# NomaDamas/AutoRAG-Research

Hardware: AMD Instinct MI355X
Metric: queries/sec (higher is better)
Workload: dtype f32

## Files before the change

### autorag_research_amd/_native.py

```python

from __future__ import annotations

import ctypes
import os
from pathlib import Path

import numpy as np

_PKG_DIR = Path(__file__).resolve().parent
LIB_PATH = _PKG_DIR / "libmi355dr.so"

_lib: ctypes.CDLL | None = None

ABI_SYMBOLS = [
    "mi355dr_create", "mi355dr_destroy", "mi355dr_last_error", "mi355dr_version", "mi355dr_reserve",
    "mi355dr_add_rows", "mi355dr_add_rows_device", "mi355dr_size", "mi355dr_dim", "mi355dr_get_rows",
    "mi355dr_update_rows", "mi355dr_update_rows_device", "mi355dr_remove_rows", "mi355dr_live_rows", "mi355dr_compact",
    "mi355dr_search", "mi355dr_search_device", "mi355dr_search_device_async", "mi355dr_search_wait",
    "mi355dr_search_subset", "mi355dr_search_subset_device", "mi355dr_score_subset", "mi355dr_search_mmr", "mi355dr_search_mmr_device", "mi355dr_mmr_select", "mi355dr_merge_groups_device", "mi355dr_search_groups", "mi355dr_search_groups_device", "mi355dr_search_range", "mi355dr_search_range_device",
    "mi355dr_search_rows", "mi355dr_search_rows_device", "mi355dr_search_range_rows", "mi355dr_search_range_rows_device", "mi355dr_view_create", "mi355dr_add_multivec", "mi355dr_size_multivec",
    "mi355dr_search_maxsim", "mi355dr_search_maxsim_device", "mi355dr_search_maxsim_subset", "mi355dr_search_maxsim_subset_device", "mi355dr_maxsim_subset", "mi355dr_maxsim_subset_ex", "mi355dr_add_multivec_device", "mi355dr_gqr_refine", "mi355dr_gqr_refine_maxsim",
    "mi355dr_set_multivec", "mi355dr_set_multivec_device", "mi355dr_live_multivec",
    "mi355dr_add_sparse", "mi355dr_size_sparse", "mi355dr_sparse_df", "mi355dr_search_sparse", "mi355dr_search_sparse_device",
    "mi355dr_search_bm25", "mi355dr_search_bm25_device",
    "mi355dr_gqr_refine_scores", "mi355dr_merge_topk_device", "mi355dr_pack_topk_device",
    "mi355dr_merge_topk_packed_device", "mi355dr_comm_unique_id", "mi355dr_comm_init", "mi355dr_comm_world", "mi355dr_comm_count", "mi355dr_comm_init_custom",
    "mi355dr_search_sharded_device", "mi355dr_search_range_sharded_device", "mi355dr_search_rows_sharded_device",
    "mi355dr_search_range_rows_sharded_device", "mi355dr_search_mmr_sharded_device", "mi355dr_mmr_select_sharded",
    "mi355dr_set_option", "mi355dr_get_stat",
    "mi355dr_reset_stats", "mi355dr_timer_start", "mi355dr_timer_stop", "mi355dr_synchronize",
    "mi355dr_dev_alloc", "mi355dr_dev_free", "mi355dr_dev_upload", "mi355dr_dev_download",
    "mi355dr_diag_mfma_stream",
    "mi355dr_debug_screen_dense", "mi355dr_debug_screen_hits", "mi355dr_debug_screen_bound", "mi355dr_debug_i8_state", "mi355dr_debug_rescore",
    "mi355dr_debug_maxsim_pass",
]


ALLGATHER_FN = ctypes.CFUNCTYPE(ctypes.c_int, ctypes.c_void_p, ctypes.c_void_p, ctypes.c_size_t, ctypes.c_void_p, ctypes.c_void_p)


class NativeError(RuntimeError):

    def __init__(self, code: int, message: str):
        super().__init__(f"libmi355dr error {code}: {message}")
        self.code = code


def _preload_torch_hip_runtime() -> None:
    import importlib.util
    import sys

    if "torch" in sys.modules:
        return
    try:
        spec = importlib.util.find_spec("torch")
    except (ImportError, ValueError):
        return
    if spec is None or not spec.submodule_search_locations:
        return
    libdir = Path(list(spec.submodule_search_locations)[0]) / "lib"
    for name in ("libhsa-runtime64.so", "libamdhip64.so"):
        f = libdir / name
        if f.exists():
            try:
                ctypes.CDLL(str(f), mode=getattr(os, "RTLD_NOW", 2) | getattr(os, "RTLD_GLOBAL", 0x100))
            except OSError:
                return


def load() -> ctypes.CDLL:
    global _lib
    if _lib is not None:
        return _lib
    if not LIB_PATH.exists():
        raise ImportError(
            f"{LIB_PATH} not found: build it with `python -c 'import __graft_entry__ as g; g.build()'` "
            "(hipcc --offload-arch=gfx950).  There is no CPU fallback for the search path."
        )
    _preload_torch_hip_runtime()
    L = ctypes.CDLL(str(LIB_PATH), mode=getattr(os, "RTLD_NOW", 2))
    vp, c_int, i64 = ctypes.c_void_p, ctypes.c_int, ctypes.c_int64
    f32p, f64p = ctypes.POINTER(ctypes.c_float), ctypes.POINTER(ctypes.c_double)
    i64p, i32p = ctypes.POINTER(ctypes.c_int64), ctypes.POINTER(ctypes.c_int32)
    L.mi355dr_create.restype = c_int
    L.mi355dr_create.argtypes = [ctypes.POINTER(vp), c_int, c_int, c_int]
    L.mi355dr_destroy.restype = None
    L.mi355dr_destroy.argtypes = [vp]
    L.mi355dr_last_error.restype = ctypes.c_char_p
    L.mi355dr_last_error.argtypes = [vp]
    L.mi355dr_version.restype = c_int
    L.mi355dr_reserve.restype = c_int
    L.mi355dr_reserve.argtypes = [vp, i64]
    L.mi355dr_add_rows.restype = c_int
    L.mi355dr_add_rows.argtypes = [vp, f32p, i64]
    L.mi355dr_add_rows_device.restype = c_int
    L.mi355dr_add_rows_device.argtypes = [vp, vp, i64]
    L.mi355dr_update_rows.restype = c_int
    L.mi355dr_update_rows.argtypes = [vp, i64p, f32p, i64]
    L.mi355dr_update_rows_device.restype = c_int
    L.mi355dr_update_rows_device.argtypes = [vp, i64p, vp, i64]
    L.mi355dr_remove_rows.restype = c_int
    L.mi355dr_remove_rows.argtypes = [vp, i64p, i64]
    L.mi355dr_compact.restype = c_int
    L.mi355dr_compact.argtypes = [vp, i64p]
    L.mi355dr_live_rows.restype = i64
    L.mi355dr_live_rows.argtypes = [vp]
    L.mi355dr_size.restype = i64
    L.mi355dr_size.argtypes = [vp]
    L.mi355dr_dim.restype = c_int
    L.mi355dr_dim.argtypes = [vp]
    L.mi355dr_get_rows.restype = c_int
    L.mi355dr_get_rows.argtypes = [vp, i64, i64, f32p]
    L.mi355dr_search.restype = c_int
    L.mi355dr_search.argtypes = [vp, f32p, c_int, c_int, f64p, i64p]
    L.mi355dr_search_device.restype = c_int
    L.mi355dr_search_device.argtypes = [vp, vp, c_int, c_int, vp, vp, vp]
    L.mi355dr_search_device_async.restype = c_int
    L.mi355dr_search_device_async.argtypes = [vp, vp, c_int, c_int, vp, vp, vp, i64p]
    L.mi355dr_search_wait.restype = c_int
    L.mi355dr_search_wait.argtypes = [vp, i64]
    L.mi355dr_search_subset.restype = c_int
    L.mi355dr_search_subset.argtypes = [vp, f32p, c_int, c_int, i64p, i64, f64p, i64p]
    L.mi355dr_search_subset_device.restype = c_int
    L.mi355dr_search_subset_device.argtypes = [vp, vp, c_int, c_int, i64p, i64, vp, vp, vp]
    L.mi355dr_score_subset.restype = c_int
    L.mi355dr_score_subset.argtypes = [vp, f32p, c_int, i64p, c_int, f64p]
    L.mi355dr_search_mmr.restype = c_int
    L.mi355dr_search_mmr.argtypes = [vp, f32p, c_int, c_int, c_int, ctypes.c_double, f64p, i64p]
    L.mi355dr_search_mmr_device.restype = c_int
    L.mi355dr_search_mmr_device.argtypes = [vp, vp, c_int, c_int, c_int, ctypes.c_double, vp, vp, vp]
    L.mi355dr_mmr_select.restype = c_int
    L.mi355dr_mmr_select.argtypes = [vp, f32p, c_int, c_int, i64p, c_int, ctypes.c_double, f64p, i64p]
    L.mi355dr_merge_groups_device.restype = c_int
    L.mi355dr_merge_groups_device.argtypes = [vp, vp, vp, c_int, c_int, i32p, c_int, c_int, vp, vp, vp, vp]
    L.mi355dr_search_groups.restype = c_int
    L.mi355dr_search_groups.argtypes = [vp, f32p, i32p, c_int, c_int, c_int, f64p, i64p, i32p]
    L.mi355dr_search_groups_device.restype = c_int
    L.mi355dr_search_groups_device.argtypes = [vp, vp, i32p, c_int, c_int, c_int, vp, vp, vp, vp]
    L.mi355dr_search_range.restype = c_int
    L.mi355dr_search_range.argtypes = [vp, f32p, c_int, f64p, c_int, f64p, i64p, i64p]
    L.mi355dr_search_range_device.restype = c_int
    L.mi355dr_search_range_device.argtypes = [vp, vp, c_int, f64p, c_int, vp, vp, vp, vp]
    L.mi355dr_search_rows.restype = c_int
    L.mi355dr_search_rows.argtypes = [vp, i64p, c_int, c_int, c_int, f64p, i64p]
    L.mi355dr_search_rows_device.restype = c_int
    L.mi355dr_search_rows_device.argtypes = [vp, i64p, c_int, c_int, c_int, vp, vp, vp]
    L.mi355dr_search_range_rows.restype = c_int
    L.mi355dr_search_range_rows.argtypes = [vp, i64p, c_int, f64p, c_int, c_int, f64p, i64p, i64p]
    L.mi355dr_search_range_rows_device.restype = c_int
    L.mi355dr_search_range_rows_device.argtypes = [vp, i64p, c_int, f64p, c_int, c_int, vp, vp, vp, vp]
    L.mi355dr_view_create.restype = c_int
    L.mi355dr_view_create.argtypes = [vp, i64p, i64, i64p, i64, ctypes.POINTER(vp)]
    L.mi355dr_add_multivec.restype = c_int
    L.mi355dr_add_multivec.argtypes = [vp, f32p, i64p, i64]
    L.mi355dr_size_multivec.restype = i64
    L.mi355dr_size_multivec.argtypes = [vp]
    L.mi355dr_search_maxsim.restype = c_int
    L.mi355dr_search_maxsim.argtypes = [vp, f32p, i32p, c_int, c_int, f32p, i64p]
    L.mi355dr_search_maxsim_device.restype = c_int
    L.mi355dr_search_maxsim_device.argtypes = [vp, vp, i32p, c_int, c_int, vp, vp, vp]
    L.mi355dr_search_maxsim_subset.restype = c_int
    L.mi355dr_search_maxsim_subset.argtypes = [vp, f32p, i32p, c_int, c_int, i64p, i64, f32p, i64p]
    L.mi355dr_search_maxsim_subset_device.restype = c_int
    L.mi355dr_search_maxsim_subset_device.argtypes = [vp, vp, i32p, c_int, c_int, i64p, i64, vp, vp, vp]
    L.mi355dr_maxsim_subset.restype = c_int
    L.mi355dr_maxsim_subset.argtypes = [vp, f32p, i32p, c_int, i64p, c_int, f32p]
    L.mi355dr_maxsim_subset_ex.restype = c_int
    L.mi355dr_maxsim_subset_ex.argtypes = [vp, f32p, i32p, c_int, i64p, c_int, c_int, f32p]
    L.mi355dr_add_multivec_device.restype = c_int
    L.mi355dr_add_multivec_device.argtypes = [vp, vp, i64p, i64]
    L.mi355dr_set_multivec.restype = c_int
    L.mi355dr_set_multivec.argtypes = [vp, i64p, f32p, i64p, i64]
    L.mi355dr_set_multivec_device.restype = c_int
    L.mi355dr_set_multivec_device.argtypes = [vp, i64p, vp, i64p, i64]
    L.mi355dr_live_multivec.restype = i64
    L.mi355dr_live_multivec.argtypes = [vp]
    c_double = ctypes.c_double
    L.mi355dr_add_sparse.restype = c_int
    L.mi355dr_add_sparse.argtypes = [vp, i32p, i64p, i64]
    L.mi355dr_size_sparse.restype = i64
    L.mi355dr_size_sparse.argtypes = [vp]
    L.mi355dr_sparse_df.restype = c_int
    L.mi355dr_sparse_df.argtypes = [vp, i32p, i64, i64p]
    L.mi355dr_search_sparse.restype = c_int
    L.mi355dr_search_sparse.argtypes = [vp, i32p, f64p, i32p, c_int, c_int, c_double, c_double, f64p, i64p]
    L.mi355dr_search_sparse_device.restype = c_int
    L.mi355dr_search_sparse_device.argtypes = [vp, i32p, f64p, i32p, c_int, c_int, c_double, c_double, vp, vp, vp]
    L.mi355dr_search_bm25.restype = c_int
    L.mi355dr_search_bm25.argtypes = [vp, i32p, i32p, c_int, c_int, c_double, c_double, f64p, i64p]
    L.mi355dr_search_bm25_device.restype = c_int
    L.mi355dr_search_bm25_device.argtypes = [vp, i32p, i32p, c_int, c_int, c_double, c_double, vp, vp, vp]
    L.mi355dr_gqr_refine.restype = c_int
    L.mi355dr_gqr_refine.argtypes = [vp, f64p, c_int, i64p, c_int, f64p, c_int, c_double, c_double, c_double, f64p]
    L.mi355dr_gqr_refine_maxsim.restype = c_int
    L.mi355dr_gqr_refine_maxsim.argtypes = [vp, f64p, i32p, c_int, i64p, c_int, f64p, c_int, c_double, c_double, c_double,
                                            f64p]
    L.mi355dr_gqr_refine_scores.restype = c_int
    L.mi355dr_gqr_refine_scores.argtypes = [vp, f64p, i32p, c_int, c_int, f64p, c_int, c_double, c_double, c_double, f64p]
    L.mi355dr_merge_topk_device.restype = c_int
    L.mi355dr_merge_topk_device.argtypes = [vp, vp, vp, c_int, c_int, c_int, vp, vp, vp]
    L.mi355dr_pack_topk_device.restype = c_int
    L.mi355dr_pack_topk_device.argtypes = [vp, vp, vp, c_int, c_int, vp, vp]
    L.mi355dr_merge_topk_packed_device.restype = c_int
    L.mi355dr_merge_topk_packed_device.argtypes = [vp, vp, c_int, c_int, c_int, vp, vp, vp]
    L.mi355dr_comm_unique_id.restype = c_int
    L.mi355dr_comm_unique_id.argtypes = [vp, ctypes.c_size_t]
    L.mi355dr_comm_init.restype = c_int
    L.mi355dr_comm_init.argtypes = [vp, c_int, c_int, vp, ctypes.c_size_t]
    L.mi355dr_comm_init_custom.restype = c_int
    L.mi355dr_comm_init_custom.argtypes = [vp, c_int, c_int, ALLGATHER_FN, vp]
    L.mi355dr_comm_world.restype = c_int
    L.mi355dr_comm_world.argtypes = [vp]
    L.mi355dr_comm_count.restype = c_int
    L.mi355dr_comm_count.argtypes = [vp, ctypes.POINTER(c_int)]
    L.mi355dr_search_sharded_device.restype = c_int
    L.mi355dr_search_sharded_device.argtypes = [vp, vp, c_int, c_int, vp, vp, vp]
    L.mi355dr_search_range_sharded_device.restype = c_int
    L.mi355dr_search_range_sharded_device.argtypes = [vp, vp, c_int, f64p, c_int, vp, vp, vp, vp]
    L.mi355dr_search_rows_sharded_device.restype = c_int
    L.mi355dr_search_rows_sharded_device.argtypes = [vp, i64p, c_int, c_int, c_int, vp, vp, vp]
    L.mi355dr_search_range_rows_sharded_device.restype = c_int
    L.mi355dr_search_range_rows_sharded_device.argtypes = [vp, i64p, c_int, f64p, c_int, c_int, vp, vp, vp, vp]
    L.mi355dr_search_mmr_sharded_device.restype = c_int
    L.mi355dr_search_mmr_sharded_device.argtypes = [vp, vp, c_int, c_int, c_int, ctypes.c_double, vp, vp, vp]
    L.mi355dr_mmr_select_sharded.restype = c_int
    L.mi355dr_mmr_select_sharded.argtypes = [vp, f32p, c_int, c_int, i64p, c_int, ctypes.c_double, f64p, i64p]
    L.mi355dr_set_option.restype = c_int
    L.mi355dr_set_option.argtypes = [vp, ctypes.c_char_p, i64]
    L.mi355dr_get_stat.restype = c_int
    L.mi355dr_get_stat.argtypes = [vp, ctypes.c_char_p, i64p]
    L.mi355dr_reset_stats.restype = c_int
    L.mi355dr_reset_stats.argtypes = [vp]
    L.mi355dr_timer_start.restype = c_int
    L.mi355dr_timer_start.argtypes = [vp]
    L.mi355dr_timer_stop.restype = c_int
    L.mi355dr_timer_stop.argtypes = [vp, f64p]
    L.mi355dr_synchronize.restype = c_int
    L.mi355dr_synchronize.argtypes = [vp]
    L.mi355dr_dev_alloc.restype = c_int
    L.mi355dr_dev_alloc.argtypes = [vp, ctypes.c_size_t, ctypes.POINTER(vp)]
    L.mi355dr_dev_free.restype = c_int
    L.mi355dr_dev_free.argtypes = [vp, vp]
    L.mi355dr_dev_upload.restype = c_int
    L.mi355dr_dev_upload.argtypes = [vp, vp, vp, ctypes.c_size_t]
    L.mi355dr_dev_download.restype = c_int
    L.mi355dr_dev_download.argtypes = [vp, vp, vp, ctypes.c_size_t]
    L.mi355dr_debug_screen_dense.restype = c_int
    L.mi355dr_debug_screen_dense.argtypes = [vp, f32p, c_int, i64, i64, f32p]
    L.mi355dr_debug_screen_hits.restype = c_int
    L.mi355dr_debug_screen_hits.argtypes = [vp, f32p, c_int, i64, i64, f32p, c_int, ctypes.POINTER(c_int), i32p, f32p,
                                            ctypes.POINTER(c_int), ctypes.POINTER(c_int)]
    L.mi355dr_debug_screen_bound.restype = c_int
    L.mi355dr_debug_screen_bound.argtypes = [vp, f32p, c_int, f32p]
    L.mi355dr_debug_i8_state.restype = c_int
    L.mi355dr_debug_i8_state.argtypes = [vp, f32p, c_int, f32p, f32p, i64, i64, f32p, f32p]
    L.mi355dr_debug_rescore.restype = c_int
    L.mi355dr_debug_rescore.argtypes = [vp, f32p, c_int, i32p, i64p, i64, f32p, f64p]
    L.mi355dr_debug_maxsim_pass.restype = c_int
    L.mi355dr_debug_maxsim_pass.argtypes = [vp, f32p, i32p, c_int, c_int, i64p, i64, c_int, ctypes.POINTER(c_int), f32p, f32p, i32p,
                                            ctypes.POINTER(c_int), f32p, ctypes.POINTER(c_int), ctypes.POINTER(c_int)]
    L.mi355dr_diag_mfma_stream.restype = c_int
    L.mi355dr_diag_mfma_stream.argtypes = [c_int, c_int, ctypes.c_double, ctypes.POINTER(ctypes.c_double)]
    _lib = L
    return L


def diag_mfma_stream(device: int, fmt: str, seconds: float) -> float:
    out = ctypes.c_double(0.0)
    rc = load().mi355dr_diag_mfma_stream(int(device), {"i8": 0, "bf16": 1}[fmt], float(seconds), ctypes.byref(out))
    if rc != 0:
        raise NativeError(rc, "mi355dr_diag_mfma_stream failed")
    return float(out.value)


def check(handle, rc: int) -> None:
    if rc != 0:
        msg = load().mi355dr_last_error(handle)
        raise NativeError(rc, msg.decode("utf-8", "replace") if msg else "")


def f32c(a) -> np.ndarray:
    return np.ascontiguousarray(a, dtype=np.float32)


def ptr(a: np.ndarray, ct):
    return a.ctypes.data_as(ctypes.POINTER(ct))
```

### autorag_research_amd/csrc/dev_common.h

```cpp
#pragma once
#include <hip/hip_runtime.h>
#include <stdint.h>

namespace mi355 {

constexpr int kWave = 64;
constexpr int kQBlockMax = 1024;
constexpr int kKMax = 1024;
constexpr int kCandCap = 2048;
constexpr int kCandCapWide = 4096;
constexpr int kSortMax = 4096;
constexpr int kIrrCap = 1024;
constexpr uint64_t kKeyNaN = 0xFFFFFFFFFFFFFFFFull;
static_assert(kSortMax >= kKMax + kCandCap, "the general prune's sort must hold k kept entries and a full candidate list");

constexpr int kStOverflow = 1;
constexpr int kStIrregular = 2;

struct QueryState {
    float* qn;
    uint16_t* qhat;
    float* thr;
    int* cnt;
    int* best_n;
    uint64_t* best_key;
    int32_t* best_row;
    uint64_t* thr_key;
    int32_t* thr_row;
    int* status;
    float* E;
    float* E16;
    float* sc;
    float* kq;
    int8_t* qhat8;
    int* carry;
};

__device__ __forceinline__ float bf16_bits_to_f32(uint16_t h) { return __uint_as_float((uint32_t)h << 16); }

__host__ __device__ inline float bf16_screen_bound(float e_q, float e_c, int d, float cscale = 1.0f) {
    return 1.0001f * (e_q * cscale + e_c) + 3.0f * e_q * e_c + (8.0f * (float)d * 5.9604645e-8f + 1.5258789e-5f) * cscale;
}

constexpr float kI8Z = 6.0f;
constexpr int kI8GroupRows = 32;
struct I8Group {
    float step;
    float err;
};
__host__ __device__ inline float i8_row_peak_limit(int d) { return kI8Z / sqrtf((float)d); }
__host__ __device__ inline float i8_query_bound(float e_q, int d) {
    return 1.0001f * e_q + 4.0f * (float)d * 5.9604645e-8f + 1.5258789e-5f + 4.0e-6f;
}
__host__ __device__ inline float i8_pair_factor(float e_q) { return 1.0001f + 3.0f * e_q; }
__device__ __forceinline__ int i8_block_threshold(float th, float m, float ek) {
    const float r = __builtin_amdgcn_rcpf(m);
    const float x = (th - ek) * r;
    const float y = floorf(x - fabsf(x) * 4.8e-7f - fabsf(th) * (1.2e-7f * r) - 2.0f);
    int out;
    asm("v_cvt_i32_f32 %0, %1" : "=v"(out) : "v"(y));
    return out;
}

__device__ __forceinline__ float bits_f(uint32_t u) { return __uint_as_float(u); }

__device__ __forceinline__ uint16_t f32_to_bf16_rn(float f) {
    uint32_t u = __float_as_uint(f);
    u += 0x7FFFu + ((u >> 16) & 1u);
    return (uint16_t)(u >> 16);
}

__device__ __forceinline__ double cosine_distance_from(float dot, float nq, float nc) {
    double sim = (double)dot / sqrt((double)nq * (double)nc);
    if (sim > 1.0) sim = 1.0;
    else if (sim < -1.0) sim = -1.0;
    return 1.0 - sim;
}

__device__ __forceinline__ double distance_from(int metric, float dot, float nq, float nc) {
    return metric == 0 ? cosine_distance_from(dot, nq, nc) : (double)dot * -1.0;
}

__device__ __forceinline__ float sim_of_dist(int metric, double dist) {
    return metric == 0 ? (float)(1.0 - dist) : (float)(-dist);
}

__device__ __forceinline__ uint64_t dist_to_key(double d) {
    if (d != d) return kKeyNaN;
    uint64_t b = (uint64_t)__double_as_longlong(d);
    return (b >> 63) ? ~b : (b | 0x8000000000000000ull);
}
__device__ __forceinline__ double key_to_dist(uint64_t k) {
    if (k == kKeyNaN) return __longlong_as_double(0x7FF8000000000000ll);
    uint64_t b = (k >> 63) ? (k & 0x7FFFFFFFFFFFFFFFull) : ~k;
    return __longlong_as_double((long long)b);
}

__device__ __forceinline__ float float_below(float x) {
    if (x != x || x == -__builtin_inff()) return x;
    uint32_t u = __float_as_uint(x);
    if (x > 0.0f) u -= 1u;
    else if (x < 0.0f) u += 1u;
    else u = 0x80000001u;
    return __uint_as_float(u);
}

__device__ __forceinline__ bool norm_is_regular(float n2) { return n2 >= 1e-30f && n2 <= 1e30f; }

constexpr float kDeadNrm2 = -1.0f;
constexpr int32_t kRowNone = 0x7FFFFFFF;
__host__ __device__ __forceinline__ bool row_is_dead(float n2) { return n2 < 0.0f; }
__device__ __forceinline__ uint64_t exact_key_of(int metric, float dot, float nq, float nc, int32_t& row) {
    if (row_is_dead(nc)) {
        row = kRowNone;
        return kKeyNaN;
    }
    return dist_to_key(distance_from(metric, dot, nq, nc));
}

__device__ __forceinline__ int next_pow2(int x) {
    int p = 1;
    while (p < x) p <<= 1;
    return p;
}

__device__ __forceinline__ void bitonic_desc_f32(float* v, int n) {
    for (int k = 2; k <= n; k <<= 1) {
        for (int j = k >> 1; j > 0; j >>= 1) {
            for (int i = threadIdx.x; i < n; i += blockDim.x) {
                const int p = i ^ j;
                if (p > i) {
                    const bool desc = ((i & k) == 0);
                    const float a = v[i], b = v[p];
                    if (desc ? (a < b) : (a > b)) {
                        v[i] = b;
                        v[p] = a;
                    }
                }
            }
            __syncthreads();
        }
    }
}

constexpr int kSelPerLane = 16;

__device__ __forceinline__ uint32_t f32_order_key(float f) {
    const uint32_t u = __float_as_uint(f);
    return (u & 0x80000000u) ? ~u : (u | 0x80000000u);
}

template <int NS>
__device__ __forceinline__ int wave_count_ge_n(const uint32_t (&key)[kSelPerLane], uint32_t x) {
    int c = 0;
#pragma unroll
    for (int j = 0; j < NS; ++j) c += __builtin_popcountll(__builtin_amdgcn_ballot_w64(key[j] >= x));
    return c;
}
template <int NS>
__device__ __forceinline__ uint32_t wave_nth_largest_n(const uint32_t (&key)[kSelPerLane], int n) {
    uint32_t x = 0;
    for (int b = 31; b >= 0; --b) {
        const uint32_t t = x | (1u << b);
        if (wave_count_ge_n<NS>(key, t) >= n) x = t;
    }
    return x;
}
__device__ __forceinline__ int wave_count_ge(const uint32_t (&key)[kSelPerLane], uint32_t x, int entries) {
    if (entries <= kWave) return wave_count_ge_n<1>(key, x);
    if (entries <= 2 * kWave) return wave_count_ge_n<2>(key, x);
    if (entries <= 4 * kWave) return wave_count_ge_n<4>(key, x);
    if (entries <= 8 * kWave) return wave_count_ge_n<8>(key, x);
    return wave_count_ge_n<kSelPerLane>(key, x);
}
__device__ __forceinline__ uint32_t wave_nth_largest(const uint32_t (&key)[kSelPerLane], int n, int entries) {
    if (entries <= kWave) return wave_nth_largest_n<1>(key, n);
    if (entries <= 2 * kWave) return wave_nth_largest_n<2>(key, n);
    if (entries <= 4 * kWave) return wave_nth_largest_n<4>(key, n);
    if (entries <= 8 * kWave) return wave_nth_largest_n<8>(key, n);
    return wave_nth_largest_n<kSelPerLane>(key, n);
}

__device__ __forceinline__ int wave_count_ge(const uint32_t (&key)[kSelPerLane], uint32_t x) {
    return wave_count_ge_n<kSelPerLane>(key, x);
}
__device__ __forceinline__ uint32_t wave_nth_largest(const uint32_t (&key)[kSelPerLane], int n) {
    return wave_nth_largest_n<kSelPerLane>(key, n);
}
// ... 263 lines not shown
```

### autorag_research_amd/csrc/index.h

```cpp
#pragma once
#include <climits>
#include <hip/hip_runtime.h>

#include <algorithm>
#include <cmath>
#include <cstdio>
#include <cstring>
#include <mutex>
#include <string>
#include <vector>

#include "dev_common.h"
#include "mi355dr.h"

namespace mi355 {
template <class T, bool Pinned = false>
struct DevBuf {
    T* p = nullptr;
    size_t bytes = 0;
    DevBuf() = default;
    DevBuf(const DevBuf&) = delete;
    DevBuf& operator=(const DevBuf&) = delete;
    ~DevBuf() { release(); }
    void release() {
        if (p) (void)(Pinned ? hipHostFree(p) : hipFree(p));
        p = nullptr;
        bytes = 0;
    }
    hipError_t grow(size_t want) {
        if (want <= bytes) return hipSuccess;
        void* q = nullptr;
        const hipError_t e = Pinned ? hipHostMalloc(&q, want) : hipMalloc(&q, want);
        if (e != hipSuccess) return e;
        release();
        p = (T*)q;
        bytes = want;
        return hipSuccess;
    }
    void swap(DevBuf& o) {
        std::swap(p, o.p);
        std::swap(bytes, o.bytes);
    }
    operator T*() const { return p; }
};
template <class T>
using HostBuf = DevBuf<T, true>;

struct Event {
    hipEvent_t e = nullptr;
    Event() = default;
    Event(const Event&) = delete;
    Event& operator=(const Event&) = delete;
    ~Event() {
        if (e) (void)hipEventDestroy(e);
    }
    hipError_t create(unsigned flags = hipEventDefault) { return e ? hipSuccess : hipEventCreateWithFlags(&e, flags); }
    operator hipEvent_t() const { return e; }
};

struct EventPair {
    hipEvent_t a, b;
    int big;
};
struct EventPairs {
    std::vector<EventPair> v;
    ~EventPairs() {
        for (auto& p : v) {
            (void)hipEventDestroy(p.a);
            (void)hipEventDestroy(p.b);
        }
    }
};
struct MultiVecStore;
struct SparseStore;
struct Pass {
    int k = 0;
    int level = 0;
    bool screening = false;
    bool i8 = false;
    bool wide = false;
    int cap = 0;
    const char* refused = nullptr;
};
struct Pending {
    bool active = false;
    Event done;
    HostBuf<int> status_host;
    hipStream_t stream = nullptr;
    const float* q_dev = nullptr;
    int B = 0;
    Pass pass;
    double* out_dist = nullptr;
    int64_t* out_rows = nullptr;
};
struct RetryBufs {
    DevBuf<float> q;
    DevBuf<double> dist;
    DevBuf<int64_t> rows;
    DevBuf<int> map;
};
constexpr int kPendingRing = 4;

template <class... Bufs>
hipError_t grow_each(size_t n, Bufs&... bufs) {
    hipError_t e = hipSuccess;
    (void)(((e = bufs.grow(n * sizeof(*bufs.p))) == hipSuccess) && ...);
    return e;
}
struct MmrBufs {
    DevBuf<double> cand_dist;
    DevBuf<int64_t> cand_rows;
    DevBuf<unsigned long long> pairs_dev;
    hipError_t reserve(size_t nb, size_t stride) {
        hipError_t e = grow_each(nb * stride, cand_dist, cand_rows);
        if (!e) e = grow_each(1, pairs_dev);
        return e;
    }
};
struct GroupBufs {
    DevBuf<int32_t> offsets, count;
    DevBuf<double> cand_dist, out_dist;
    DevBuf<int64_t> cand_rows, out_rows;
    hipError_t reserve(size_t G, size_t S, size_t fetch_k, size_t k, bool host) {
        hipError_t e = grow_each(G + 1, offsets);
        if (!e) e = grow_each(S * fetch_k, cand_dist, cand_rows);
        if (!e && host) e = grow_each(G * k, out_dist, out_rows);
        if (!e && host) e = grow_each(G, count);
        return e;
    }
};
struct RangeBufs {
    DevBuf<uint64_t> key, rkey;
    DevBuf<int32_t> row, xfrom;
    DevBuf<unsigned long long> count, stat;
    DevBuf<double> radius, fb_dist;
    DevBuf<int> redo, flag, fb_map;
    DevBuf<int64_t> fb_rows;
    DevBuf<float> fb_q;
    int collect_lds = 0;
    hipError_t reserve(size_t nb, size_t R, size_t m, size_t pairs, size_t dim) {
        hipError_t e = grow_each(nb * R, key, row);
        if (!e) e = grow_each(nb, count, rkey, xfrom, radius, flag, fb_map);
        if (!e) e = grow_each(2, stat);
        if (!e) e = grow_each(2 + 2 * pairs, redo);
        if (!e) e = grow_each(nb * dim, fb_q);
        if (!e) e = grow_each(nb * m, fb_dist, fb_rows);
        return e;
    }
};
struct RowQueryBufs {
    DevBuf<int64_t> ids, pair_row, cand_rows, cand_count;
    DevBuf<float> q, self_dot;
    DevBuf<int> valid;
    DevBuf<int32_t> pair_q;
    DevBuf<double> cand_dist, self_dist, radius;
    DevBuf<unsigned long long> skipped_dev;
    hipError_t reserve(size_t nb, size_t stride, size_t dim, bool range) {
        hipError_t e = grow_each(nb, ids, valid, pair_q, pair_row);
        if (!e) e = grow_each(nb * dim, q);
        if (!e) e = grow_each(nb * stride, cand_dist, cand_rows);
        if (!e) e = grow_each(1, skipped_dev);
        if (!e && range) e = grow_each(nb, cand_count, self_dot, self_dist, radius);
        return e;
    }
};
struct ShardBufs {
    DevBuf<int64_t> send, recv;
    DevBuf<float> stage, stage_all;
    DevBuf<unsigned long long> local_skipped;
};
}

struct mi355dr_index {
    int device = 0, dim = 0, dpad = 0, metric = 0;
    hipStream_t stream = nullptr;
    std::mutex mu;
    std::string err;
    mi355dr_index() = default;
    ~mi355dr_index() {
        if (stream) (void)hipStreamDestroy(stream);
    }

    int64_t n = 0, cap_rows = 0;
    mi355::DevBuf<float> rows;
    mi355::DevBuf<uint16_t> shadow;
    mi355::DevBuf<float> nrm2;
    mi355::DevBuf<int32_t> irr_rows;
    mi355::DevBuf<int> irr_count;
    int irr_n = 0;
    mi355::DevBuf<unsigned> n2max_dev;
    float cmax = 0.0f;
    mi355::DevBuf<unsigned> bf16_res2_dev;
    float bf16_ec = 0.00390625f;
    int dpad8 = 0;
    mi355::DevBuf<int8_t> shadow8;
    mi355::DevBuf<uint8_t> flag8;
    mi355::DevBuf<mi355::I8Group> grp8;
    mi355::DevBuf<int32_t> irr8_rows;
    mi355::DevBuf<int> irr8_count;
    int irr8_n = 0;
    mi355::DevBuf<int> dead_count;
    int64_t dead_n = 0;

    bool qstate_ready = false;
    mi355::QueryState st{};
    mi355::DevBuf<void> st_mem[sizeof(mi355::QueryState) / sizeof(void*)];
    mi355::DevBuf<float> qdev;
    mi355::DevBuf<int32_t> cand_row;
    mi355::DevBuf<float> cand_val;
    mi355::DevBuf<int> qlist_dev;
    int* status_or_dev = nullptr;
    mi355::HostBuf<int> status_host;
    mi355::DevBuf<double> out_dist_dev;
    mi355::DevBuf<int64_t> out_rows_dev;
    mi355::DevBuf<int64_t> out_count_dev;
    mi355::DevBuf<unsigned long long> stat_dev;
    mi355::DevBuf<int> prune_skip;
    mi355::DevBuf<int32_t> subset_ids;
    mi355::MmrBufs mmr;
    mi355::GroupBufs grp;
    mi355::RangeBufs rng;
    mi355::RowQueryBufs rowq;
    mi355::ShardBufs shd;
    bool is_view = false;
    mi355::DevBuf<int64_t> view_row_map;
    mi355::DevBuf<int64_t> view_doc_map;
    int64_t view_rows = 0, view_docs = 0;
    int prune_parity = 0;

    int path = 0;
    int screen_dtype = 0;
    int i8_backoff = 0, i8_probation = 0;
    int i8_demoted_k = INT_MAX;
    double i8_min_budget = 0.25;
    mi355::RetryBufs retry[3];
    mi355::Pending pend[mi355::kPendingRing];
    mi355::Pending sub_pend[4];
    int64_t seq_next = 0, seq_done = 0;
    int last_pass_k = 10;
    int maxsim_coop = -1;
    int maxsim_persistent = 0;
    int maxsim_wg = -1;
    int maxsim_tighten = 1;
    int maxsim_aligned = 1;
    int maxsim_wg_min = 8;
    int maxsim_wg_pipe = 1;
    int maxsim_pack8 = -1;
    int maxsim_wg_bps = 4;
    int maxsim_pass_groups = 4;
    int maxsim_screen = 1;
    int maxsim_subset_screen = -1;
    int64_t maxsim_subset_screen_min = 512;
    int64_t row_offset = 0;
    int round_a = 0;
    int screen_rq = 1;
    int screen_stream = 1;
    int prefilter16 = 0;
    int profile = 0;
    int starter = 1;
    int prune_companion = 1;
    int scan_dma = 1;
    int defer_round_b = 1;
    int chunk0_set = 0;
    int64_t chunk0_rows = 1024;
    int64_t chunk_growth = 3;
    int chunk_growth_set = 0;
    int64_t small_chunk_rows = 16384;
    int cap = mi355::kCandCap;
    int cap_set = 0;
    int prune_wide = 1;
    int screen_flush_sync = 1, screen_flush_lanes = 48, screen_flush_alone = 40;
    int wide_inflation_x10 = 100;
    int chunk_taper_x100 = 0;
    int64_t compact_slice_rows = 65536;
    int64_t view_slice_rows = 65536;
    int64_t range_chunk_rows = (int64_t)1 << 21;
    int range_slots = mi355::kSortMax;
    int64_t shard_stage_bytes = (int64_t)256 << 20;
    int64_t starter_rows_wide = 65536;

    int64_t s_screen_launches = 0, s_screen_ns = 0, s_screen_rows = 0, s_fallback_queries = 0, s_chunks = 0,
            s_passes = 0, s_starters = 0;
    int64_t s_big_launches = 0, s_big_ns = 0, s_big_rows = 0;
    int screen_rq_split_tests = 1;
    int64_t debug_park = 0;
    mi355::DevBuf<float> park_thr;
    int screen_drift = 3;
    mi355::DevBuf<int> rq_progress;
    int rq_epoch = 0;
    int64_t s_rq_launches = 0;
    int64_t s_retry_queries = 0;
    int64_t s_ms_screened = 0, s_ms_candidates = 0, s_ms_fallbacks = 0;
    int64_t s_ms_screen_ns = 0, s_ms_screen_launches = 0, s_ms_exact_ns = 0, s_ms_exact_launches = 0, s_ms_pack_ns = 0;
    int64_t s_ms_packed_launches = 0;
    int64_t s_ms_packed_blocks = 0;
    int64_t s_ms_packed_built = 0;
    int64_t s_ms_set_docs = 0;
    int64_t s_ms_moved_blocks = 0;
    int64_t s_compactions = 0;
    int64_t s_compact_moved_rows = 0;
    int64_t s_subset_searches = 0;
    int64_t s_subset_rows_scored = 0;
    int64_t s_subset_rerun_queries = 0;
    int64_t s_mss_searches = 0, s_mss_docs = 0, s_mss_screened = 0, s_mss_exact = 0, s_mss_fallbacks = 0;
    int64_t s_mmr_searches = 0, s_mmr_queries = 0, s_mmr_pairs = 0;
    int64_t s_group_searches = 0, s_group_subqueries = 0, s_groups_merged = 0;
    int64_t s_range_searches = 0, s_range_queries = 0, s_range_in_range = 0, s_range_candidates = 0, s_range_rescored = 0,
            s_range_redo_chunks = 0, s_range_fallback_queries = 0;
    int64_t s_rows_searches = 0, s_rows_queries = 0, s_rows_skipped = 0;
    int64_t s_shard_range_searches = 0, s_shard_rows_searches = 0, s_shard_mmr_searches = 0, s_shard_gather_bytes = 0;
    int64_t s_sparse_searches = 0, s_sparse_queries = 0, s_sparse_postings_scored = 0, s_sparse_overflows = 0;
    int sparse_tile_docs = 2048;
    int sparse_cand_cap = 2048;
    int64_t s_ms_screen_cols = 0;
    mi355::Event ms_ev[4];
    struct MsScreenForm {
        int family = 0, ncb = 0, waves = 0, bps = 0, pipe = 0, now = 0, grid = 0, reserved = 0;
    } last_screen_form;
    mi355::EventPairs ev_pool, ev_pending;
    mi355::Event t0, t1;

    void* comm = nullptr;
    int comm_rank = 0, comm_world = 0;
    mi355dr_allgather_fn comm_custom = nullptr;
    void* comm_custom_user = nullptr;
    int64_t* comm_packed[2] = {nullptr, nullptr};
    int64_t* comm_packed_all[2] = {nullptr, nullptr};
    hipStream_t comm_stream = nullptr;
    hipEvent_t comm_done[2] = {nullptr, nullptr};
    bool comm_done_armed[2] = {false, false};
    size_t comm_cap = 0;

    mi355::MultiVecStore* mv = nullptr;
    mi355::SparseStore* sp = nullptr;
};


namespace mi355 {

int fail(mi355dr_index* idx, int code, const std::string& msg);
inline int view_refuses(mi355dr_index* idx, const char* what, bool ask_parent = false) {
    return fail(idx, MI355DR_E_INVALID, std::string(what) + (ask_parent ? ": not on a view (it is a read-only snapshot under the parent's ids) -- ask the parent index"
                                                                        : ": a view is read-only"));
}
void multivec_destroy(mi355dr_index* idx);
int multivec_reserve(mi355dr_index* idx, int64_t n_blocks, int64_t n_docs);
int64_t multivec_bytes(const mi355dr_index* idx);
void sparse_destroy(mi355dr_index* idx);
int64_t sparse_bytes(const mi355dr_index* idx);
enum { kSparseStatDocs, kSparseStatTotalLen, kSparseStatPostings, kSparseStatVocab };
int64_t sparse_stat(const mi355dr_index* idx, int which);
int drain_searches(mi355dr_index* idx);
void comm_destroy(mi355dr_index* idx);
int comm_all_gather(mi355dr_index* idx, const void* send_dev, void* recv_dev, size_t bytes_per_rank, hipStream_t stream);
struct MultiVecView {
    const float* tok;
    const int64_t* blk_off;
    const int64_t* blk_off_host;
    const int32_t* tok_cnt_host;
    int dpad;
    int64_t n_docs;
};
bool multivec_view(const mi355dr_index* idx, MultiVecView* out);

__host__ __device__ inline int ms_perm(int j) {
    constexpr int P[8] = {0, 4, 2, 6, 1, 5, 3, 7};
    return (j & ~7) | P[j & 7];
}

template <class T>
inline void multivec_pack_query_row(const T* src, int d, int dpad, T* dst) {
    for (int c = 0; c < dpad; ++c) {
        const int oc = ms_perm(c);
        dst[c] = oc < d ? src[oc] : T(0);
    }
}

#define HIPCHECK(idx, expr)                                                                              \
    do {                                                                                                 \
        hipError_t e__ = (expr);                                                                         \
        if (e__ != hipSuccess) {                                                                         \
            char buf__[512];                                                                             \
            snprintf(buf__, sizeof(buf__), "%s failed: %s (%s:%d)", #expr, hipGetErrorString(e__), __FILE__, \
                     __LINE__);                                                                          \
            return mi355::fail(idx, e__ == hipErrorOutOfMemory ? MI355DR_E_NOMEM : MI355DR_E_HIP, buf__); \
        }                                                                                                \
    } while (0)

#define CHECK(expr)                          \
    do {                                     \
        int rc__ = (expr);                   \
        if (rc__ != MI355DR_OK) return rc__; \
    } while (0)

inline int64_t round_up(int64_t x, int64_t m) { return (x + m - 1) / m * m; }

}
```

### autorag_research_amd/csrc/k_prep.h

```cpp
#pragma once
#include "dev_common.h"

namespace mi355 {

__global__ __launch_bounds__(64) void k_row_nrm2(const float* __restrict__ rows, int64_t row0, int64_t n, int d,
                                                  float* __restrict__ nrm2, unsigned* __restrict__ n2max,
                                                  const int64_t* __restrict__ ids) {
    __shared__ float tile[kStageFloats];
    const int lane = threadIdx.x;
    const int64_t j = (int64_t)blockIdx.x * kWave + lane;
    const bool live = j < n;
    const int64_t i = ids ? (live ? ids[j] : 0) : row0 + j;
    const float* my_row = live ? rows + i * (int64_t)d : nullptr;
    float acc = 0.0f;
    for (int k0 = 0; k0 < d; k0 += kStageCols) {
        stage_rows(tile, my_row, k0, d, lane);
        __syncthreads();
        const int kn = min(kStageCols, d - k0);
        const float* t = tile + lane * kStageLd;
        for (int k = 0; k < kn; ++k) acc = __builtin_fmaf(t[k], t[k], acc);
        __syncthreads();
    }
    if (live) nrm2[i] = acc;
    float m = (live && norm_is_regular(acc)) ? acc : 0.0f;
// ... 13 lines not shown
    __shared__ float sh[4];
    if ((int64_t)blockIdx.x >= n) return;
    const int64_t i = ids ? ids[blockIdx.x] : row0 + blockIdx.x;
    const float n2 = nrm2[i];
    const bool regular = norm_is_regular(n2);
    const float rc = regular ? (absolute ? 1.0f : 1.0f / sqrtf(n2)) : 0.0f;
    const float* r = rows + i * (int64_t)d;
    uint16_t* s = shadow + i * (int64_t)dpad;
    float e2 = 0.0f;
    for (int k = threadIdx.x; k < dpad; k += blockDim.x) {
        uint16_t v = 0;
        if (k < d) {
            if (regular) {
                const float ch = r[k] * rc;
                v = f32_to_bf16_rn(ch);
                const float e = ch - bf16_bits_to_f32(v);
                e2 = __builtin_fmaf(e, e, e2);
            } else {
                v = (uint16_t)0x7FC0;
            }
        }
        s[k] = v;
    }
#pragma unroll
    for (int o = 32; o > 0; o >>= 1) e2 += __shfl_xor(e2, o);
    if ((threadIdx.x & 63) == 0) sh[threadIdx.x >> 6] = e2;
    __syncthreads();
    if (threadIdx.x == 0) {
        if (regular) {
            const unsigned v = __float_as_uint((sh[0] + sh[1]) + (sh[2] + sh[3]));
            if (v > *(volatile unsigned*)res2_max) atomicMax(res2_max, v);
        }
        else if (ids == nullptr) {
            int slot = atomicAdd(irr_count, 1);
            if (slot < kIrrCap) irr_rows[slot] = (int32_t)i;
        }
    }
}


__device__ __forceinline__ float block256_reduce(float v, bool is_max, float* sh) {
#pragma unroll
    for (int o = 32; o > 0; o >>= 1) {
        const float w = __shfl_xor(v, o);
        v = is_max ? fmaxf(v, w) : v + w;
    }
    __syncthreads();
    if ((threadIdx.x & 63) == 0) sh[threadIdx.x >> 6] = v;
    __syncthreads();
    return is_max ? fmaxf(fmaxf(sh[0], sh[1]), fmaxf(sh[2], sh[3])) : (sh[0] + sh[1]) + (sh[2] + sh[3]);
}

__global__ __launch_bounds__(256) void k_build_shadow8(const float* __restrict__ rows, const float* __restrict__ nrm2,
                                                        int64_t g0, int64_t n_total, int64_t first_new, int d, int dpad8,
                                                        int8_t* __restrict__ shadow8, uint8_t* __restrict__ flag8,
                                                        I8Group* __restrict__ grp, int32_t* __restrict__ irr8_rows,
                                                        int* __restrict__ irr8_count, int absolute,
                                                        const int64_t* __restrict__ groups) {
    __shared__ float s_peak[kI8GroupRows];
    __shared__ float s_err[kI8GroupRows];
    __shared__ float s_step;
    const int lane = threadIdx.x & 63, wave = threadIdx.x >> 6;
    const int64_t g = groups ? groups[blockIdx.x] : g0 + blockIdx.x;
    const int64_t row_g = g * kI8GroupRows;
    const float peak_limit = i8_row_peak_limit(d);
    for (int j = 0; j < 8; ++j) {
        const int lr = wave * 8 + j;
        const int64_t i = row_g + lr;
        float peak = -1.0f;
        if (i < n_total) {
            const float n2 = nrm2[i];
            if (norm_is_regular(n2)) {
                const float rc = absolute ? 1.0f : 1.0f / sqrtf(n2);
                const float lim = absolute ? peak_limit * sqrtf(n2) : peak_limit;
                const float* r = rows + i * (int64_t)d;
                float mx = 0.0f;
                for (int k = lane; k < d; k += kWave) mx = fmaxf(mx, fabsf(r[k] * rc));
#pragma unroll
                for (int o = 32; o > 0; o >>= 1) mx = fmaxf(mx, __shfl_xor(mx, o));
                if (mx <= lim) peak = mx;
            }
        }
        if (lane == 0) s_peak[lr] = peak;
    }
    __syncthreads();
    if (threadIdx.x == 0) {
        float mx = 0.0f;
        for (int j = 0; j < kI8GroupRows; ++j) mx = fmaxf(mx, s_peak[j]);
        s_step = mx * (1.0f / 127.0f) * 1.0000005f;
    }
    __syncthreads();
    const float step = s_step;
    const float inv_step = step > 0.0f ? 1.0f / step : 0.0f;
    for (int j = 0; j < 8; ++j) {
        const int lr = wave * 8 + j;
        const int64_t i = row_g + lr;
        if (i >= n_total) {
            if (lane == 0) s_err[lr] = 0.0f;
            continue;
        }
        const bool tight = s_peak[lr] >= 0.0f && step > 0.0f;
        const float rc = tight ? (absolute ? 1.0f : 1.0f / sqrtf(nrm2[i])) : 0.0f;
        const float* r = rows + i * (int64_t)d;
        int8_t* s = shadow8 + i * (int64_t)dpad8;
        float e2 = 0.0f;
        for (int k = lane; k < dpad8; k += kWave) {
            float qv = 0.0f;
            if (k < d && tight) {
                const float ch = r[k] * rc;
                qv = fminf(fmaxf(rintf(ch * inv_step), -127.0f), 127.0f);
                const float e = __builtin_fmaf(-step, qv, ch);
                e2 = __builtin_fmaf(e, e, e2);
            }
            s[k] = (int8_t)qv;
        }
#pragma unroll
        for (int o = 32; o > 0; o >>= 1) e2 += __shfl_xor(e2, o);
        if (lane == 0) {
            s_err[lr] = tight ? sqrtf(e2) * 1.001f : 0.0f;
            flag8[i] = tight ? 0 : 1;
            if (!tight && i >= first_new) {
                const int slot = atomicAdd(irr8_count, 1);
                if (slot < kIrrCap) irr8_rows[slot] = (int32_t)i;
            }
        }
    }
    __syncthreads();
    if (threadIdx.x == 0) {
        float mx = 0.0f;
        for (int j = 0; j < kI8GroupRows; ++j) mx = fmaxf(mx, s_err[j]);
        grp[g].step = step;
        grp[g].err = mx;
    }
}

__global__ __launch_bounds__(64) void k_prep_queries(const float* __restrict__ q, int B, int d, int dpad, int metric,
                                                      QueryState st, int dpad8, int i8, float bf16_ec, int* status_or,
                                                      int* prune_skip, int cnt0, float cscale) {
    extern __shared__ float qs[];
    const int b = blockIdx.x;
    const int lane = threadIdx.x;
    if (b == 0 && lane == 0) {
        if (status_or) *status_or = 0;
        if (prune_skip) prune_skip[0] = prune_skip[1] = 0;
    }
    uint16_t* qh = st.qhat + (int64_t)b * dpad;
    if (b >= B) {
        for (int k = lane; k < dpad; k += kWave) qh[k] = 0;
        if (lane == 0) {
            st.qn[b] = 0.0f;
            st.thr[b] = __builtin_inff();
            st.cnt[b] = 0;
            st.carry[b] = 0;
            st.best_n[b] = 0;
            st.thr_key[b] = 0;
            st.thr_row[b] = -1;
            st.status[b] = 0;
            st.E[b] = bf16_screen_bound(0.00390625f, bf16_ec, d, cscale);
            st.E16[b] = st.E[b];
            st.sc[b] = 0.0f;
            st.kq[b] = 1.0f;
        }
        if (i8)
            for (int k = lane; k < dpad8; k += kWave) st.qhat8[(int64_t)b * dpad8 + k] = 0;
        return;
    }
    const float* qr = q + (int64_t)b * d;
    for (int k = lane; k < d; k += kWave) qs[k] = qr[k];
    __syncthreads();
    float acc = 0.0f;
    for (int k = 0; k < d; ++k) acc = __builtin_fmaf(qs[k], qs[k], acc);
    const bool regular = norm_is_regular(acc);
    const float rq = regular ? 1.0f / sqrtf(acc) : 0.0f;
    float eq2 = 0.0f;
    for (int k = lane; k < dpad; k += kWave) {
        uint16_t v = 0;
        if (k < d && regular) {
            const float qh_f = qs[k] * rq;
            v = f32_to_bf16_rn(qh_f);
            const float e = qh_f - bf16_bits_to_f32(v);
            eq2 = __builtin_fmaf(e, e, eq2);
        }
        qh[k] = v;
    }
#pragma unroll
    for (int o = 32; o > 0; o >>= 1) eq2 += __shfl_xor(eq2, o);
    float E = bf16_screen_bound(sqrtf(eq2) * 1.001f, bf16_ec, d, cscale), sc = 1.0f, kq = 1.0f;
    const float E16 = E;
    if (i8) {
        float mx = 0.0f;
        for (int k = lane; k < d; k += kWave) mx = fmaxf(mx, fabsf(qs[k] * rq));
#pragma unroll
        for (int o = 32; o > 0; o >>= 1) mx = fmaxf(mx, __shfl_xor(mx, o));
        const float sq = mx / 127.0f;
        const float inv = sq > 0.0f ? 1.0f / sq : 0.0f;
        float e2 = 0.0f;
        int8_t* q8 = st.qhat8 + (int64_t)b * dpad8;
        for (int k = lane; k < dpad8; k += kWave) {
            float qv = 0.0f;
            if (k < d && regular) {
                const float qh_f = qs[k] * rq;
                qv = fminf(fmaxf(rintf(qh_f * inv), -127.0f), 127.0f);
                const float e = __builtin_fmaf(-sq, qv, qh_f);
                e2 = __builtin_fmaf(e, e, e2);
            }
            q8[k] = (int8_t)qv;
        }
#pragma unroll
        for (int o = 32; o > 0; o >>= 1) e2 += __shfl_xor(e2, o);
        const float e_q = sqrtf(e2) * 1.001f;
        E = i8_query_bound(e_q, d) * cscale;
        kq = i8_pair_factor(e_q);
        sc = sq;
    }
    if (lane == 0) {
        st.qn[b] = acc;
        st.E[b] = E;
        st.E16[b] = E16;
        st.sc[b] = sc;
        st.kq[b] = kq;
        st.thr[b] = (regular || metric == 2) ? -__builtin_inff() : __builtin_inff();
        st.cnt[b] = cnt0;
        st.carry[b] = 0;
        st.best_n[b] = 0;
        st.thr_key[b] = kKeyNaN;
        st.thr_row[b] = 0x7FFFFFFF;
        st.status[b] = regular ? 0 : kStIrregular;
    }
}

}
```

### autorag_research_amd/csrc/k_select.h

```cpp
#pragma once
#include "dev_common.h"

namespace mi355 {

struct PruneArgs {
    const float* rows;
    const float* nrm2;
    const float* q;
    QueryState st;
    int32_t* cand_row;
    float* cand_val;
    const int* qlist;
    unsigned long long* stat;
    int cap, d, k, metric;
    int exact;
    const uint8_t* flag8;
    float cscale;
    const uint16_t* shadow16;
    int dpad;
    int round_a;
    int* skip_list;
    int skip_parity;
    int thr_only;
    int one_wave_only;
    int defer_b;
};

__device__ __forceinline__ float unit_sim(int metric, double dist, float inv_qn) {
    return metric == 0 ? (float)(1.0 - dist) : (float)(-dist) * inv_qn;
}
__device__ __forceinline__ float screen_threshold(int metric, double dist_k, float E, float nq) {
    if (metric == 0) return float_below((float)((1.0 - dist_k) - (double)E));
    const double u = -dist_k / sqrt((double)nq);
    return float_below((float)(u - fabs(u) * 4e-6 - (double)E));
}

constexpr int kPruneSmallThreads = 64, kPruneSmallSort = 1024;
constexpr int kPruneBigThreads = 256, kPruneBigSort = kSortMax;

__host__ __device__ inline size_t prune_qs_floats(int d) { return ((size_t)d + 3) / 4 * 4 + 16; }
__host__ __device__ inline size_t prune_lds_bytes(int d, int threads, int sortmax, int dpad16) {
    size_t x = (size_t)(threads / kWave) * kStageFloats * sizeof(float);
    size_t lf = (size_t)sortmax * sizeof(float);
    if (lf > x) x = lf;
    return (size_t)sortmax * 8 + (size_t)sortmax * 4 + x + (size_t)sortmax * 4 + prune_qs_floats(d) * 4 + (size_t)dpad16 * 4;
}

template <int PER, int T, bool ROWS = false>
__device__ __forceinline__ void load_candidate_keys(uint32_t (&key)[PER], const float* __restrict__ cval,
                                                    const int32_t* __restrict__ crow, const uint8_t* __restrict__ flag8,
                                                    int n_new, int tid, int32_t* rows_out = nullptr) {
    float v[PER];
    int32_t r[PER];
    const int last = n_new - 1;
#pragma unroll
    for (int j = 0; j < PER; ++j) {
        v[j] = 0.0f;
        r[j] = 0;
        if (j * T >= n_new) continue;
        v[j] = cval[min(j * T + tid, last)];
        if (ROWS) r[j] = crow[min(j * T + tid, last)];
    }
    uint8_t f[PER];
#pragma unroll
    for (int j = 0; j < PER; ++j) f[j] = 0;
    if (flag8 != nullptr) {
        if (!ROWS) {
#pragma unroll
            for (int j = 0; j < PER; ++j) {
                if (j * T >= n_new) continue;
                r[j] = crow[min(j * T + tid, last)];
            }
        }
#pragma unroll
        for (int j = 0; j < PER; ++j) {
            if (j * T >= n_new) continue;
            f[j] = flag8[r[j]];
        }
    }
#pragma unroll
    for (int j = 0; j < PER; ++j) {
        uint32_t kk = 0;
        if (j * T + tid < n_new) {
            if (v[j] != v[j]) kk = 0xFFFFFFFFu;
            else if (!f[j]) kk = f32_order_key(v[j]);
        }
        key[j] = kk;
        if (ROWS) rows_out[j] = r[j];
    }
}

template <int THREADS, int SORT>
__device__ __forceinline__ void prune_body(const PruneArgs& a, char* smem);

template <int THREADS, int SORT>
__global__ __launch_bounds__(THREADS) void k_prune(PruneArgs a) {
    extern __shared__ __attribute__((aligned(16))) char smem[];
    const bool list_mode = a.skip_list != nullptr && a.qlist == nullptr;
    const int tid = threadIdx.x;
    const int lane = tid & 63, wave = tid >> 6;
    int q = a.qlist ? a.qlist[blockIdx.x] : blockIdx.x;
    if (SORT == kPruneBigSort && list_mode) {
        if (blockIdx.x == 0 && tid == 0) a.skip_list[a.skip_parity ^ 1] = 0;
        const int n_left = a.skip_list[a.skip_parity];
        for (int i = blockIdx.x; i < n_left; i += gridDim.x) {
            PruneArgs b = a;
            b.skip_list = nullptr;
            b.qlist = a.skip_list + 2 + a.skip_parity * kQBlockMax + i - 0;
            b.qlist -= blockIdx.x;
            prune_body<THREADS, SORT>(b, smem);
            __syncthreads();
        }
        return;
    }
    prune_body<THREADS, SORT>(a, smem);
}

template <int THREADS, int SORT>
__device__ __forceinline__ void prune_body(const PruneArgs& a, char* smem) {
    constexpr int kWaves = THREADS / kWave;
    uint64_t* SK = (uint64_t*)smem;
    int32_t* SR = (int32_t*)(smem + (size_t)SORT * 8);
    char* X = smem + (size_t)SORT * 12;
    constexpr size_t xa = (size_t)kWaves * kStageFloats * sizeof(float), xb = (size_t)SORT * sizeof(float);
    constexpr size_t xbytes = xa > xb ? xa : xb;
    float* Lf = (float*)X;
    float* tiles = (float*)X;
    int32_t* R = (int32_t*)(X + xbytes);
    float* qs = (float*)(X + xbytes + (size_t)SORT * 4);
    int& s_cnt = *(int*)(X + xbytes + (size_t)SORT * 4 + (prune_qs_floats(a.d) - 16) * 4);
    float* q16 = qs + prune_qs_floats(a.d);
    const bool list_mode = a.skip_list != nullptr && a.qlist == nullptr;
    const int q = a.qlist ? a.qlist[blockIdx.x] : blockIdx.x;
    const int tid = threadIdx.x;
    const int lane = tid & 63, wave = tid >> 6;
    const int raw_cnt = a.st.cnt[q];
    const int n_best = a.st.best_n[q];
    if (raw_cnt == 0) return;
    if (a.exact && SORT < kPruneBigSort) return;
    auto leave_for_general = [&]() {
        if (a.one_wave_only) {
            if (tid == 0) {
                a.st.status[q] |= kStOverflow;
                a.st.cnt[q] = 0;
            }
            return;
        }
        if (list_mode && tid == 0) {
            const int i = atomicAdd(&a.skip_list[a.skip_parity], 1);
            a.skip_list[2 + a.skip_parity * kQBlockMax + i] = q;
        }
    };
    if (raw_cnt > a.cap) {
        if (SORT < kPruneBigSort) {
            leave_for_general();
            return;
        }
        if (tid == 0) {
            a.st.status[q] |= kStOverflow;
            a.st.cnt[q] = 0;
        }
        return;
    }
    if (n_best + raw_cnt > SORT) {
        if (SORT < kPruneBigSort) {
            leave_for_general();
            return;
        }
        if (tid == 0) {
            a.st.status[q] |= kStOverflow;
            a.st.cnt[q] = 0;
        }
        return;
    }
    const int n_new = raw_cnt;
    const int32_t* crow = a.cand_row + (int64_t)q * a.cap;
    const float* cval = a.cand_val + (int64_t)q * a.cap;
    uint64_t* bkey = a.st.best_key + (int64_t)q * kKMax;
// ... 37 lines not shown
                int n = 0;
#pragma unroll
                for (int j = 0; j < kSelPerLane; ++j) {
                    if (j * kWave >= n_new) break;
                    const bool want = key[j] >= x && key[j] != 0 && !((in_a >> j) & 1u);
                    const unsigned long long bal = __builtin_amdgcn_ballot_w64(want);
                    const int pos = n + (int)__builtin_amdgcn_mbcnt_hi((unsigned)(bal >> 32),
                                                                       __builtin_amdgcn_mbcnt_lo((unsigned)bal, 0));
                    if (want && pos < room) {
                        R[pos] = j * kWave + lane;
                        if (mark) in_a |= 1u << j;
                    }
                    n += __builtin_popcountll(bal);
                }
                return min(n, room);
            };
            wave_sync();
            const int wantA = min(n_cand, min(kWave, max(a.k, a.round_a > 0 ? a.round_a : max(32, 2 * a.k))));
            int nA = 0;
            if (wantA > 0) {
                const uint32_t xA = wave_nth_largest(key, wantA, n_new);
                nA = compact(xA, kWave, true);
                wave_sync();
                rescore_list(nA, n_best);
            }
            for (int i = lane; i < n_best; i += kWave) {
                SK[i] = bkey[i];
                SR[i] = brow[i];
            }
            kept_loaded = true;
            wave_sync();
            int n1 = n_best + nA;
            int nB = 0, carried = 0;
            if (n_cand > nA && !a.thr_only) {
                float cut = -__builtin_inff(), cut16 = -__builtin_inff();
                if (n1 >= a.k) {
                    uint32_t sk[kSelPerLane];
#pragma unroll
                    for (int j = 0; j < kSelPerLane; ++j) {
                        const int e = j * kWave + lane;
                        uint32_t kk = 0;
                        if (e < n1 && SK[e] != kKeyNaN) kk = f32_order_key(sim_of_dist(a.metric, key_to_dist(SK[e])));
                        sk[j] = kk;
                    }
                    if (wave_count_ge(sk, 1u, n1) >= a.k) {
                        const uint32_t xs = wave_nth_largest(sk, a.k, n1);
                        const float kth = __uint_as_float((xs & 0x80000000u) ? (xs & 0x7FFFFFFFu) : ~xs);
                        const float ku = a.metric == 0 ? kth : kth * inv_qn;
                        cut = ku - fabsf(ku) * (a.metric == 0 ? 0.0f : 4e-6f) - E * 1.001f - 2e-6f * a.cscale;
                        if (a.shadow16 != nullptr && a.metric == 0) cut16 = kth - a.st.E16[q] * 1.001f - 2e-6f;
                    }
                }
                const uint32_t xB = cut == -__builtin_inff() ? 1u : f32_order_key(cut);
                nB = compact(xB, SORT, false);
                wave_sync();
                if (a.defer_b && cut != -__builtin_inff()) {
                    int32_t* crow_w = a.cand_row + (int64_t)q * a.cap;
                    float* cval_w = a.cand_val + (int64_t)q * a.cap;
                    int32_t cr[kSelPerLane];
                    float cv[kSelPerLane];
#pragma unroll
                    for (int j = 0; j < kSelPerLane; ++j) {
                        if (j * kWave >= nB) break;
                        const int i = j * kWave + lane;
                        if (i < nB) {
                            cr[j] = crow[R[i]];
                            cv[j] = cval[R[i]];
                        }
                    }
                    asm volatile("s_waitcnt vmcnt(0)" ::: "memory");
#pragma unroll
                    for (int j = 0; j < kSelPerLane; ++j) {
                        if (j * kWave >= nB) break;
                        const int i = j * kWave + lane;
                        if (i < nB) {
                            crow_w[i] = cr[j];
                            cval_w[i] = cv[j];
                        }
                    }
                    carried = nB;
                    nB = 0;
                }
                if (a.shadow16 != nullptr && cut16 != -__builtin_inff() && nB > 0) {
                    const int words = a.dpad / 2;
                    int nS = 0;
                    for (int base = 0; base < nB; base += kWave) {
                        const int e = base + lane;
                        const bool live = e < nB;
                        const int ci = live ? R[e] : 0;
                        const float* rp = live ? (const float*)(a.shadow16 + (int64_t)crow[ci] * a.dpad) : nullptr;
                        const float t16 = staged_dot16(tile, rp, q16, words, lane);
                        const bool keep = live && !(t16 < cut16);
                        const unsigned long long bal = __builtin_amdgcn_ballot_w64(keep);
                        const int pos = nS + (int)__builtin_amdgcn_mbcnt_hi((unsigned)(bal >> 32),
                                                                           __builtin_amdgcn_mbcnt_lo((unsigned)bal, 0));
                        wave_sync();
                        if (keep) R[pos] = ci;
                        nS += __builtin_popcountll(bal);
                    }
                    nB = nS;
                    wave_sync();
                }
                rescore_list(nB, n1);
            }
            if (lane == 0) a.stat[2 * q + 1] += (unsigned long long)(nA + nB);
            wave_sync();
            const int n_tot = n1 + nB;
            uint64_t* K2 = (uint64_t*)X;
            int32_t* R2 = (int32_t*)(X + (size_t)SORT * 8);
            int n_sel = n_tot;
            if (n_tot > a.k) {
                uint32_t sk[kSelPerLane];
#pragma unroll
                for (int j = 0; j < kSelPerLane; ++j) {
                    const int e = j * kWave + lane;
                    uint32_t kk = 0;
                    if (e < n_tot) kk = SK[e] == kKeyNaN ? 1u : f32_order_key(sim_of_dist(a.metric, key_to_dist(SK[e])));
                    sk[j] = kk;
                }
                const uint32_t xs = wave_nth_largest(sk, a.k, n_tot);
                n_sel = 0;
#pragma unroll
                for (int j = 0; j < kSelPerLane; ++j) {
                    if (j * kWave >= n_tot) break;
                    const bool want = sk[j] >= xs && sk[j] != 0;
                    const unsigned long long bal = __builtin_amdgcn_ballot_w64(want);
                    const int pos = n_sel + (int)__builtin_amdgcn_mbcnt_hi((unsigned)(bal >> 32),
                                                                           __builtin_amdgcn_mbcnt_lo((unsigned)bal, 0));
                    if (want) {
                        K2[pos] = SK[j * kWave + lane];
                        R2[pos] = SR[j * kWave + lane];
                    }
                    n_sel += __builtin_popcountll(bal);
                }
            } else {
                for (int i = lane; i < n_tot; i += kWave) {
                    K2[i] = SK[i];
                    R2[i] = SR[i];
                }
            }
            const int np = next_pow2(max(n_sel, 1));
            for (int i = n_sel + lane; i < np; i += kWave) {
                K2[i] = kKeyNaN;
                R2[i] = 0x7FFFFFFF;
            }
            __syncthreads();
            bitonic_asc_key_row(K2, R2, np);
            const int n_keep = min(a.k, n_sel);
            if (!a.thr_only)
                for (int i = lane; i < n_keep; i += kWave) {
                    bkey[i] = K2[i];
                    brow[i] = R2[i];
                }
            if (lane == 0) {
                if (!a.thr_only) a.st.best_n[q] = n_keep;
                a.st.cnt[q] = carried;
                a.st.carry[q] = carried;
                if (n_keep >= a.k) {
                    const uint64_t wk = K2[a.k - 1];
                    if (!a.thr_only) {
                        a.st.thr_key[q] = wk;
                        a.st.thr_row[q] = R2[a.k - 1];
                    }
                    if (wk != kKeyNaN && !(a.st.status[q] & kStIrregular))
                        a.st.thr[q] = screen_threshold(a.metric, key_to_dist(wk), E, nq);
                }
            }
            return;
        }
    }
    if (!a.exact) {
        const int nLp = next_pow2(n_new);
        for (int i = tid; i < nLp; i += THREADS) {
            float v = -__builtin_inff();
            if (i < n_new) {
                v = cval[i];
                if (v != v) v = __builtin_inff();
                else if (a.flag8 && a.flag8[crow[i]]) v = -__builtin_inff();
            }
            Lf[i] = v;
            R[i] = i;
        }
        if (tid == 0) s_cnt = 0;
        __syncthreads();
        bitonic_desc_f32_i32(Lf, R, nLp);
        for (int i = tid; i < nLp; i += THREADS)
            if (Lf[i] > -__builtin_inff() && (i + 1 == nLp || !(Lf[i + 1] > -__builtin_inff()))) s_cnt = i + 1;
        for (int k = tid; k < a.d; k += THREADS) qs[k] = a.q[(int64_t)q * a.d + k];
        __syncthreads();
        const int n_cand = s_cnt;
        __syncthreads();
        float* tile = tiles + wave * kStageFloats;
        auto rescore = [&](int e0, int e1, int dst) {
            for (int base = e0; base < e1; base += THREADS) {
                const int e = base + wave * kWave + lane;
                const bool live = e < e1;
                const int32_t row = live ? crow[R[e]] : -1;
                const float* rp = live ? a.rows + (int64_t)row * a.d : nullptr;
                float acc = 0.0f;
                if (base + wave * kWave < e1) acc = staged_dot(tile, rp, qs, a.d, lane);
                if (live) {
                    int32_t kept = row;
                    SK[dst + (e - e0)] = exact_key_of(a.metric, acc, nq, a.nrm2[row], kept);
                    SR[dst + (e - e0)] = kept;
                }
            }
        };
        const int nA = min(n_cand, min(THREADS, max(32, 2 * a.k)));
        rescore(0, nA, n_best);
        int n_pass = nA;
        if (n_cand > nA) {
            for (int i = tid; i < n_best; i += THREADS) {
                SK[i] = bkey[i];
                SR[i] = brow[i];
            }
            kept_loaded = true;
            const int n1 = n_best + nA;
            const int np1 = next_pow2(n1);
            for (int i = n1 + tid; i < np1; i += THREADS) {
                SK[i] = kKeyNaN;
                SR[i] = 0x7FFFFFFF;
            }
            __syncthreads();
            bitonic_asc_key_row(SK, SR, np1);
            n_base = min(a.k, n1);
            float cut = -__builtin_inff();
            if (n1 >= a.k) {
                const uint64_t wk = SK[a.k - 1];
                if (wk != kKeyNaN) {
                    const float ku = unit_sim(a.metric, key_to_dist(wk), inv_qn);
                    cut = ku - fabsf(ku) * (a.metric == 0 ? 0.0f : 4e-6f) - E * 1.001f - 2e-6f * a.cscale;
                }
            }
            if (tid == 0) s_cnt = nA;
            __syncthreads();
            for (int i = nA + tid; i < n_cand; i += THREADS) {
                const float v = cval[R[i]];
                if (!(v < cut)) atomicMax(&s_cnt, i + 1);
            }
            __syncthreads();
            n_pass = s_cnt;
            rescore(nA, n_pass, n_base);
            n_res = n_pass - nA;
        } else {
            n_res = nA;
        }
        if (tid == 0) a.stat[2 * q + 1] += (unsigned long long)n_pass;
    } else {
        n_res = n_new;
        for (int i = tid; i < n_new; i += THREADS) {
            int32_t row = crow[i];
            SK[n_best + i] = exact_key_of(a.metric, cval[i], nq, a.nrm2[row], row);
            SR[n_best + i] = row;
        }
    }
    if (!kept_loaded)
        for (int i = tid; i < n_best; i += THREADS) {
            SK[i] = bkey[i];
            SR[i] = brow[i];
        }
    const int n_tot = n_base + n_res;
    const int np = next_pow2(n_tot);
    for (int i = n_tot + tid; i < np; i += THREADS) {
        SK[i] = kKeyNaN;
        SR[i] = 0x7FFFFFFF;
    }
    __syncthreads();
    bitonic_asc_key_row(SK, SR, np);
    const int n_keep = min(a.k, n_tot);
    for (int i = tid; i < n_keep; i += THREADS) {
        bkey[i] = SK[i];
        brow[i] = SR[i];
    }
    if (tid == 0) {
        a.st.best_n[q] = n_keep;
        a.st.cnt[q] = 0;
        if (n_keep >= a.k) {
            const uint64_t wk = SK[a.k - 1];
            a.st.thr_key[q] = wk;
            a.st.thr_row[q] = SR[a.k - 1];
            if (!a.exact && wk != kKeyNaN && !(a.st.status[q] & kStIrregular))
                a.st.thr[q] = screen_threshold(a.metric, key_to_dist(wk), E, nq);
        }
    }
}

__global__ __launch_bounds__(64) void k_emit_irregular(const int32_t* __restrict__ irr_rows, int irr_n, QueryState st,
                                                        int32_t* cand_row, float* cand_val, int cap, int skip_below) {
    const int q = blockIdx.x;
    if (st.status[q] & kStIrregular) return;
    for (int i = threadIdx.x; i < irr_n; i += blockDim.x) {
        if (irr_rows[i] < skip_below) continue;
        const int slot = atomicAdd(&st.cnt[q], 1);
        if (slot < cap) {
            cand_row[(int64_t)q * cap + slot] = irr_rows[i];
            cand_val[(int64_t)q * cap + slot] = __builtin_nanf("");
        }
    }
}

__global__ __launch_bounds__(64) void k_finalize(QueryState st, int k, int64_t row_offset, const int64_t* __restrict__ row_map,
                                                  double* out_dist, int64_t* out_rows, int* status_or) {
    const int q = blockIdx.x;
    const int n = st.best_n[q];
    for (int s = threadIdx.x; s < k; s += blockDim.x) {
        if (s < n && st.best_row[(int64_t)q * kKMax + s] != kRowNone) {
            out_dist[(int64_t)q * k + s] = key_to_dist(st.best_key[(int64_t)q * kKMax + s]);
            const int32_t r = st.best_row[(int64_t)q * kKMax + s];
            out_rows[(int64_t)q * k + s] = row_map ? row_map[r] : (int64_t)r + row_offset;
        } else {
            out_dist[(int64_t)q * k + s] = __longlong_as_double(0x7FF8000000000000ll);
            out_rows[(int64_t)q * k + s] = -1;
        }
    }
    if (threadIdx.x == 0 && st.status[q] != 0) atomicOr(status_or, st.status[q]);
}

__global__ __launch_bounds__(256) void k_merge_topk(const double* __restrict__ dist_all,
                                                     const int64_t* __restrict__ rows_all, int64_t rank_stride, int world,
                                                     int B, int k, double* out_dist, int64_t* out_rows) {
    extern __shared__ __attribute__((aligned(16))) char smem[];
    uint64_t* SK = (uint64_t*)smem;
    const int np_ = next_pow2(world * k);
    int32_t* SI = (int32_t*)(smem + (size_t)np_ * 8);
    const int q = blockIdx.x;
    const int n = world * k;
    const int np = next_pow2(n);
    for (int i = threadIdx.x; i < np; i += blockDim.x) {
        if (i < n) {
            const int w = i / k, s = i % k;
            const int64_t src = (int64_t)w * rank_stride + (int64_t)q * k + s;
            const int64_t r = rows_all[src];
            SK[i] = r < 0 ? kKeyNaN : dist_to_key(dist_all[src]);
            SI[i] = r < 0 ? 0x7FFFFFFF : i;
        } else {
            SK[i] = kKeyNaN;
            SI[i] = 0x7FFFFFFF;
        }
    }
    __syncthreads();
    for (int kk = 2; kk <= np; kk <<= 1) {
        for (int j = kk >> 1; j > 0; j >>= 1) {
            for (int i = threadIdx.x; i < np; i += blockDim.x) {
                const int p = i ^ j;
                if (p > i) {
                    const bool asc = ((i & kk) == 0);
                    const uint64_t ka = SK[i], kb = SK[p];
                    const int32_t ia = SI[i], ib = SI[p];
                    auto grow = [&](int32_t ix) -> int64_t {
                        if (ix == 0x7FFFFFFF) return INT64_MAX;
                        const int w = ix / k, s = ix % k;
                        return rows_all[(int64_t)w * rank_stride + (int64_t)q * k + s];
                    };
                    bool a_before_b, b_before_a;
                    if (ka != kb) {
                        a_before_b = ka < kb;
                        b_before_a = !a_before_b;
                    } else {
                        const int64_t ra = grow(ia), rb = grow(ib);
                        a_before_b = ra < rb;
                        b_before_a = rb < ra;
                    }
                    if (asc ? b_before_a : a_before_b) {
                        SK[i] = kb;
                        SK[p] = ka;
                        SI[i] = ib;
                        SI[p] = ia;
                    }
                }
            }
            __syncthreads();
        }
    }
    for (int s = threadIdx.x; s < k; s += blockDim.x) {
        const int32_t ix = s < np ? SI[s] : 0x7FFFFFFF;
        if (ix != 0x7FFFFFFF) {
            const int w = ix / k, ss = ix % k;
            const int64_t src = (int64_t)w * rank_stride + (int64_t)q * k + ss;
            out_dist[(int64_t)q * k + s] = dist_all[src];
            out_rows[(int64_t)q * k + s] = rows_all[src];
        } else {
            out_dist[(int64_t)q * k + s] = __longlong_as_double(0x7FF8000000000000ll);
            out_rows[(int64_t)q * k + s] = -1;
        }
    }
}

}
```

### autorag_research_amd/csrc/mi355dr.hip

```cpp
#include "index.h"
#include "k_prep.h"
#include "k_scan.h"
#include "k_scan_ids.h"
#include "subset_ids.h"
#include "screen_common.h"
#include "k_screen.h"
#include "k_screen256c.h"
#include "k_screen_rq.h"

#define MI355_RQ_FORMS(X) X(1) X(2) X(3) X(4) X(5) X(6)
inline bool screen_rq_has(int ksteps) { return ksteps >= 1 && ksteps <= 6; }
#include "k_screen_stream.h"
#include "k_select.h"
#include "k_prune_wide.h"
#include "k_update.h"
#include "k_compact.h"
#include "k_view.h"
#include "k_block.h"
#include "k_mmr.h"
#include "mmr_order.h"
#include "k_groups.h"
#include "k_range.h"
#include "k_rows.h"
#include "k_shard.h"

using namespace mi355;

namespace {
std::mutex g_err_mu;
std::string g_err;
}

namespace mi355 {
int fail(mi355dr_index* idx, int code, const std::string& msg) {
    if (idx) idx->err = msg;
    else {
        std::lock_guard<std::mutex> g(g_err_mu);
        g_err = msg;
    }
    return code;
}
}

namespace {


int ensure_capacity(mi355dr_index* idx, int64_t want_rows) {
    if (want_rows <= idx->cap_rows) return MI355DR_OK;
    int64_t new_cap = std::max<int64_t>(want_rows, idx->cap_rows + idx->cap_rows / 2);
    new_cap = round_up(std::max<int64_t>(new_cap, kT2), kT2);
    DevBuf<float> rows, nrm2;
    DevBuf<uint16_t> shadow;
    DevBuf<int8_t> shadow8;
    DevBuf<uint8_t> flag8;
    DevBuf<I8Group> grp8;
    const size_t row_b = (size_t)idx->dim * sizeof(float), sh_b = (size_t)idx->dpad * sizeof(uint16_t), sh8_b = (size_t)idx->dpad8;
    const size_t grp_b = (size_t)(new_cap / kI8GroupRows) * sizeof(I8Group);
    HIPCHECK(idx, rows.grow(new_cap * row_b));
    HIPCHECK(idx, shadow.grow(new_cap * sh_b));
    HIPCHECK(idx, nrm2.grow(new_cap * sizeof(float)));
    HIPCHECK(idx, shadow8.grow(new_cap * sh8_b));
    HIPCHECK(idx, flag8.grow(new_cap));
    HIPCHECK(idx, grp8.grow(grp_b));
    hipStream_t s = idx->stream;
    HIPCHECK(idx, hipMemsetAsync(shadow, 0, new_cap * sh_b, s));
    HIPCHECK(idx, hipMemsetAsync(shadow8, 0, new_cap * sh8_b, s));
    HIPCHECK(idx, hipMemsetAsync(flag8, 0, new_cap, s));
    HIPCHECK(idx, hipMemsetAsync(grp8, 0, grp_b, s));
    if (idx->n > 0) {
        const size_t n = idx->n, live_grp_b = (n + kI8GroupRows - 1) / kI8GroupRows * sizeof(I8Group);
        HIPCHECK(idx, hipMemcpyAsync(rows, idx->rows, n * row_b, hipMemcpyDeviceToDevice, s));
        HIPCHECK(idx, hipMemcpyAsync(shadow, idx->shadow, n * sh_b, hipMemcpyDeviceToDevice, s));
        HIPCHECK(idx, hipMemcpyAsync(nrm2, idx->nrm2, n * sizeof(float), hipMemcpyDeviceToDevice, s));
        HIPCHECK(idx, hipMemcpyAsync(shadow8, idx->shadow8, n * sh8_b, hipMemcpyDeviceToDevice, s));
        HIPCHECK(idx, hipMemcpyAsync(flag8, idx->flag8, n, hipMemcpyDeviceToDevice, s));
        HIPCHECK(idx, hipMemcpyAsync(grp8, idx->grp8, live_grp_b, hipMemcpyDeviceToDevice, s));
    }
    HIPCHECK(idx, hipStreamSynchronize(s));
    idx->rows.swap(rows);
    idx->shadow.swap(shadow);
    idx->nrm2.swap(nrm2);
    idx->shadow8.swap(shadow8);
    idx->flag8.swap(flag8);
    idx->grp8.swap(grp8);
    idx->cap_rows = new_cap;
    return MI355DR_OK;
}

int ensure_qstate(mi355dr_index* idx) {
    if (idx->qstate_ready) return MI355DR_OK;
    const size_t B = kQBlockMax;
    auto own = [&](auto*& view, size_t bytes) {
        DevBuf<void>& mem = idx->st_mem[((char*)&view - (char*)&idx->st) / sizeof(void*)];
        const hipError_t e = mem.grow(bytes);
        view = static_cast<std::remove_reference_t<decltype(view)>>(mem.p);
        return e;
    };
    HIPCHECK(idx, own(idx->st.qn, B * sizeof(float)));
    HIPCHECK(idx, own(idx->st.qhat, B * idx->dpad * sizeof(uint16_t)));
    HIPCHECK(idx, own(idx->st.thr, B * sizeof(float)));
    HIPCHECK(idx, own(idx->st.cnt, B * sizeof(int)));
    HIPCHECK(idx, own(idx->st.best_n, B * sizeof(int)));
    HIPCHECK(idx, own(idx->st.best_key, B * kKMax * sizeof(uint64_t)));
    HIPCHECK(idx, own(idx->st.best_row, B * kKMax * sizeof(int32_t)));
    HIPCHECK(idx, own(idx->st.thr_key, B * sizeof(uint64_t)));
    HIPCHECK(idx, own(idx->st.thr_row, B * sizeof(int32_t)));
    HIPCHECK(idx, own(idx->st.status, (B + 1) * sizeof(int)));
    idx->status_or_dev = idx->st.status + B;
    HIPCHECK(idx, own(idx->st.E, B * sizeof(float)));
    HIPCHECK(idx, own(idx->st.E16, B * sizeof(float)));
    HIPCHECK(idx, own(idx->st.sc, B * sizeof(float)));
    HIPCHECK(idx, own(idx->st.kq, B * sizeof(float)));
    HIPCHECK(idx, idx->rq_progress.grow(kRqProgressWords * sizeof(int)));
    HIPCHECK(idx, hipMemset(idx->rq_progress, 0, kRqProgressWords * sizeof(int)));
    HIPCHECK(idx, own(idx->st.qhat8, B * idx->dpad8));
    HIPCHECK(idx, own(idx->st.carry, B * sizeof(int)));
    HIPCHECK(idx, idx->qdev.grow(B * idx->dim * sizeof(float)));
    HIPCHECK(idx, idx->cand_row.grow(B * kCandCapWide * sizeof(int32_t)));
    HIPCHECK(idx, idx->cand_val.grow(B * kCandCapWide * sizeof(float)));
    HIPCHECK(idx, idx->qlist_dev.grow(2 * B * sizeof(int)));
    HIPCHECK(idx, idx->status_host.grow((B + 1) * sizeof(int)));
    HIPCHECK(idx, idx->out_dist_dev.grow(B * kKMax * sizeof(double)));
    HIPCHECK(idx, idx->out_rows_dev.grow(B * kKMax * sizeof(int64_t)));
    HIPCHECK(idx, idx->out_count_dev.grow(B * sizeof(int64_t)));
    HIPCHECK(idx, idx->prune_skip.grow((2 + 2 * B) * sizeof(int)));
    HIPCHECK(idx, idx->stat_dev.grow(2 * B * sizeof(unsigned long long)));
    HIPCHECK(idx, hipMemsetAsync(idx->stat_dev, 0, 2 * B * sizeof(unsigned long long), idx->stream));
    if (prune_lds_bytes(idx->dim, kPruneBigThreads, kPruneBigSort, 0) > 160 * 1024 || scan_lds_bytes(idx->dim, 1) > 160 * 1024)
        return fail(idx, MI355DR_E_UNSUPPORTED, "dim too large for the select kernels' LDS budget");
    HIPCHECK(idx, hipFuncSetAttribute((const void*)k_prune<kPruneBigThreads, kPruneBigSort>,
                                      hipFuncAttributeMaxDynamicSharedMemorySize,
                                      (int)prune_lds_bytes(idx->dim, kPruneBigThreads, kPruneBigSort, 0)));
    HIPCHECK(idx, hipFuncSetAttribute((const void*)k_prune<kPruneSmallThreads, kPruneSmallSort>,
                                      hipFuncAttributeMaxDynamicSharedMemorySize,
                                      (int)prune_lds_bytes(idx->dim, kPruneSmallThreads, kPruneSmallSort, idx->dpad)));
    HIPCHECK(idx, hipFuncSetAttribute((const void*)k_prune_wide<2, 32>, hipFuncAttributeMaxDynamicSharedMemorySize,
                                      (int)prune_wide_lds_bytes(idx->dim, 2)));
    {
        int per = kScanQ;
        while (per > 1 && scan_lds_bytes(idx->dim, per) > 150 * 1024) per >>= 1;
        HIPCHECK(idx, hipFuncSetAttribute((const void*)k_scan, hipFuncAttributeMaxDynamicSharedMemorySize,
                                          (int)scan_lds_bytes(idx->dim, per)));
    }
    HIPCHECK(idx, hipFuncSetAttribute((const void*)k_scan32, hipFuncAttributeMaxDynamicSharedMemorySize, kScan32Lds));
    HIPCHECK(idx, hipFuncSetAttribute((const void*)k_scan_ids, hipFuncAttributeMaxDynamicSharedMemorySize,
                                      (int)scan_ids_lds_bytes(idx->dim, kScanQ)));
    HIPCHECK(idx, hipFuncSetAttribute((const void*)k_screen<false>, hipFuncAttributeMaxDynamicSharedMemorySize, kScreenLds));
    HIPCHECK(idx, hipFuncSetAttribute((const void*)k_screen<true>, hipFuncAttributeMaxDynamicSharedMemorySize, kScreenLds));
    {
        const int stream_lds = kStreamQueryBytesMax + kStreamStages * kStreamStageBytes;
        HIPCHECK(idx, hipFuncSetAttribute((const void*)k_screen_stream<false, 32>, hipFuncAttributeMaxDynamicSharedMemorySize, stream_lds));
        HIPCHECK(idx, hipFuncSetAttribute((const void*)k_screen_stream<true, 32>, hipFuncAttributeMaxDynamicSharedMemorySize, stream_lds));
        HIPCHECK(idx, hipFuncSetAttribute((const void*)k_screen_stream<false, 64>, hipFuncAttributeMaxDynamicSharedMemorySize, stream_lds));
        HIPCHECK(idx, hipFuncSetAttribute((const void*)k_screen_stream<true, 64>, hipFuncAttributeMaxDynamicSharedMemorySize, stream_lds));
    }
    HIPCHECK(idx, hipFuncSetAttribute((const void*)k_screen256c<false>, hipFuncAttributeMaxDynamicSharedMemorySize,
                                      kScreen256Lds));
    HIPCHECK(idx, hipFuncSetAttribute((const void*)k_screen256c<true>, hipFuncAttributeMaxDynamicSharedMemorySize,
                                      kScreen256Lds));
#define MI355_RQ_ATTR(KS)                                                                                              \
    HIPCHECK(idx, hipFuncSetAttribute((const void*)k_screen_rq<KS, true, true>, hipFuncAttributeMaxDynamicSharedMemorySize, rq_lds(KS)));
    MI355_RQ_FORMS(MI355_RQ_ATTR)
#undef MI355_RQ_ATTR
    HIPCHECK(idx, hipFuncSetAttribute((const void*)k_screen_rq<6, false, true>, hipFuncAttributeMaxDynamicSharedMemorySize, rq_lds(6)));
    HIPCHECK(idx, hipFuncSetAttribute((const void*)k_merge_topk, hipFuncAttributeMaxDynamicSharedMemorySize,
                                      kSortMax * 12));
    if (mmr_lds_bytes(idx->dim, kMmrMax) > 160 * 1024)
        return fail(idx, MI355DR_E_UNSUPPORTED, "dim too large for the select kernels' LDS budget");
    HIPCHECK(idx, hipFuncSetAttribute((const void*)k_mmr_select, hipFuncAttributeMaxDynamicSharedMemorySize,
                                      (int)mmr_lds_bytes(idx->dim, kMmrMax)));
    HIPCHECK(idx, hipFuncSetAttribute((const void*)k_shard_mmr_select, hipFuncAttributeMaxDynamicSharedMemorySize,
                                      (int)mmr_lds_bytes(idx->dim, kMmrMax)));
    HIPCHECK(idx, hipFuncSetAttribute((const void*)k_merge_groups, hipFuncAttributeMaxDynamicSharedMemorySize,
                                      (int)groups_lds_bytes(kSortMax)));
    idx->qstate_ready = true;
    return MI355DR_OK;
}

inline float screen_bound(int d) {
    return (float)(std::ldexp(1.0, -7) + std::ldexp(1.0, -15) + 8.0 * d * std::ldexp(1.0, -24));
}

EventPair take_events(mi355dr_index* idx) {
    if (!idx->ev_pool.v.empty()) {
        EventPair p = idx->ev_pool.v.back();
        idx->ev_pool.v.pop_back();
        return p;
    }
    EventPair p{};
    (void)hipEventCreate(&p.a);
    (void)hipEventCreate(&p.b);
    return p;
}

void drain_events(mi355dr_index* idx) {
    std::vector<EventPair> keep;
    for (auto& p : idx->ev_pending.v) {
        if (hipEventQuery(p.b) == hipErrorNotReady) {
            keep.push_back(p);
            continue;
        }
        float ms = 0.f;
        if (hipEventElapsedTime(&ms, p.a, p.b) == hipSuccess) {
            idx->s_screen_ns += (int64_t)(ms * 1e6);
            if (p.big) idx->s_big_ns += (int64_t)(ms * 1e6);
        }
        idx->ev_pool.v.push_back(p);
    }
    idx->ev_pending.v.swap(keep);
}

constexpr double kInflationBf16 = 5.0, kInflationI8 = 16.0;
constexpr double kSmallBlockBudget = 1.6;
constexpr double kInflationI8Wide = 10.0, kInflationBf16Wide = 4.0;
inline bool wide_ok(const mi355dr_index* idx, int k) { return idx->prune_wide && k >= kWideKMin && k <= kWideKMax; }
inline double growth_budget(const mi355dr_index* idx, int k, bool i8) {
    if (wide_ok(idx, k) && idx->path != MI355DR_PATH_SCAN) {
        const int room = std::min(kWideEntries, idx->cap_set ? idx->cap : kCandCapWide);
        return 0.75 * room / ((double)k * (i8 ? idx->wide_inflation_x10 / 10.0 : kInflationBf16Wide)) - 1.0;
    }
    const int room = k < kPruneSmallSort / 2 ? kPruneSmallSort - k : idx->cap;
    return 0.6 * std::min(room, idx->cap) / ((double)k * (i8 ? kInflationI8 : kInflationBf16));
}

inline bool i8_available(const mi355dr_index* idx) { return idx->irr8_n <= kIrrCap; }
Pass decide_pass(const mi355dr_index* idx, int k, int level, bool force_scan, const char* no_screen = nullptr) {
    Pass ps;
    ps.k = k;
    ps.level = level;
    const int path = force_scan ? (int)MI355DR_PATH_SCAN : idx->path;
    if (level > 0) ps.i8 = false;
    else if (idx->screen_dtype == MI355DR_SCREEN_I8) ps.i8 = true;
    else ps.i8 = idx->screen_dtype == MI355DR_SCREEN_AUTO && i8_available(idx) && k < idx->i8_demoted_k &&
                 growth_budget(idx, k, true) >= idx->i8_min_budget;
    const bool screen_possible = ps.i8 ? i8_available(idx) : idx->irr_n <= kIrrCap;
    ps.screening = idx->n > 0 && screen_possible && path != MI355DR_PATH_SCAN;
    ps.wide = ps.screening && wide_ok(idx, k);
    ps.cap = !idx->cap_set && ps.wide ? kCandCapWide : idx->cap;
    if (idx->screen_dtype == MI355DR_SCREEN_I8 && !i8_available(idx) && path != MI355DR_PATH_SCAN)
        ps.refused = "int8 screen unavailable: too many rows outside the residual limit";
    else if (path == MI355DR_PATH_SCREEN && !screen_possible && idx->n > 0) ps.refused = no_screen;
    return ps;
}
inline bool idle_i8(const mi355dr_index* idx) { return decide_pass(idx, idx->last_pass_k, 0, false).i8; }

int launch_prune(mi355dr_index* idx, hipStream_t s, const Pass& ps, int nblocks, const int* qlist, int exact,
                 bool thr_only = false, bool one_wave_only = false, bool defer_b = false) {
    PruneArgs pa{};
    pa.thr_only = thr_only ? 1 : 0;
    pa.one_wave_only = one_wave_only ? 1 : 0;
    pa.defer_b = defer_b && idx->defer_round_b ? 1 : 0;
    pa.rows = idx->rows;
    pa.nrm2 = idx->nrm2;
    pa.q = idx->qdev;
    pa.st = idx->st;
    pa.cand_row = idx->cand_row;
    pa.cand_val = idx->cand_val;
    pa.qlist = qlist;
    pa.stat = idx->stat_dev;
    pa.cap = ps.cap;
    pa.d = idx->dim;
    pa.k = ps.k;
    pa.metric = idx->metric;
    pa.exact = exact;
    pa.flag8 = (ps.i8 && (idx->irr8_n > 0 || idx->dead_n > 0)) ? idx->flag8 : nullptr;
    pa.cscale = idx->metric == MI355DR_METRIC_IP ? idx->cmax : 1.0f;
    pa.shadow16 = (ps.i8 && idx->metric == 0 && !exact && idx->prefilter16) ? idx->shadow : nullptr;
    pa.dpad = idx->dpad;
    pa.round_a = idx->round_a;
    if (!exact && ps.wide) {
        pa.shadow16 = nullptr;
        hipLaunchKernelGGL((k_prune_wide<2, 32>), dim3(nblocks), dim3(2 * kWave), prune_wide_lds_bytes(idx->dim, 2), s, pa);
        HIPCHECK(idx, hipGetLastError());
        return MI355DR_OK;
    }
    if (pa.cap > kCandCap) return fail(idx, MI355DR_E_INTERNAL, "general-form prune on a list stride above kCandCap");
    const bool list_mode = qlist == nullptr;
    pa.skip_list = list_mode ? idx->prune_skip : nullptr;
    pa.skip_parity = list_mode ? (idx->prune_parity ^= 1) : 0;
    hipLaunchKernelGGL((k_prune<kPruneSmallThreads, kPruneSmallSort>), dim3(nblocks), dim3(kPruneSmallThreads),
                       prune_lds_bytes(idx->dim, kPruneSmallThreads, kPruneSmallSort, pa.shadow16 ? idx->dpad : 0), s, pa);
    HIPCHECK(idx, hipGetLastError());
    if (one_wave_only) return MI355DR_OK;
    hipLaunchKernelGGL((k_prune<kPruneBigThreads, kPruneBigSort>), dim3(list_mode ? std::min(nblocks, 64) : nblocks),
                       dim3(kPruneBigThreads), prune_lds_bytes(idx->dim, kPruneBigThreads, kPruneBigSort, 0), s, pa);
    HIPCHECK(idx, hipGetLastError());
    return MI355DR_OK;
}

int launch_prep(mi355dr_index* idx, hipStream_t s, int B, int Bpad, int metric, bool i8, int cnt0 = 0) {
    hipLaunchKernelGGL(k_prep_queries, dim3(Bpad), dim3(64), (size_t)idx->dim * sizeof(float), s, idx->qdev, B, idx->dim,
                       idx->dpad, metric, idx->st, idx->dpad8, i8 ? 1 : 0, idx->bf16_ec, idx->status_or_dev,
                       idx->prune_skip, cnt0, idx->metric == MI355DR_METRIC_IP ? idx->cmax : 1.0f);
    idx->prune_parity = 0;
    HIPCHECK(idx, hipGetLastError());
    return MI355DR_OK;
}

inline int screen_tile(int B) { return B > kTileN ? kT2 : kTileM; }

constexpr int kRetryLevels = 2;

enum ScreenKernel { kKernTile = 0, kKernStream = 1, kKern256c = 2, kKernRq = 3 };
inline ScreenKernel screen_kernel_for(const mi355dr_index* idx, bool i8, int B, int64_t rows, bool emit_all) {
    const int tile = (emit_all || rows <= idx->small_chunk_rows) ? kTileM : screen_tile(B);
    const int row_bytes = i8 ? idx->dpad8 : idx->dpad * 2;
    const int ksteps = row_bytes / kRowB;
    if (tile == kT2) return i8 && idx->screen_rq && screen_rq_has(ksteps) ? kKernRq : kKern256c;
    if (!emit_all && idx->screen_stream && B <= 64 && ksteps >= 1 && (B <= 32 ? 32 : 64) * row_bytes <= kStreamQueryBytesMax)
        return kKernStream;
    return kKernTile;
}

int launch_screen(mi355dr_index* idx, hipStream_t s, bool i8, int B, int64_t r0, int64_t r_end, int cap, int emit_mode,
                  int flush_mask) {
    const bool emit_all = emit_mode != 0;
    const ScreenKernel kern = screen_kernel_for(idx, i8, B, r_end - r0, emit_all);
    const int tile = kern == kKern256c || kern == kKernRq ? kT2 : kTileM;
    ScreenArgs2 sa{};
    sa.status = idx->st.status;
    sa.shadow = i8 ? (const void*)idx->shadow8 : (const void*)idx->shadow;
    sa.qhat = i8 ? (const void*)idx->st.qhat8 : (const void*)idx->st.qhat;
    sa.thr = idx->st.thr;
    sa.sc = idx->st.sc;
    sa.kq = idx->st.kq;
    sa.grp = idx->grp8;
    sa.flag8 = idx->flag8;
    sa.cnt = idx->st.cnt;
    sa.cand_row = idx->cand_row;
    sa.cand_val = idx->cand_val;
    sa.row_bytes = i8 ? idx->dpad8 : idx->dpad * 2;
    sa.ksteps = sa.row_bytes / kRowB;
    sa.cap = cap;
    sa.ct0 = (int)(r0 / tile);
    sa.n_ctiles = (int)(round_up(r_end, tile) / tile) - sa.ct0;
    sa.n_qtiles = (int)(round_up(B, tile) / tile);
    sa.row_end = r_end;
    sa.row0 = r0;
    sa.emit_all = emit_mode;
    const int64_t grid = round_up(sa.n_ctiles, 8) * sa.n_qtiles;
    switch (kern) {
    case kKernRq: {
        sa.ct0 = (int)(r0 / kRqRows);
        sa.n_ctiles = (int)(round_up(r_end, kRqRows) / kRqRows) - sa.ct0;
        const unsigned g2 = screen_rq_grid(sa.n_ctiles, sa.n_qtiles);
        idx->s_rq_launches++;
        if (idx->debug_park > 0 && r_end - r0 >= idx->debug_park) {
            if (!idx->park_thr) {
                std::vector<float> inf(kQBlockMax, INFINITY);
                HIPCHECK(idx, idx->park_thr.grow(kQBlockMax * sizeof(float)));
                HIPCHECK(idx, hipMemcpy(idx->park_thr, inf.data(), kQBlockMax * sizeof(float), hipMemcpyHostToDevice));
            }
            sa.thr = idx->park_thr;
        }
        sa.progress = idx->rq_progress;
        sa.epoch = idx->rq_epoch = idx->rq_epoch % 4095 + 1;
        if (sa.epoch == 1) HIPCHECK(idx, hipMemsetAsync(idx->rq_progress, 0, kRqProgressWords * sizeof(int), s));
        sa.drift = idx->screen_drift;
        sa.flush_mask = flush_mask;
        sa.flush_alone = idx->screen_flush_alone;
        if (sa.ksteps == 6 && !idx->screen_rq_split_tests) {
            hipLaunchKernelGGL((k_screen_rq<6, false, true>), dim3(g2), dim3(512), rq_lds(6), s, sa);
        } else {
            switch (sa.ksteps) {
#define MI355_RQ_LAUNCH(KS) \
    case KS: hipLaunchKernelGGL((k_screen_rq<KS, true, true>), dim3(g2), dim3(512), rq_lds(KS), s, sa); break;
                MI355_RQ_FORMS(MI355_RQ_LAUNCH)
#undef MI355_RQ_LAUNCH
            }
        }
        break;
    }
    case kKern256c: {
        const unsigned g2 = screen256_grid(sa.n_ctiles, sa.n_qtiles);
        if (i8) hipLaunchKernelGGL((k_screen256c<true>), dim3(g2), dim3(512), kScreen256Lds, s, sa);
        else hipLaunchKernelGGL((k_screen256c<false>), dim3(g2), dim3(512), kScreen256Lds, s, sa);
        break;
    }
    case kKernStream: {
        const int nq = B <= 32 ? 32 : 64;
        const unsigned gs = (unsigned)std::min(sa.n_ctiles, 256);
        const size_t lds = screen_stream_lds(nq, sa.row_bytes);
        if (i8 && nq == 32) hipLaunchKernelGGL((k_screen_stream<true, 32>), dim3(gs), dim3(256), lds, s, (ScreenArgs)sa);
        else if (i8) hipLaunchKernelGGL((k_screen_stream<true, 64>), dim3(gs), dim3(256), lds, s, (ScreenArgs)sa);
        else if (nq == 32) hipLaunchKernelGGL((k_screen_stream<false, 32>), dim3(gs), dim3(256), lds, s, (ScreenArgs)sa);
        else hipLaunchKernelGGL((k_screen_stream<false, 64>), dim3(gs), dim3(256), lds, s, (ScreenArgs)sa);
        break;
    }
    case kKernTile:
        if (i8) hipLaunchKernelGGL(k_screen<true>, dim3((unsigned)grid), dim3(256), kScreenLds, s, (ScreenArgs)sa);
        else hipLaunchKernelGGL(k_screen<false>, dim3((unsigned)grid), dim3(256), kScreenLds, s, (ScreenArgs)sa);
        break;
    }
    HIPCHECK(idx, hipGetLastError());
    if (emit_mode == kEmitAll) {
        const int per_query = (int)(r_end - r0);
        hipLaunchKernelGGL(k_set_counts, dim3((B + 255) / 256), dim3(256), 0, s, idx->st.cnt, B, per_query);
        HIPCHECK(idx, hipGetLastError());
    }
    return MI355DR_OK;
}

constexpr int kStarterKMax = 32;
constexpr int64_t kStarterRows = 16384;
struct PassPlan {
    int64_t sample = 0;
    std::vector<int64_t> ends;
    bool emit_all_first = false;
};
PassPlan plan_pass(const mi355dr_index* idx, const Pass& ps, int B, double growth) {
    PassPlan p;
    const int64_t n = idx->n;
    const int k = ps.k, cap = ps.cap;
    const bool wide = ps.wide;
    const int tile = screen_tile(B);
    int64_t seen = 0;
    const int64_t starter_rows = std::min<int64_t>(wide ? idx->starter_rows_wide : kStarterRows, n / 4) / kTileM * kTileM;
    const int64_t starter_slabs = (starter_rows + kSlabRows - 1) / kSlabRows;
    if (idx->starter && (k <= kStarterKMax || wide) && ps.level == 0 && idx->chunk0_set == 0 && n >= 4 * 1024 &&
        starter_slabs <= cap && starter_slabs >= k) {
        p.sample = starter_rows;
        seen = p.sample;
    } else {
        const int64_t c0 = std::min<int64_t>(n, round_up(std::max<int64_t>(tile, std::min<int64_t>(idx->chunk0_rows, cap)), tile));
        p.emit_all_first = c0 <= cap;
        p.ends.push_back(c0);
        seen = c0;
        if (c0 >= n) return p;
    }
    const double rmax = 1.0 + growth;
    const double span = (double)n / (double)seen;
    int steps = std::max(1, (int)std::ceil(std::log(span) / std::log(rmax) - 0.15));
    const double r = std::pow(span, 1.0 / steps);
    double taper = std::max(1.0, (idx->chunk_taper_x100 > 0 ? idx->chunk_taper_x100 : (wide ? 120 : 100)) / 100.0);
    if (steps > 1 && taper > 1.0) {
        const double room = std::max(1.0, rmax * 1.25 / r);
        taper = std::min(taper, std::pow(room, 2.0 / (steps - 1)));
    } else {
        taper = 1.0;
    }
    double pos = (double)seen;
    int64_t prev = p.sample > 0 ? 0 : seen;
    for (int i = 1; i <= steps; ++i) {
        pos *= r * std::pow(taper, (steps - 1) / 2.0 - (i - 1));
        int64_t end = i == steps ? n : std::min<int64_t>(n, round_up((int64_t)pos, tile));
        if (tile == kT2 && end < n) {
            const int n_qtiles = (int)(round_up(B, kT2) / kT2);
            const int64_t round_rows = (int64_t)8 * (32 / n_qtiles) * kT2;
            const int64_t len = end - prev;
            if (len >= 2 * round_rows) end = std::min<int64_t>(n, prev + (len + round_rows / 2) / round_rows * round_rows);
        }
        if (end <= prev) continue;
        p.ends.push_back(end);
        prev = end;
        if (end >= n) break;
    }
    if (p.ends.empty() || p.ends.back() < n) p.ends.push_back(n);
    return p;
}

inline int starter_count(const PassPlan& p) { return (int)((p.sample + kSlabRows - 1) / kSlabRows); }

PassPlan make_plan(const mi355dr_index* idx, const Pass& ps, int B) {
    const double budget = growth_budget(idx, ps.k, ps.i8);
    double growth = std::max(0.25, std::min((double)idx->chunk_growth, budget));
    if (B <= 64 && ps.level == 0 && idx->chunk_growth_set == 0) growth = std::max(growth, std::min(8.0, budget * kSmallBlockBudget));
    if (ps.level == 1) growth = std::max(0.25, growth * 0.5);
    if (ps.level >= 2) growth = 0.25;
    return plan_pass(idx, ps, B, growth);
}

int run_screen(mi355dr_index* idx, hipStream_t s, const Pass& ps, int B, const PassPlan& plan) {
    int64_t kept_all_below = 0;
    const bool i8 = ps.i8;
    const int side_n = i8 ? idx->irr8_n : idx->irr_n;
    constexpr int kSideMerge = 32;
    bool side_done = false;
    const bool lean = plan.sample > 0 && idx->prune_companion == 0;
    auto timed = [&](bool big, int64_t rows, auto&& launch) -> int {
        EventPair ev{};
        if (idx->profile) {
            ev = take_events(idx);
            HIPCHECK(idx, hipEventRecord(ev.a, s));
        }
        CHECK(launch());
        if (idx->profile) {
            HIPCHECK(idx, hipEventRecord(ev.b, s));
            ev.big = big ? 1 : 0;
            idx->ev_pending.v.push_back(ev);
        }
        idx->s_screen_launches++;
        idx->s_screen_rows += rows;
        if (big) {
            idx->s_big_launches++;
            idx->s_big_rows += rows;
        }
        return MI355DR_OK;
    };
    if (plan.sample > 0) {
        CHECK(timed(false, plan.sample, [&] { return launch_screen(idx, s, i8, B, 0, plan.sample, ps.cap, kEmitSlabMax, -1); }));
        CHECK(launch_prune(idx, s, ps, B, nullptr, 0, true, true));
        idx->s_starters++;
    }
    int64_t done = 0;
    for (size_t ci = 0; ci < plan.ends.size(); ++ci) {
        const int64_t end = plan.ends[ci];
        const bool emit_all = ci == 0 && plan.emit_all_first;
        if (emit_all) kept_all_below = end;
        const bool big = !emit_all && end - done > idx->small_chunk_rows && screen_tile(B) == kT2;
        const int64_t seen = ci == 0 ? (plan.sample > 0 ? plan.sample : end) : done;
        const double lanes = 8.0 * ps.k * 4096.0 / (double)std::max<int64_t>(seen, 1);
        int period = 1;
        while (period < 64 && period * 2 * lanes <= idx->screen_flush_lanes) period *= 2;
        const int flush_mask = idx->screen_flush_sync ? period - 1 : -1;
        CHECK(timed(big, end - done, [&] { return launch_screen(idx, s, i8, B, done, end, ps.cap, emit_all ? kEmitAll : 0, flush_mask); }));
        idx->s_chunks++;
        if (end >= idx->n && side_n > 0 && side_n <= kSideMerge) {
            hipLaunchKernelGGL(k_emit_irregular, dim3(B), dim3(64), 0, s, i8 ? idx->irr8_rows : idx->irr_rows, side_n, idx->st,
                               idx->cand_row, idx->cand_val, ps.cap, (int)kept_all_below);
            HIPCHECK(idx, hipGetLastError());
            side_done = true;
        }
        const bool last = end >= idx->n && (side_n == 0 || side_done);
        CHECK(launch_prune(idx, s, ps, B, nullptr, 0, false, lean, !last));
        done = end;
    }
    if (side_n > 0 && !side_done) {
        hipLaunchKernelGGL(k_emit_irregular, dim3(B), dim3(64), 0, s, i8 ? idx->irr8_rows : idx->irr_rows, side_n, idx->st,
                           idx->cand_row, idx->cand_val, ps.cap, (int)kept_all_below);
        HIPCHECK(idx, hipGetLastError());
        CHECK(launch_prune(idx, s, ps, B, nullptr, 0, false, lean));
    }
    idx->s_passes++;
    return MI355DR_OK;
}

int launch_scan(mi355dr_index* idx, hipStream_t s, const int* qlist, int nq, int cap, int64_t r0, int64_t r1,
                const int32_t* ids = nullptr) {
    ScanArgs sa{};
    sa.rows = idx->rows;
    sa.nrm2 = idx->nrm2;
    sa.q = idx->qdev;
    sa.st = idx->st;
    sa.cand_row = idx->cand_row;
    sa.cand_val = idx->cand_val;
    sa.qlist = qlist;
    sa.nq = nq;
    sa.cap = cap;
    sa.d = idx->dim;
    sa.metric = idx->metric;
    sa.row0 = r0;
    sa.row1 = r1;
    const dim3 grid((unsigned)((r1 - r0 + kScanThreads - 1) / kScanThreads));
    const ScanIdsArgs ia{sa, ids};
    if (ids) hipLaunchKernelGGL(k_scan_ids, grid, dim3(kScanThreads), scan_ids_lds_bytes(idx->dim, nq), s, ia);
    else if (idx->dim % kScan32PieceCols == 0 && idx->scan_dma)
        hipLaunchKernelGGL(k_scan32, grid, dim3(kScanThreads), kScan32Lds, s, sa, idx->n);
    else hipLaunchKernelGGL(k_scan, grid, dim3(kScanThreads), scan_lds_bytes(idx->dim, nq), s, sa);
    HIPCHECK(idx, hipGetLastError());
    return MI355DR_OK;
}

int scan_range(mi355dr_index* idx, hipStream_t s, const Pass& ps, int off, int nq, int64_t r0, int64_t r1, const int32_t* ids) {
    CHECK(launch_scan(idx, s, idx->qlist_dev + off, nq, ps.cap, r0, r1, ids));
    return launch_prune(idx, s, ps, nq, idx->qlist_dev + off, 1);
}

int run_scan(mi355dr_index* idx, hipStream_t s, const Pass& ps, const std::vector<int>& qs, int64_t total,
             const int32_t* ids = nullptr) {
    if (qs.empty()) return MI355DR_OK;
    HIPCHECK(idx, hipMemcpyAsync(idx->qlist_dev, qs.data(), qs.size() * sizeof(int), hipMemcpyHostToDevice, s));
    const int nq_all = (int)qs.size(), cap = ps.cap;
    hipLaunchKernelGGL(k_reset_queries, dim3((nq_all + 255) / 256), dim3(256), 0, s, idx->st, idx->qlist_dev, nq_all);
    HIPCHECK(idx, hipGetLastError());
    const int per = kScanQ;
    for (int off = 0; off < nq_all; off += per) {
        const int nq = std::min(per, nq_all - off);
        int64_t done = 0;
        int64_t chunk = std::min<int64_t>(idx->chunk0_rows, cap);
        while (done < total) {
            const int64_t end = std::min<int64_t>(total, done + chunk);
            CHECK(scan_range(idx, s, ps, off, nq, done, end, ids));
            if (end - done > cap) {
                HIPCHECK(idx, hipMemcpyAsync(idx->status_host, idx->st.status, kQBlockMax * sizeof(int),
                                             hipMemcpyDeviceToHost, s));
                HIPCHECK(idx, hipStreamSynchronize(s));
                std::vector<int> redo;
                for (int j = 0; j < nq; ++j)
                    if (idx->status_host[qs[off + j]] & kStOverflow) redo.push_back(qs[off + j]);
                if (!redo.empty()) {
                    const int roff = kQBlockMax;
                    HIPCHECK(idx, hipMemcpyAsync(idx->qlist_dev + roff, redo.data(), redo.size() * sizeof(int),
                                                 hipMemcpyHostToDevice, s));
                    for (int q : redo) idx->status_host[q] &= ~kStOverflow;
                    for (int q : redo)
                        HIPCHECK(idx, hipMemcpyAsync(idx->st.status + q, idx->status_host + q, sizeof(int),
                                                     hipMemcpyHostToDevice, s));
                    for (int64_t p = done; p < end; p += cap)
                        CHECK(scan_range(idx, s, ps, roff, (int)redo.size(), p, std::min<int64_t>(end, p + cap), ids));
                    if (ids) {
                        HIPCHECK(idx, hipStreamSynchronize(s));
                        idx->s_subset_rerun_queries += (int64_t)redo.size();
                    }
                }
            }
            done = end;
            chunk = std::max<int64_t>(chunk, done * (idx->chunk_growth_set ? idx->chunk_growth : 63));
        }
    }
    if (ids) HIPCHECK(idx, hipStreamSynchronize(s));
    else idx->s_fallback_queries += nq_all;
    return MI355DR_OK;
}

int subset_block(mi355dr_index* idx, hipStream_t s, const float* q_dev, int B, int k, int64_t m, double* out_dist_dev,
                 int64_t* out_rows_dev) {
    const Pass ps = decide_pass(idx, k, 0, true);
    idx->last_pass_k = k;
    if (q_dev != idx->qdev)
        HIPCHECK(idx, hipMemcpyAsync(idx->qdev, q_dev, (size_t)B * idx->dim * sizeof(float), hipMemcpyDeviceToDevice, s));
    CHECK(launch_prep(idx, s, B, (int)round_up(B, screen_tile(B)), idx->metric, ps.i8));
    std::vector<int> all(B);
    for (int i = 0; i < B; ++i) all[i] = i;
    if (m > 0) CHECK(run_scan(idx, s, ps, all, m, idx->subset_ids));
    hipLaunchKernelGGL(k_finalize, dim3(B), dim3(64), 0, s, idx->st, k, idx->row_offset, idx->view_row_map.p, out_dist_dev,
                       out_rows_dev, idx->status_or_dev);
    HIPCHECK(idx, hipGetLastError());
    HIPCHECK(idx, hipMemcpyAsync(idx->status_host, idx->st.status, (size_t)kQBlockMax * sizeof(int), hipMemcpyDeviceToHost, s));
    HIPCHECK(idx, hipStreamSynchronize(s));
    for (int i = 0; i < B; ++i)
        if (idx->status_host[i] & kStOverflow)
            return fail(idx, MI355DR_E_INTERNAL, "subset scan: query " + std::to_string(i) + " lost a candidate chunk");
    return MI355DR_OK;
}

int pending_alloc(mi355dr_index* idx, Pending& p) {
    HIPCHECK(idx, p.status_host.grow((kQBlockMax + 1) * sizeof(int)));
    HIPCHECK(idx, p.done.create(hipEventDisableTiming));
    return MI355DR_OK;
}

int enqueue_block(mi355dr_index* idx, hipStream_t s, const float* q_dev, int B, int k, double* out_dist_dev,
                  int64_t* out_rows_dev, Pending& p, int level = 0, bool force_scan = false) {
    CHECK(ensure_qstate(idx));
    CHECK(pending_alloc(idx, p));
    idx->last_pass_k = k;
    if (level == 0 && idx->screen_dtype == MI355DR_SCREEN_AUTO && k >= idx->i8_demoted_k && --idx->i8_probation <= 0)
        idx->i8_demoted_k = INT_MAX;
    const int Bpad = (int)round_up(B, screen_tile(B));
    const Pass ps = decide_pass(idx, k, level, force_scan, "screen path unavailable (metric or too many irregular rows)");
    if (ps.refused) return fail(idx, MI355DR_E_UNSUPPORTED, ps.refused);
    if (q_dev != idx->qdev)
        HIPCHECK(idx, hipMemcpyAsync(idx->qdev, q_dev, (size_t)B * idx->dim * sizeof(float), hipMemcpyDeviceToDevice, s));
    PassPlan plan;
    if (ps.screening) plan = make_plan(idx, ps, B);
    CHECK(launch_prep(idx, s, B, Bpad, idx->metric, ps.i8, starter_count(plan)));
    if (idx->n > 0) {
        if (ps.screening) {
            CHECK(run_screen(idx, s, ps, B, plan));
        } else {
            std::vector<int> all(B);
            for (int i = 0; i < B; ++i) all[i] = i;
            CHECK(run_scan(idx, s, ps, all, idx->n));
        }
    }
    hipLaunchKernelGGL(k_finalize, dim3(B), dim3(64), 0, s, idx->st, k, idx->row_offset, idx->view_row_map.p, out_dist_dev,
                       out_rows_dev, idx->status_or_dev);
    HIPCHECK(idx, hipGetLastError());
    HIPCHECK(idx, hipMemcpyAsync(p.status_host, idx->st.status, (size_t)(kQBlockMax + 1) * sizeof(int), hipMemcpyDeviceToHost, s));
    HIPCHECK(idx, hipEventRecord(p.done, s));
    p.active = true;
    p.stream = s;
    p.q_dev = q_dev;
    p.B = B;
    p.pass = ps;
    p.out_dist = out_dist_dev;
    p.out_rows = out_rows_dev;
    return MI355DR_OK;
}

int search_block(mi355dr_index* idx, hipStream_t s, const float* q_dev, int B, int k, double* out_dist_dev,
                 int64_t* out_rows_dev, int level = 0, bool force_scan = false);

int complete_block(mi355dr_index* idx, Pending& p) {
    if (!p.active) return MI355DR_OK;
    p.active = false;
    HIPCHECK(idx, hipEventSynchronize(p.done));
    drain_events(idx);
    if (!p.pass.screening) {
        for (int i = 0; i < p.B; ++i)
            if (p.status_host[i] & kStOverflow)
                return fail(idx, MI355DR_E_INTERNAL, "exact scan: query " + std::to_string(i) + " lost a candidate chunk");
        return MI355DR_OK;
    }
    if (p.status_host[kQBlockMax] == 0) return MI355DR_OK;
    hipStream_t s = p.stream;
    const int B = p.B, k = p.pass.k, level = p.pass.level;
    std::vector<int> sub;
    int n_todo = 0;
    {
        std::vector<int> retry;
        for (int i = 0; i < B; ++i) {
            const int st = p.status_host[i];
            if (st == 0) continue;
            if (level < kRetryLevels && !(st & kStIrregular)) retry.push_back(i);
            else sub.push_back(i);
        }
        n_todo = (int)sub.size();
        sub.insert(sub.end(), retry.begin(), retry.end());
    }
    const int n_sub = (int)sub.size(), n_retry = n_sub - n_todo;
    if (n_sub == 0) return MI355DR_OK;
    RetryBufs& rb = idx->retry[level];
    HIPCHECK(idx, rb.q.grow((size_t)kQBlockMax * idx->dim * sizeof(float)));
    HIPCHECK(idx, rb.dist.grow((size_t)kQBlockMax * kKMax * sizeof(double)));
    HIPCHECK(idx, rb.rows.grow((size_t)kQBlockMax * kKMax * sizeof(int64_t)));
    HIPCHECK(idx, rb.map.grow((size_t)kQBlockMax * sizeof(int)));
    HIPCHECK(idx, hipMemcpyAsync(rb.map, sub.data(), n_sub * sizeof(int), hipMemcpyHostToDevice, s));
    hipLaunchKernelGGL(k_gather_queries, dim3(n_sub), dim3(128), 0, s, p.q_dev, rb.map, idx->dim, rb.q);
    HIPCHECK(idx, hipGetLastError());
    HIPCHECK(idx, hipStreamSynchronize(s));
    if (n_todo > 0) CHECK(search_block(idx, s, rb.q, n_todo, k, rb.dist, rb.rows, level + 1, true));
    if (n_retry > 0) {
        idx->s_retry_queries += n_retry;
        if (p.pass.i8 && idx->screen_dtype == MI355DR_SCREEN_AUTO && n_retry * 100 > B) {
            idx->i8_demoted_k = std::min(idx->i8_demoted_k, k);
            idx->i8_backoff = idx->i8_backoff == 0 ? 16 : std::min(idx->i8_backoff * 2, 4096);
            idx->i8_probation = idx->i8_backoff;
        }
        CHECK(search_block(idx, s, rb.q + (size_t)n_todo * idx->dim, n_retry, k, rb.dist + (size_t)n_todo * k,
                           rb.rows + (size_t)n_todo * k, level + 1));
    }
    hipLaunchKernelGGL(k_scatter_results, dim3(n_sub), dim3(128), 0, s, rb.dist, rb.rows, rb.map, k, p.out_dist, p.out_rows);
    HIPCHECK(idx, hipGetLastError());
    HIPCHECK(idx, hipStreamSynchronize(s));
    return MI355DR_OK;
}

int complete_until(mi355dr_index* idx, int64_t seq) {
    int rc = MI355DR_OK;
    while (idx->seq_done < seq) {
        const int r = complete_block(idx, idx->pend[idx->seq_done % kPendingRing]);
        if (rc == MI355DR_OK) rc = r;
        idx->seq_done++;
    }
    return rc;
}
int drain_pending(mi355dr_index* idx) { return complete_until(idx, idx->seq_next); }

int search_block(mi355dr_index* idx, hipStream_t s, const float* q_dev, int B, int k, double* out_dist_dev,
                 int64_t* out_rows_dev, int level, bool force_scan) {
    Pending& p = idx->sub_pend[std::min(level, kRetryLevels + 1)];
    CHECK(enqueue_block(idx, s, q_dev, B, k, out_dist_dev, out_rows_dev, p, level, force_scan));
    return complete_block(idx, p);
}

inline size_t merge_lds(int world, int k) {
    size_t np = 1;
    while (np < (size_t)world * k) np <<= 1;
    return np * 12;
}
inline int merge_threads(int world, int k) { return (int64_t)world * k <= 128 ? 64 : 256; }

int launch_merge(mi355dr_index* idx, const double* dist_all, const int64_t* rows_all, int64_t stride, int world, int B, int k,
                 double* out_dist_dev, int64_t* out_rows_dev, void* stream) {
    if (world <= 0 || B < 0 || k <= 0) return fail(idx, MI355DR_E_INVALID, "bad merge shape");
    if ((int64_t)world * k > kSortMax) return fail(idx, MI355DR_E_UNSUPPORTED, "world*k exceeds 4096");
    if (B == 0) return MI355DR_OK;
    HIPCHECK(idx, hipSetDevice(idx->device));
    CHECK(ensure_qstate(idx));
    hipStream_t s = stream ? (hipStream_t)stream : idx->stream;
    hipLaunchKernelGGL(k_merge_topk, dim3(B), dim3(merge_threads(world, k)), merge_lds(world, k), s, dist_all, rows_all, stride,
                       world, B, k, out_dist_dev, out_rows_dev);
    HIPCHECK(idx, hipGetLastError());
    return MI355DR_OK;
}

int upload_and_prep(mi355dr_index* idx, const float* queries, int B, int metric) {
    HIPCHECK(idx, hipSetDevice(idx->device));
    CHECK(drain_pending(idx));
    CHECK(ensure_qstate(idx));
    HIPCHECK(idx, hipMemcpyAsync(idx->qdev, queries, (size_t)B * idx->dim * sizeof(float), hipMemcpyHostToDevice, idx->stream));
    return launch_prep(idx, idx->stream, B, (int)round_up(B, screen_tile(B)), metric, idle_i8(idx));
}

int check_search_args(mi355dr_index* idx, const void* q, int B, int k, const void* od, const void* orow) {
    if (!idx) return fail(nullptr, MI355DR_E_INVALID, "null index");
    if (B < 0 || k <= 0) return fail(idx, MI355DR_E_INVALID, "B must be >= 0 and k > 0");
    if (k > kKMax) return fail(idx, MI355DR_E_UNSUPPORTED, "k exceeds 1024");
    if (B > 0 && (!q || !od || !orow)) return fail(idx, MI355DR_E_INVALID, "null buffer");
    return MI355DR_OK;
}

int check_radii(mi355dr_index* idx, const std::string& what, const double* radius, int B) {
    for (int b = 0; b < B; ++b)
        if (radius[b] != radius[b]) return fail(idx, MI355DR_E_INVALID, what + ": radius " + std::to_string(b) + " is NaN");
    return MI355DR_OK;
}

enum : unsigned { kCallNoView = 1, kCallDrain = 2 };
struct Call {
    std::unique_lock<std::mutex> lock;
    hipStream_t s = nullptr;
};
template <class ArgCheck>
int begin_call(mi355dr_index* idx, const char* what, void* stream, unsigned flags, Call& c, ArgCheck&& args_ok) {
    if (!idx) return fail(nullptr, MI355DR_E_INVALID, "null index");
    if ((flags & kCallNoView) && idx->is_view) return view_refuses(idx, what, true);
    CHECK(args_ok());
    c.lock = std::unique_lock<std::mutex>(idx->mu);
    HIPCHECK(idx, hipSetDevice(idx->device));
    if (flags & kCallDrain) CHECK(drain_pending(idx));
    c.s = stream ? (hipStream_t)stream : idx->stream;
    return ensure_qstate(idx);
}

template <class Count>
struct BlockOut {
    double* dist;
    int64_t* rows;
    Count* count;
};
template <class Count = int64_t>
struct CallIO {
    bool host;
    hipStream_t s;
    const float* q;
    BlockOut<Count> out;
    int width;
};

template <class Count>
int block_queries(mi355dr_index* idx, const CallIO<Count>& io, int b0, int nb, const float** q_dev) {
    *q_dev = io.q + (int64_t)b0 * idx->dim;
    if (!io.host) return MI355DR_OK;
    HIPCHECK(idx, hipMemcpyAsync(idx->qdev, *q_dev, (size_t)nb * idx->dim * sizeof(float), hipMemcpyHostToDevice, io.s));
    *q_dev = idx->qdev;
    return MI355DR_OK;
}

BlockOut<int64_t> block_outputs(mi355dr_index* idx, const CallIO<>& io, int b0) {
    if (io.host) return {idx->out_dist_dev, idx->out_rows_dev, io.out.count ? idx->out_count_dev.p : nullptr};
    return {io.out.dist + (int64_t)b0 * io.width, io.out.rows + (int64_t)b0 * io.width, io.out.count ? io.out.count + b0 : nullptr};
}

template <class Count>
int block_return(mi355dr_index* idx, const CallIO<Count>& io, int b0, int nb, const BlockOut<Count>& o) {
    if (!io.host) return MI355DR_OK;
    const size_t n = (size_t)nb * io.width;
    HIPCHECK(idx, hipMemcpyAsync(io.out.dist + (int64_t)b0 * io.width, o.dist, n * sizeof(double), hipMemcpyDeviceToHost, io.s));
    HIPCHECK(idx, hipMemcpyAsync(io.out.rows + (int64_t)b0 * io.width, o.rows, n * sizeof(int64_t), hipMemcpyDeviceToHost, io.s));
    if (o.count) HIPCHECK(idx, hipMemcpyAsync(io.out.count + b0, o.count, (size_t)nb * sizeof(Count), hipMemcpyDeviceToHost, io.s));
    return MI355DR_OK;
}

int launch_rescore(mi355dr_index* idx, hipStream_t s, const int32_t* pair_q_dev, const int64_t* pair_row_dev, int64_t n_pairs,
                   float* dot_dev, double* dist_dev) {
    hipLaunchKernelGGL(k_rescore_pairs, dim3((unsigned)((n_pairs + kWave - 1) / kWave)), dim3(kWave), 0, s, idx->rows, idx->nrm2,
                       idx->qdev, idx->st.qn, pair_q_dev, pair_row_dev, n_pairs, idx->dim, idx->metric, dot_dev, dist_dev);
    HIPCHECK(idx, hipGetLastError());
    return MI355DR_OK;
}

struct PairBufs {
    DevBuf<int32_t> q;
    DevBuf<int64_t> row;
    DevBuf<float> dot;
    DevBuf<double> dist;
};
int rescore_host_pairs(mi355dr_index* idx, PairBufs& bufs, const float* queries, int B, const int32_t* pair_q,
                       const int64_t* pair_row, int64_t n_pairs, float* out_dot, double* out_dist) {
    hipStream_t s = idx->stream;
    CHECK(upload_and_prep(idx, queries, B, idx->metric));
    HIPCHECK(idx, grow_each(n_pairs, bufs.q, bufs.row, bufs.dot, bufs.dist));
    HIPCHECK(idx, hipMemcpyAsync(bufs.q.p, pair_q, n_pairs * sizeof(int32_t), hipMemcpyHostToDevice, s));
    HIPCHECK(idx, hipMemcpyAsync(bufs.row.p, pair_row, n_pairs * sizeof(int64_t), hipMemcpyHostToDevice, s));
    CHECK(launch_rescore(idx, s, bufs.q.p, bufs.row.p, n_pairs, bufs.dot.p, bufs.dist.p));
    if (out_dot) HIPCHECK(idx, hipMemcpyAsync(out_dot, bufs.dot.p, n_pairs * sizeof(float), hipMemcpyDeviceToHost, s));
// ... 153 lines not shown

int mi355dr_add_rows(mi355dr_index* idx, const float* rows, int64_t n) {
    return add_rows_impl(idx, rows, n, hipMemcpyHostToDevice);
}
int mi355dr_add_rows_device(mi355dr_index* idx, const float* rows_dev, int64_t n) {
    return add_rows_impl(idx, rows_dev, n, hipMemcpyDeviceToDevice);
}

namespace {
constexpr int64_t kMutSlice = (int64_t)1 << 16;

int mutate_rows_impl(mi355dr_index* idx, const int64_t* row_ids, const float* rows, int64_t n, hipMemcpyKind kind, bool remove) {
    if (!idx) return fail(nullptr, MI355DR_E_INVALID, "null index");
    std::lock_guard<std::mutex> g(idx->mu);
    if (idx->is_view) return view_refuses(idx, remove ? "remove_rows" : "update_rows");
    if (n < 0) return fail(idx, MI355DR_E_INVALID, "negative row count");
    if (n == 0) {
        HIPCHECK(idx, hipSetDevice(idx->device));
        return drain_pending(idx);
    }
    if (!row_ids || (!remove && !rows)) return fail(idx, MI355DR_E_INVALID, "null argument");
    std::vector<int64_t> sorted(row_ids, row_ids + n);
    std::sort(sorted.begin(), sorted.end());
    if (sorted.front() < 0 || sorted.back() >= idx->n) return fail(idx, MI355DR_E_INVALID, "row id out of range");
    for (int64_t i = 1; i < n; ++i)
        if (sorted[i] == sorted[i - 1]) return fail(idx, MI355DR_E_INVALID, "duplicated row id " + std::to_string(sorted[i]));
    std::vector<int64_t> groups;
    for (int64_t r : sorted)
        if (groups.empty() || groups.back() != r / kI8GroupRows) groups.push_back(r / kI8GroupRows);
    HIPCHECK(idx, hipSetDevice(idx->device));
    CHECK(drain_pending(idx));
    hipStream_t s = idx->stream;
    DevBuf<void> ids_dev, groups_dev, stage;
    HIPCHECK(idx, ids_dev.grow((size_t)n * sizeof(int64_t)));
    HIPCHECK(idx, groups_dev.grow(groups.size() * sizeof(int64_t)));
    HIPCHECK(idx, hipMemcpyAsync(ids_dev.p, row_ids, (size_t)n * sizeof(int64_t), hipMemcpyHostToDevice, s));
    HIPCHECK(idx, hipMemcpyAsync(groups_dev.p, groups.data(), groups.size() * sizeof(int64_t), hipMemcpyHostToDevice, s));
    if (!remove && kind == hipMemcpyHostToDevice)
        HIPCHECK(idx, stage.grow((size_t)std::min(n, kMutSlice) * idx->dim * sizeof(float)));
    for (int64_t r0 = 0; r0 < n; r0 += kMutSlice) {
        const int64_t m = std::min(kMutSlice, n - r0);
        const int64_t* ids = (const int64_t*)ids_dev.p + r0;
        if (remove) {
            hipLaunchKernelGGL(k_mark_dead, dim3((unsigned)((m + 255) / 256)), dim3(256), 0, s, ids, m, idx->nrm2);
            HIPCHECK(idx, hipGetLastError());
        } else {
            const float* src = rows + r0 * idx->dim;
            if (stage.p) {
                HIPCHECK(idx, hipMemcpyAsync(stage.p, src, (size_t)m * idx->dim * sizeof(float), hipMemcpyHostToDevice, s));
                src = (const float*)stage.p;
            }
            const int vec4 = idx->dim % 4 == 0 && (uintptr_t)src % 16 == 0;
            hipLaunchKernelGGL(k_update_rows, dim3((unsigned)m), dim3(256), 0, s, src, ids, m, idx->dim, vec4, idx->rows);
            HIPCHECK(idx, hipGetLastError());
        }
        CHECK(build_rows(idx, s, 0, m, ids, !remove));
    }
    CHECK(build_groups(idx, s, 0, (int64_t)groups.size(), (const int64_t*)groups_dev.p, idx->n, idx->n));
    HIPCHECK(idx, hipMemsetAsync(idx->irr_count, 0, sizeof(int), s));
    HIPCHECK(idx, hipMemsetAsync(idx->irr8_count, 0, sizeof(int), s));
    HIPCHECK(idx, hipMemsetAsync(idx->dead_count, 0, sizeof(int), s));
    hipLaunchKernelGGL(k_rebuild_side_lists, dim3((unsigned)((idx->n + 255) / 256)), dim3(256), 0, s, idx->nrm2, idx->flag8,
                       (int64_t)0, idx->n, idx->irr_rows, idx->irr_count, idx->irr8_rows, idx->irr8_count, idx->dead_count);
    HIPCHECK(idx, hipGetLastError());
    return commit_corpus(idx, s, true);
}
}

int mi355dr_update_rows(mi355dr_index* idx, const int64_t* row_ids, const float* rows, int64_t n) {
    return mutate_rows_impl(idx, row_ids, rows, n, hipMemcpyHostToDevice, false);
}
int mi355dr_update_rows_device(mi355dr_index* idx, const int64_t* row_ids, const float* rows_dev, int64_t n) {
    return mutate_rows_impl(idx, row_ids, rows_dev, n, hipMemcpyDeviceToDevice, false);
}
int mi355dr_remove_rows(mi355dr_index* idx, const int64_t* row_ids, int64_t n) {
    return mutate_rows_impl(idx, row_ids, nullptr, n, hipMemcpyHostToDevice, true);
}

int mi355dr_compact(mi355dr_index* idx, int64_t* new_of_old) {
    if (!idx) return fail(nullptr, MI355DR_E_INVALID, "null index");
    std::lock_guard<std::mutex> g(idx->mu);
    if (idx->is_view) return view_refuses(idx, "compact");
    HIPCHECK(idx, hipSetDevice(idx->device));
    CHECK(drain_pending(idx));
    const int64_t n_old = idx->n;
    if (idx->dead_n == 0) {
        if (new_of_old)
            for (int64_t r = 0; r < n_old; ++r) new_of_old[r] = r;
        return MI355DR_OK;
    }
    hipStream_t s = idx->stream;
    std::vector<float> n2;
    std::vector<int32_t> src_of_dst;
    int64_t first_dead = n_old;
    try {
        n2.resize((size_t)n_old);
        HIPCHECK(idx, hipMemcpyAsync(n2.data(), idx->nrm2, (size_t)n_old * sizeof(float), hipMemcpyDeviceToHost, s));
        HIPCHECK(idx, hipStreamSynchronize(s));
        for (int64_t r = 0; r < n_old; ++r)
            if (row_is_dead(n2[(size_t)r])) {
                first_dead = r;
                break;
            }
        src_of_dst.reserve((size_t)(n_old - first_dead));
        for (int64_t r = first_dead; r < n_old; ++r)
            if (!row_is_dead(n2[(size_t)r])) src_of_dst.push_back((int32_t)r);
    } catch (const std::bad_alloc&) {
        return fail(idx, MI355DR_E_NOMEM, "compact: out of host memory for the row maps");
    }
    const int64_t n_moved = (int64_t)src_of_dst.size(), n_new = first_dead + n_moved;
    const int64_t slice = std::min(idx->compact_slice_rows, n_moved);
    const size_t row_b = (size_t)idx->dim * sizeof(float);
    DevBuf<int32_t> map_dev;
    DevBuf<float> stage;
    if (n_moved > 0) {
        HIPCHECK(idx, map_dev.grow((size_t)n_moved * sizeof(int32_t)));
        HIPCHECK(idx, stage.grow((size_t)slice * (row_b + sizeof(float))));
        HIPCHECK(idx, hipMemcpyAsync(map_dev.p, src_of_dst.data(), (size_t)n_moved * sizeof(int32_t), hipMemcpyHostToDevice, s));
    }
    float* stage_n2 = stage.p + slice * idx->dim;
    const int vec4 = idx->dim % 4 == 0 && (uintptr_t)idx->rows.p % 16 == 0 && (uintptr_t)stage.p % 16 == 0;
    for (int64_t j0 = 0; j0 < n_moved; j0 += slice) {
        const int64_t m = std::min(slice, n_moved - j0), dst0 = first_dead + j0;
        hipLaunchKernelGGL(k_compact_gather, dim3((unsigned)((m + kCompactWaves - 1) / kCompactWaves)), dim3(64 * kCompactWaves),
                           0, s, idx->rows, idx->nrm2, map_dev.p + j0, m, idx->dim, vec4, stage.p, stage_n2);
        HIPCHECK(idx, hipGetLastError());
        HIPCHECK(idx, hipMemcpyAsync(idx->rows + dst0 * idx->dim, stage.p, (size_t)m * row_b, hipMemcpyDeviceToDevice, s));
        HIPCHECK(idx, hipMemcpyAsync(idx->nrm2 + dst0, stage_n2, (size_t)m * sizeof(float), hipMemcpyDeviceToDevice, s));
    }
    const int64_t tail_end = std::min(round_up(n_old, kT2), idx->cap_rows), tail = tail_end - n_new;
    const int64_t g_tail = (n_new + kI8GroupRows - 1) / kI8GroupRows, g_end = tail_end / kI8GroupRows;
    if (tail > 0) {
        HIPCHECK(idx, hipMemsetAsync(idx->nrm2 + n_new, 0, (size_t)tail * sizeof(float), s));
        HIPCHECK(idx, hipMemsetAsync(idx->shadow + n_new * idx->dpad, 0, (size_t)tail * idx->dpad * sizeof(uint16_t), s));
        HIPCHECK(idx, hipMemsetAsync(idx->shadow8 + n_new * idx->dpad8, 0, (size_t)tail * idx->dpad8, s));
        HIPCHECK(idx, hipMemsetAsync(idx->flag8 + n_new, 0, (size_t)tail, s));
    }
    if (g_end > g_tail) HIPCHECK(idx, hipMemsetAsync(idx->grp8 + g_tail, 0, (size_t)(g_end - g_tail) * sizeof(I8Group), s));
    CHECK(build_rows(idx, s, first_dead, n_moved, nullptr, false));
    const int64_t g_lo = first_dead / kI8GroupRows;
    CHECK(build_groups(idx, s, g_lo, g_tail - g_lo, nullptr, n_new, n_new));
    HIPCHECK(idx, hipMemsetAsync(idx->irr_count, 0, sizeof(int), s));
    HIPCHECK(idx, hipMemsetAsync(idx->irr8_count, 0, sizeof(int), s));
    HIPCHECK(idx, hipMemsetAsync(idx->dead_count, 0, sizeof(int), s));
    if (n_new > 0) {
        hipLaunchKernelGGL(k_rebuild_side_lists, dim3((unsigned)((n_new + 255) / 256)), dim3(256), 0, s, idx->nrm2, idx->flag8,
                           (int64_t)0, n_new, idx->irr_rows, idx->irr_count, idx->irr8_rows, idx->irr8_count, idx->dead_count);
        HIPCHECK(idx, hipGetLastError());
    }
    CHECK(commit_corpus(idx, s, true));
    idx->n = n_new;
    idx->i8_demoted_k = INT_MAX;
    idx->i8_backoff = idx->i8_probation = 0;
    idx->s_compactions += n_moved > 0;
    idx->s_compact_moved_rows += n_moved;
    if (new_of_old) {
        int64_t next = 0;
        for (int64_t r = 0; r < n_old; ++r) new_of_old[r] = row_is_dead(n2[(size_t)r]) ? -1 : next++;
    }
    return MI355DR_OK;
}

namespace {
#define VIEWCHECK(parent, view, expr)                                                         \
    do {                                                                                      \
        int rc__ = (expr);                                                                    \
        if (rc__ != MI355DR_OK) return fail(parent, rc__, "view_create: " + (view)->err);     \
    } while (0)

int view_local_ids(mi355dr_index* parent, const int64_t* ids, int64_t m, int64_t n, std::vector<int32_t>& out) {
    try {
        subset_prepare_ids(ids, m, parent->row_offset, n, out);
    } catch (const std::bad_alloc&) {
        return fail(parent, MI355DR_E_NOMEM, "view_create: out of host memory for the id list");
    }
    return MI355DR_OK;
}

int view_upload_map(mi355dr_index* parent, const std::vector<int32_t>& local, DevBuf<int64_t>& map) {
    if (local.empty()) return MI355DR_OK;
    std::vector<int64_t> global;
    try {
        global.resize(local.size());
    } catch (const std::bad_alloc&) {
        return fail(parent, MI355DR_E_NOMEM, "view_create: out of host memory for the id map");
    }
    for (size_t j = 0; j < local.size(); ++j) global[j] = (int64_t)local[j] + parent->row_offset;
    HIPCHECK(parent, map.grow(global.size() * sizeof(int64_t)));
    HIPCHECK(parent, hipMemcpy(map.p, global.data(), global.size() * sizeof(int64_t), hipMemcpyHostToDevice));
    return MI355DR_OK;
}

int view_build(mi355dr_index* parent, mi355dr_index* view, const int64_t* row_ids, int64_t m_rows, const int64_t* doc_ids,
               int64_t m_docs) {
    hipStream_t s = parent->stream;
    const int d = parent->dim;
    const size_t row_b = (size_t)d * sizeof(float);
    const int64_t slice = parent->view_slice_rows;
    std::vector<int32_t> rows, docs;
    CHECK(view_local_ids(parent, row_ids, m_rows, parent->n, rows));
    DevBuf<int32_t> ids_dev;
    if (!rows.empty()) {
        HIPCHECK(parent, ids_dev.grow(rows.size() * sizeof(int32_t)));
        HIPCHECK(parent, hipMemcpyAsync(ids_dev.p, rows.data(), rows.size() * sizeof(int32_t), hipMemcpyHostToDevice, s));
        HIPCHECK(parent, hipStreamSynchronize(s));
    }
    if (!rows.empty() && parent->dead_n > 0) {
        const int64_t m = (int64_t)rows.size();
        DevBuf<float> n2_dev;
        std::vector<float> n2;
        try {
            n2.resize((size_t)m);
        } catch (const std::bad_alloc&) {
            return fail(parent, MI355DR_E_NOMEM, "view_create: out of host memory for the listed rows' norms");
        }
        HIPCHECK(parent, n2_dev.grow((size_t)m * sizeof(float)));
        hipLaunchKernelGGL(k_view_gather_nrm2, dim3((unsigned)((m + 255) / 256)), dim3(256), 0, s, parent->nrm2.p, ids_dev.p, m, n2_dev.p);
        HIPCHECK(parent, hipGetLastError());
        HIPCHECK(parent, hipMemcpyAsync(n2.data(), n2_dev.p, (size_t)m * sizeof(float), hipMemcpyDeviceToHost, s));
        HIPCHECK(parent, hipStreamSynchronize(s));
        int64_t keep = 0;
        for (int64_t j = 0; j < m; ++j)
            if (!row_is_dead(n2[(size_t)j])) rows[(size_t)keep++] = rows[(size_t)j];
        if (keep < m) {
            rows.resize((size_t)keep);
            if (keep > 0) {
                HIPCHECK(parent, hipMemcpyAsync(ids_dev.p, rows.data(), (size_t)keep * sizeof(int32_t), hipMemcpyHostToDevice, s));
                HIPCHECK(parent, hipStreamSynchronize(s));
            }
        }
    }
    MultiVecView pv{};
    if (m_docs > 0 && multivec_view(parent, &pv)) {
        CHECK(view_local_ids(parent, doc_ids, m_docs, pv.n_docs, docs));
        docs.erase(std::remove_if(docs.begin(), docs.end(), [&](int32_t i) { return pv.tok_cnt_host[i] <= 0; }), docs.end());
    }
    const int64_t n_rows = (int64_t)rows.size(), n_docs = (int64_t)docs.size();
    int64_t tok_total = 0, tok_longest = 0, blk_total = 0;
    for (int32_t i : docs) {
        const int64_t T = pv.tok_cnt_host[i];
        tok_total += T;
        tok_longest = std::max(tok_longest, T);
        blk_total += (T + kMsBlkRows - 1) / kMsBlkRows;
    }
    const int64_t stage_rows = std::max(std::min(slice, n_rows), std::max(std::min(slice, tok_total), tok_longest));
    DevBuf<float> stage;
    if (stage_rows > 0) HIPCHECK(parent, stage.grow((size_t)stage_rows * row_b));
    if (n_rows > 0) {
        VIEWCHECK(parent, view, mi355dr_reserve(view, n_rows));
        const int vec4 = d % 4 == 0 && (uintptr_t)parent->rows.p % 16 == 0 && (uintptr_t)stage.p % 16 == 0;
        for (int64_t j0 = 0; j0 < n_rows; j0 += slice) {
            const int64_t m = std::min(slice, n_rows - j0);
            hipLaunchKernelGGL(k_view_gather_rows, dim3((unsigned)((m + kViewWaves - 1) / kViewWaves)), dim3(64 * kViewWaves), 0, s,
                               parent->rows.p, ids_dev.p + j0, m, d, vec4, stage.p);
            HIPCHECK(parent, hipGetLastError());
            HIPCHECK(parent, hipStreamSynchronize(s));
            VIEWCHECK(parent, view, mi355dr_add_rows_device(view, stage.p, m));
        }
        CHECK(view_upload_map(parent, rows, view->view_row_map));
    }
    if (n_docs > 0) {
        VIEWCHECK(parent, view, multivec_reserve(view, blk_total, n_docs));
        std::vector<ViewTokBlock> blocks;
        std::vector<int64_t> offsets;
        DevBuf<ViewTokBlock> blocks_dev;
        for (int64_t i0 = 0, i1; i0 < n_docs; i0 = i1) {
            blocks.clear();
            offsets.assign(1, 0);
            try {
                for (i1 = i0; i1 < n_docs && (i1 == i0 || offsets.back() + pv.tok_cnt_host[docs[(size_t)i1]] <= slice); ++i1) {
                    const int64_t T = pv.tok_cnt_host[docs[(size_t)i1]], blk0 = pv.blk_off_host[docs[(size_t)i1]];
                    for (int64_t t = 0; t < T; t += kMsBlkRows)
                        blocks.push_back(ViewTokBlock{blk0 + t / kMsBlkRows, offsets.back() + t, (int32_t)std::min<int64_t>(kMsBlkRows, T - t), 0});
                    offsets.push_back(offsets.back() + T);
                }
            } catch (const std::bad_alloc&) {
                return fail(parent, MI355DR_E_NOMEM, "view_create: out of host memory for a slice's block table");
            }
            HIPCHECK(parent, blocks_dev.grow(blocks.size() * sizeof(ViewTokBlock)));
            HIPCHECK(parent, hipMemcpyAsync(blocks_dev.p, blocks.data(), blocks.size() * sizeof(ViewTokBlock), hipMemcpyHostToDevice, s));
            hipLaunchKernelGGL(k_view_gather_toks, dim3((unsigned)blocks.size()), dim3(64 * kViewWaves), 0, s, pv.tok, blocks_dev.p, d,
                               pv.dpad, stage.p);
            HIPCHECK(parent, hipGetLastError());
            HIPCHECK(parent, hipStreamSynchronize(s));
            VIEWCHECK(parent, view, mi355dr_add_multivec_device(view, stage.p, offsets.data(), i1 - i0));
        }
        CHECK(view_upload_map(parent, docs, view->view_doc_map));
    }
    view->view_rows = n_rows;
    view->view_docs = n_docs;
    return MI355DR_OK;
}
}

int mi355dr_view_create(mi355dr_index* parent, const int64_t* row_ids, int64_t m_rows, const int64_t* doc_ids, int64_t m_docs,
                        mi355dr_index** out_view) {
    if (out_view) *out_view = nullptr;
    if (!parent) return fail(nullptr, MI355DR_E_INVALID, "null index");
    if (!out_view) return fail(parent, MI355DR_E_INVALID, "view_create: out_view is null");
    if (m_rows < 0 || m_docs < 0 || (m_rows > 0 && !row_ids) || (m_docs > 0 && !doc_ids))
        return fail(parent, MI355DR_E_INVALID, "view_create: counts must be >= 0 and a list with a count not null");
    std::lock_guard<std::mutex> g(parent->mu);
    if (parent->is_view) return view_refuses(parent, "view_create", true);
    HIPCHECK(parent, hipSetDevice(parent->device));
    CHECK(drain_pending(parent));
    mi355dr_index* view = nullptr;
// ... 975 lines not shown
    const CallIO<> io{true, s, nullptr, {out_dist, out_rows, nullptr}, k};
    std::vector<int32_t> pq;
    std::vector<int64_t> pr, first, ordered_rows, mine, all;
    std::vector<double> got, ordered_dist;
    std::vector<MmrCand> list;
    PairBufs bufs;
    for (int b0 = 0; b0 < B && m > 0; b0 += kQBlockMax) {
        const int nb = std::min(kQBlockMax, B - b0);
        const size_t plane = (size_t)nb * m;
        try {
            pr.clear();
            first.assign(1, 0);
            for (int b = 0; b < nb; ++b) {
                mmr_unique_rows(cand_rows + (int64_t)(b0 + b) * m, m, idx->row_offset, idx->n, pr);
                first.push_back((int64_t)pr.size());
            }
            pq.resize(pr.size());
            for (int b = 0; b < nb; ++b) std::fill(pq.begin() + first[b], pq.begin() + first[b + 1], b);
            got.resize(pr.size());
            mine.assign(2 * plane, -1);
            all.resize(2 * plane * world);
            ordered_dist.assign(plane, (double)NAN);
            ordered_rows.assign(plane, -1);
        } catch (const std::bad_alloc&) {
            return fail(idx, MI355DR_E_NOMEM, "mmr_select_sharded: out of host memory for the candidate lists");
        }
        CHECK(shard_reserve_words(idx, 2 * plane));
        const int64_t n_pairs = (int64_t)pr.size();
        if (n_pairs > 0)
            CHECK(rescore_host_pairs(idx, bufs, queries + (int64_t)b0 * idx->dim, nb, pq.data(), pr.data(), n_pairs, nullptr, got.data()));
        for (int b = 0; b < nb; ++b)
            for (int64_t i = first[b]; i < first[b + 1]; ++i) {
                const size_t at = (size_t)b * m + (size_t)(i - first[b]);
                mine[at] = pr[i] + idx->row_offset;
                memcpy(&mine[plane + at], &got[i], sizeof(double));
            }
        HIPCHECK(idx, hipMemcpyAsync(idx->shd.send.p, mine.data(), 2 * plane * sizeof(int64_t), hipMemcpyHostToDevice, s));
        CHECK(shard_gather(idx, s, idx->shd.send.p, idx->shd.recv.p, 2 * plane * sizeof(int64_t)));
        HIPCHECK(idx, hipMemcpyAsync(all.data(), idx->shd.recv.p, 2 * plane * world * sizeof(int64_t), hipMemcpyDeviceToHost, s));
        HIPCHECK(idx, hipStreamSynchronize(s));
        try {
            for (int b = 0; b < nb; ++b) {
                list.clear();
                for (int r = 0; r < world; ++r) {
                    const int64_t* rr = all.data() + (size_t)r * 2 * plane + (size_t)b * m;
                    for (int j = 0; j < m && (int)list.size() < m; ++j) {
                        if (rr[j] < 0) continue;
                        double dist;
                        memcpy(&dist, rr + plane + j, sizeof(double));
                        list.push_back(MmrCand{dist, rr[j]});
                    }
                }
                mmr_order(list.data(), (int64_t)list.size());
                for (size_t j = 0; j < list.size(); ++j) {
                    ordered_dist[(size_t)b * m + j] = list[j].dist;
                    ordered_rows[(size_t)b * m + j] = list[j].row;
                }
            }
        } catch (const std::bad_alloc&) {
            return fail(idx, MI355DR_E_NOMEM, "mmr_select_sharded: out of host memory for the candidate lists");
        }
        HIPCHECK(idx, hipMemcpyAsync(idx->mmr.cand_dist.p, ordered_dist.data(), plane * sizeof(double), hipMemcpyHostToDevice, s));
        HIPCHECK(idx, hipMemcpyAsync(idx->mmr.cand_rows.p, ordered_rows.data(), plane * sizeof(int64_t), hipMemcpyHostToDevice, s));
        const BlockOut<int64_t> o = block_outputs(idx, io, b0);
        CHECK(shard_mmr_block(idx, s, nb, m, k, lambda, o.dist, o.rows));
        CHECK(block_return(idx, io, b0, nb, o));
        HIPCHECK(idx, hipStreamSynchronize(s));
    }
    HIPCHECK(idx, hipStreamSynchronize(s));
    return shard_mmr_finish(idx, B);
}

int mi355dr_merge_topk_device(mi355dr_index* idx, const double* dist_all_dev, const int64_t* rows_all_dev, int world,
                              int B, int k, double* out_dist_dev, int64_t* out_rows_dev, void* stream) {
    if (!idx) return fail(nullptr, MI355DR_E_INVALID, "null index");
    std::lock_guard<std::mutex> g(idx->mu);
    return launch_merge(idx, dist_all_dev, rows_all_dev, (int64_t)B * k, world, B, k, out_dist_dev, out_rows_dev, stream);
}

int mi355dr_pack_topk_device(mi355dr_index* idx, const double* dist_dev, const int64_t* rows_dev, int B, int k,
                             int64_t* packed_dev, void* stream) {
    if (!idx || !dist_dev || !rows_dev || !packed_dev) return fail(idx, MI355DR_E_INVALID, "null argument");
    std::lock_guard<std::mutex> g(idx->mu);
    if (B < 0 || k <= 0) return fail(idx, MI355DR_E_INVALID, "bad shape");
    HIPCHECK(idx, hipSetDevice(idx->device));
    hipStream_t s = stream ? (hipStream_t)stream : idx->stream;
    const size_t bytes = (size_t)B * k * 8;
    if (bytes) {
        HIPCHECK(idx, hipMemcpyAsync(packed_dev, dist_dev, bytes, hipMemcpyDeviceToDevice, s));
        HIPCHECK(idx, hipMemcpyAsync(packed_dev + (size_t)B * k, rows_dev, bytes, hipMemcpyDeviceToDevice, s));
    }
    return MI355DR_OK;
}

int mi355dr_merge_topk_packed_device(mi355dr_index* idx, const int64_t* packed_all_dev, int world, int B, int k,
                                     double* out_dist_dev, int64_t* out_rows_dev, void* stream) {
    if (!idx) return fail(nullptr, MI355DR_E_INVALID, "null index");
    std::lock_guard<std::mutex> g(idx->mu);
    const int64_t plane = (int64_t)B * k;
    return launch_merge(idx, (const double*)packed_all_dev, packed_all_dev + plane, 2 * plane, world, B, k, out_dist_dev, out_rows_dev, stream);
}

namespace {
using Index = mi355dr_index;

struct Field {
    int Index::*i = nullptr;
    int64_t Index::*l = nullptr;
    double Index::*x100 = nullptr;
    bool is_switch = false;
    constexpr Field(int Index::*p, bool is_switch = false) : i(p), is_switch(is_switch) {}
    constexpr Field(int64_t Index::*p) : l(p) {}
    constexpr Field(double Index::*p) : x100(p) {}
    void set(Index* idx, int64_t v) const {
        if (i) idx->*i = is_switch ? v != 0 : (int)v;
        else if (l) idx->*l = v;
        else idx->*x100 = (double)v / 100.0;
    }
};
constexpr bool kSwitch = true;

struct Option {
    const char* key;
    Field field;
    int64_t lo = INT64_MIN, hi = INT64_MAX;
    void (*then)(Index*) = nullptr;
    int64_t gap_lo = 0, gap_hi = 0;
};
const Option kOptions[] = {
    {"path", &Index::path, 0, 2},
    {"screen_dtype", &Index::screen_dtype, 0, 2, [](Index* x) {
         x->i8_demoted_k = INT_MAX;
         x->i8_backoff = x->i8_probation = 0;
     }},
    {"i8_min_budget_x100", &Index::i8_min_budget, 1, 1000},
    {"maxsim_screen", {&Index::maxsim_screen, kSwitch}},
    {"maxsim_coop", &Index::maxsim_coop, -1, 1},
    {"maxsim_persistent", {&Index::maxsim_persistent, kSwitch}},
    {"maxsim_wg", &Index::maxsim_wg, -1, 2},
    {"maxsim_tighten", {&Index::maxsim_tighten, kSwitch}},
    {"maxsim_aligned", {&Index::maxsim_aligned, kSwitch}},
    {"maxsim_wg_min", &Index::maxsim_wg_min, 8, 9},
    {"maxsim_wg_pipe", {&Index::maxsim_wg_pipe, kSwitch}},
    {"maxsim_pack8", &Index::maxsim_pack8, -1, 1},
    {"maxsim_wg_bps", &Index::maxsim_wg_bps, 2, 4, nullptr, 2, 4},
    {"maxsim_pass_groups", &Index::maxsim_pass_groups, 1, 4},
    {"maxsim_subset_screen", &Index::maxsim_subset_screen, -1, 1},
    {"maxsim_subset_screen_min", &Index::maxsim_subset_screen_min, 0},
    {"row_offset", &Index::row_offset},
    {"profile", {&Index::profile, kSwitch}},
    {"chunk0_rows", &Index::chunk0_rows, 1, INT64_MAX, [](Index* x) { x->chunk0_set = 1; }},
    {"starter", {&Index::starter, kSwitch}},
    {"prune_companion", {&Index::prune_companion, kSwitch}},
    {"scan_dma", {&Index::scan_dma, kSwitch}},
    {"defer_round_b", {&Index::defer_round_b, kSwitch}},
    {"chunk_growth", &Index::chunk_growth, 1, INT64_MAX, [](Index* x) { x->chunk_growth_set = 1; }},
    {"screen_stream", {&Index::screen_stream, kSwitch}},
    {"screen_rq", {&Index::screen_rq, kSwitch}},
    {"debug_park_thresholds", &Index::debug_park},
    {"screen_rq_split_tests", {&Index::screen_rq_split_tests, kSwitch}},
    {"screen_drift", &Index::screen_drift, 0, 1024},
    {"small_chunk_rows", &Index::small_chunk_rows, 0},
    {"round_a", &Index::round_a, 0, 64},
    {"prefilter16", {&Index::prefilter16, kSwitch}},
    {"cand_cap", &Index::cap, 16, kCandCap, [](Index* x) { x->cap_set = 1; }},
    {"prune_wide", {&Index::prune_wide, kSwitch}},
    {"screen_flush_sync", {&Index::screen_flush_sync, kSwitch}},
    {"screen_flush_lanes", &Index::screen_flush_lanes, 1, 64},
    {"screen_flush_alone", &Index::screen_flush_alone, 8, 60},
    {"wide_inflation_x10", &Index::wide_inflation_x10, 20, 400},
    {"chunk_taper_x100", &Index::chunk_taper_x100, 0, 300, nullptr, 0, 100},
    {"starter_rows_wide", &Index::starter_rows_wide, 4096, 262144},
    {"compact_slice_rows", &Index::compact_slice_rows, 32, (int64_t)1 << 22},
    {"view_slice_rows", &Index::view_slice_rows, 32, (int64_t)1 << 22},
    {"range_chunk_rows", &Index::range_chunk_rows, 256, (int64_t)1 << 31},
    {"range_slots", &Index::range_slots, 16, kSortMax},
    {"sparse_tile_docs", &Index::sparse_tile_docs, 256, 8192},
    {"sparse_cand_cap", &Index::sparse_cand_cap, 16, 2048},
    {"shard_stage_bytes", &Index::shard_stage_bytes, 1},
};

struct Stat {
    const char* key;
    int64_t Index::*counter;
    bool reset;
    int64_t (*value)(const Index*) = nullptr;
};
const Stat kStats[] = {
    {"screen_launches", &Index::s_screen_launches, true},
    {"screen_ns", &Index::s_screen_ns, true},
    {"screen_rows", &Index::s_screen_rows, true},
    {"screen256_launches", &Index::s_big_launches, true},
    {"screen_rq_launches", &Index::s_rq_launches, true},
    {"screen256_ns", &Index::s_big_ns, true},
    {"screen256_rows", &Index::s_big_rows, true},
    {"fallback_queries", &Index::s_fallback_queries, true},
    {"chunks", &Index::s_chunks, true},
    {"passes", &Index::s_passes, true},
    {"starters", &Index::s_starters, true},
    {"retry_queries", &Index::s_retry_queries, true},
    {"maxsim_screened", &Index::s_ms_screened, true},
    {"maxsim_candidates", &Index::s_ms_candidates, true},
    {"maxsim_fallbacks", &Index::s_ms_fallbacks, true},
    {"maxsim_screen_ns", &Index::s_ms_screen_ns, true},
    {"maxsim_pack_ns", &Index::s_ms_pack_ns, true},
    {"maxsim_screen_launches", &Index::s_ms_screen_launches, true},
    {"maxsim_exact_ns", &Index::s_ms_exact_ns, true},
    {"maxsim_exact_launches", &Index::s_ms_exact_launches, true},
    {"maxsim_screen_cols", &Index::s_ms_screen_cols, true},
    {"maxsim_packed_launches", &Index::s_ms_packed_launches, true},
    {"maxsim_packed_blocks", &Index::s_ms_packed_blocks, false},
    {"maxsim_packed_built", &Index::s_ms_packed_built, false},
    {"maxsim_set_docs", &Index::s_ms_set_docs, true},
    {"maxsim_moved_blocks", &Index::s_ms_moved_blocks, true},
    {"subset_searches", &Index::s_subset_searches, true},
    {"subset_rows_scored", &Index::s_subset_rows_scored, true},
    {"subset_rerun_queries", &Index::s_subset_rerun_queries, true},
    {"maxsim_subset_searches", &Index::s_mss_searches, true},
    {"maxsim_subset_docs", &Index::s_mss_docs, true},
    {"maxsim_subset_screened", &Index::s_mss_screened, true},
    {"maxsim_subset_exact", &Index::s_mss_exact, true},
    {"maxsim_subset_fallbacks", &Index::s_mss_fallbacks, true},
    {"mmr_searches", &Index::s_mmr_searches, true},
    {"mmr_queries", &Index::s_mmr_queries, true},
    {"mmr_pairs_scored", &Index::s_mmr_pairs, true},
    {"group_searches", &Index::s_group_searches, true},
    {"group_subqueries", &Index::s_group_subqueries, true},
    {"groups_merged", &Index::s_groups_merged, true},
    {"range_searches", &Index::s_range_searches, true},
    {"range_queries", &Index::s_range_queries, true},
    {"range_in_range", &Index::s_range_in_range, true},
    {"range_candidates", &Index::s_range_candidates, true},
    {"range_rescored", &Index::s_range_rescored, true},
    {"range_redo_chunks", &Index::s_range_redo_chunks, true},
    {"range_fallback_queries", &Index::s_range_fallback_queries, true},
    {"rows_searches", &Index::s_rows_searches, true},
    {"rows_queries", &Index::s_rows_queries, true},
    {"rows_skipped", &Index::s_rows_skipped, true},
    {"sharded_range_searches", &Index::s_shard_range_searches, true},
    {"sharded_rows_searches", &Index::s_shard_rows_searches, true},
    {"sharded_mmr_searches", &Index::s_shard_mmr_searches, true},
    {"shard_gather_bytes", &Index::s_shard_gather_bytes, true},
    {"sparse_searches", &Index::s_sparse_searches, true},
    {"sparse_queries", &Index::s_sparse_queries, true},
    {"sparse_postings_scored", &Index::s_sparse_postings_scored, true},
    {"sparse_overflows", &Index::s_sparse_overflows, true},
    {"sparse_docs", nullptr, false, [](const Index* x) -> int64_t { return sparse_stat(x, kSparseStatDocs); }},
    {"sparse_total_len", nullptr, false, [](const Index* x) -> int64_t { return sparse_stat(x, kSparseStatTotalLen); }},
    {"sparse_postings", nullptr, false, [](const Index* x) -> int64_t { return sparse_stat(x, kSparseStatPostings); }},
    {"sparse_vocab", nullptr, false, [](const Index* x) -> int64_t { return sparse_stat(x, kSparseStatVocab); }},
    {"compactions", &Index::s_compactions, true},
    {"compact_moved_rows", &Index::s_compact_moved_rows, true},
    {"view", nullptr, false, [](const Index* x) -> int64_t { return x->is_view ? 1 : 0; }},
    {"view_rows", &Index::view_rows, false},
    {"view_docs", &Index::view_docs, false},
    {"i8_demoted", nullptr, false, [](const Index* x) -> int64_t { return x->i8_demoted_k != INT_MAX ? 1 : 0; }},
    {"i8_demoted_k", nullptr, false, [](const Index* x) -> int64_t { return x->i8_demoted_k == INT_MAX ? 0 : x->i8_demoted_k; }},
    {"irregular_rows", nullptr, false, [](const Index* x) -> int64_t { return x->irr_n; }},
    {"loose_rows", nullptr, false, [](const Index* x) -> int64_t { return x->irr8_n; }},
    {"dead_rows", nullptr, false, [](const Index* x) -> int64_t { return x->dead_n; }},
    {"screen_dtype_active", nullptr, false, [](const Index* x) -> int64_t { return idle_i8(x) ? MI355DR_SCREEN_I8 : MI355DR_SCREEN_BF16; }},
    {"hbm_bytes_resident", nullptr, false, [](const Index* x) -> int64_t {
         return x->cap_rows * ((int64_t)x->dim * 4 + (int64_t)x->dpad * 2 + (int64_t)x->dpad8 + 5) +
                x->cap_rows / kI8GroupRows * (int64_t)sizeof(I8Group) + multivec_bytes(x) +
                (int64_t)(x->view_row_map.bytes + x->view_doc_map.bytes) +
                sparse_bytes(x);
     }},
};
}

int mi355dr_set_option(mi355dr_index* idx, const char* key, int64_t value) {
    if (!idx || !key) return fail(idx, MI355DR_E_INVALID, "null argument");
    std::lock_guard<std::mutex> g(idx->mu);
    if (idx->seq_done < idx->seq_next) {
        HIPCHECK(idx, hipSetDevice(idx->device));
        CHECK(drain_pending(idx));
    }
    if (idx->is_view && strcmp(key, "row_offset") == 0) return view_refuses(idx, "option row_offset");
    for (const Option& o : kOptions) {
        if (strcmp(o.key, key) != 0) continue;
        if (value < o.lo || value > o.hi || (value > o.gap_lo && value < o.gap_hi)) {
            std::string range = o.hi == INT64_MAX ? " must be >= " + std::to_string(o.lo)
                                                  : " must be in [" + std::to_string(o.lo) + ", " + std::to_string(o.hi) + "]";
            if (o.gap_lo < o.gap_hi) range += ", not between " + std::to_string(o.gap_lo) + " and " + std::to_string(o.gap_hi);
            return fail(idx, MI355DR_E_INVALID, o.key + range);
        }
        if (strcmp(key, "sparse_tile_docs") == 0 && (value & (value - 1)) != 0)
            return fail(idx, MI355DR_E_INVALID, "sparse_tile_docs must be a power of two");
        o.field.set(idx, value);
        if (o.then) o.then(idx);
        return MI355DR_OK;
    }
    return fail(idx, MI355DR_E_INVALID, std::string("unknown option: ") + key);
}

int mi355dr_get_stat(mi355dr_index* idx, const char* key, int64_t* out) {
    if (!idx || !key || !out) return fail(idx, MI355DR_E_INVALID, "null argument");
    std::lock_guard<std::mutex> g(idx->mu);
    const std::string k(key);
    if (k == "candidates" || k == "rescored") {
        unsigned long long v[2] = {0, 0};
        if (idx->stat_dev) {
            std::vector<unsigned long long> per(2 * kQBlockMax);
            HIPCHECK(idx, hipSetDevice(idx->device));
            HIPCHECK(idx, hipMemcpy(per.data(), idx->stat_dev, per.size() * sizeof(unsigned long long), hipMemcpyDeviceToHost));
            for (int i = 0; i < kQBlockMax; ++i) {
                v[0] += per[2 * i];
                v[1] += per[2 * i + 1];
            }
        }
        *out = (int64_t)(k == "candidates" ? v[0] : v[1]);
        return MI355DR_OK;
    }
    for (const Stat& st : kStats) {
        if (k != st.key) continue;
        *out = st.counter ? idx->*st.counter : st.value(idx);
        return MI355DR_OK;
    }
    return fail(idx, MI355DR_E_INVALID, "unknown stat: " + k);
}

int mi355dr_reset_stats(mi355dr_index* idx) {
    if (!idx) return fail(nullptr, MI355DR_E_INVALID, "null index");
    std::lock_guard<std::mutex> g(idx->mu);
    for (const Stat& st : kStats)
        if (st.reset) idx->*st.counter = 0;
    if (idx->stat_dev) {
        HIPCHECK(idx, hipSetDevice(idx->device));
        HIPCHECK(idx, hipMemset(idx->stat_dev, 0, 2 * kQBlockMax * sizeof(unsigned long long)));
    }
    return MI355DR_OK;
}

int mi355dr_timer_start(mi355dr_index* idx) {
    if (!idx) return fail(nullptr, MI355DR_E_INVALID, "null index");
    HIPCHECK(idx, hipSetDevice(idx->device));
    HIPCHECK(idx, hipEventRecord(idx->t0, idx->stream));
    return MI355DR_OK;
}
int mi355dr_timer_stop(mi355dr_index* idx, double* elapsed_ms) {
    if (!idx || !elapsed_ms) return fail(idx, MI355DR_E_INVALID, "null argument");
    HIPCHECK(idx, hipSetDevice(idx->device));
    HIPCHECK(idx, hipEventRecord(idx->t1, idx->stream));
    HIPCHECK(idx, hipEventSynchronize(idx->t1));
    float ms = 0.f;
    HIPCHECK(idx, hipEventElapsedTime(&ms, idx->t0, idx->t1));
    *elapsed_ms = ms;
    return MI355DR_OK;
}
int mi355dr_synchronize(mi355dr_index* idx) {
    if (!idx) return fail(nullptr, MI355DR_E_INVALID, "null index");
    HIPCHECK(idx, hipSetDevice(idx->device));
    HIPCHECK(idx, hipStreamSynchronize(idx->stream));
    return MI355DR_OK;
}

int mi355dr_dev_alloc(mi355dr_index* idx, size_t bytes, void** out) {
    if (!idx || !out) return fail(idx, MI355DR_E_INVALID, "null argument");
    HIPCHECK(idx, hipSetDevice(idx->device));
    HIPCHECK(idx, hipMalloc(out, bytes ? bytes : 1));
    return MI355DR_OK;
}
int mi355dr_dev_free(mi355dr_index* idx, void* p) {
    if (!idx) return fail(nullptr, MI355DR_E_INVALID, "null index");
    HIPCHECK(idx, hipSetDevice(idx->device));
    if (p) HIPCHECK(idx, hipFree(p));
    return MI355DR_OK;
}
int mi355dr_dev_upload(mi355dr_index* idx, void* dst_dev, const void* src_host, size_t bytes) {
    if (!idx) return fail(nullptr, MI355DR_E_INVALID, "null index");
    HIPCHECK(idx, hipSetDevice(idx->device));
    HIPCHECK(idx, hipMemcpy(dst_dev, src_host, bytes, hipMemcpyHostToDevice));
    return MI355DR_OK;
}
int mi355dr_dev_download(mi355dr_index* idx, void* dst_host, const void* src_dev, size_t bytes) {
    if (!idx) return fail(nullptr, MI355DR_E_INVALID, "null index");
    HIPCHECK(idx, hipSetDevice(idx->device));
    HIPCHECK(idx, hipMemcpy(dst_host, src_dev, bytes, hipMemcpyDeviceToHost));
    return MI355DR_OK;
}

int mi355dr_debug_screen_dense(mi355dr_index* idx, const float* queries, int B, int64_t row0, int64_t n, float* out_t) {
    if (!idx || !queries || !out_t) return fail(idx, MI355DR_E_INVALID, "null argument");
    std::lock_guard<std::mutex> g(idx->mu);
    if (B <= 0 || B > kQBlockMax || n <= 0 || n > kCandCap || row0 < 0 || row0 % screen_tile(B) != 0 || row0 + n > idx->n)
        return fail(idx, MI355DR_E_INVALID,
                    "debug_screen_dense: need 1<=B<=1024, 1<=n<=2048, row0 a multiple of the tile (128; 256 if B>128)");
    CHECK(upload_and_prep(idx, queries, B, 2));
    hipStream_t s = idx->stream;
    const bool i8 = idle_i8(idx);
    CHECK(launch_screen(idx, s, i8, B, row0, row0 + n, kCandCap, 0, -1));
    std::vector<int> cnt(B);
    std::vector<int32_t> crow((size_t)B * kCandCap);
    std::vector<float> cval((size_t)B * kCandCap);
    HIPCHECK(idx, hipMemcpyAsync(cnt.data(), idx->st.cnt, B * sizeof(int), hipMemcpyDeviceToHost, s));
    HIPCHECK(idx, hipMemcpyAsync(crow.data(), idx->cand_row, crow.size() * sizeof(int32_t), hipMemcpyDeviceToHost, s));
    HIPCHECK(idx, hipMemcpyAsync(cval.data(), idx->cand_val, cval.size() * sizeof(float), hipMemcpyDeviceToHost, s));
    std::vector<uint8_t> flag(n, 0);
    if (i8) HIPCHECK(idx, hipMemcpyAsync(flag.data(), idx->flag8 + row0, n, hipMemcpyDeviceToHost, s));
    HIPCHECK(idx, hipStreamSynchronize(s));
    for (int64_t i = 0; i < (int64_t)B * n; ++i) out_t[i] = NAN;
    for (int b = 0; b < B; ++b) {
        const int c = std::min(cnt[b], kCandCap);
        for (int j = 0; j < c; ++j) {
            const int64_t r = crow[(size_t)b * kCandCap + j] - row0;
            if (r >= 0 && r < n && !flag[r]) out_t[(int64_t)b * n + r] = cval[(size_t)b * kCandCap + j];
        }
    }
    return MI355DR_OK;
}

int mi355dr_debug_screen_hits(mi355dr_index* idx, const float* queries, int B, int64_t row0, int64_t n, const float* thr,
                              int cap, int* out_count, int32_t* out_rows, float* out_vals, int* out_status, int* out_kernel) {
    if (!idx || !queries || !thr || !out_count || !out_rows || !out_vals || !out_status || !out_kernel)
        return fail(idx, MI355DR_E_INVALID, "null argument");
    std::lock_guard<std::mutex> g(idx->mu);
    if (B <= 0 || B > kQBlockMax || n <= 0 || row0 < 0 || row0 % screen_tile(B) != 0 || row0 + n > idx->n || cap < 16 ||
        cap > kCandCapWide)
        return fail(idx, MI355DR_E_INVALID,
                    "debug_screen_hits: need 1<=B<=1024, n>=1, row0 a multiple of the tile (128; 256 if B>128), 16<=cap<=4096");
    for (int b = 0; b < B; ++b)
        if (!(thr[b] < INFINITY))
            return fail(idx, MI355DR_E_INVALID, "debug_screen_hits: thresholds must be finite or -inf");
// ... 77 lines not shown
```

### autorag_research_amd/csrc/screen_common.h

```cpp
#pragma once
#include "dev_common.h"

namespace mi355 {

typedef __bf16 bf16x8 __attribute__((ext_vector_type(8)));
typedef float f32x16 __attribute__((ext_vector_type(16)));
typedef int i32x4 __attribute__((ext_vector_type(4)));
typedef int i32x16 __attribute__((ext_vector_type(16)));

constexpr int kTileM = 128;
constexpr int kTileN = 128;
constexpr int kStepK = 64;
constexpr int kRowB = 128;

struct ScreenArgs {
    const void* shadow;
    const void* qhat;
    const float* thr;
    const float* sc;
    const float* kq;
    const I8Group* grp;
    const uint8_t* flag8;
    int* cnt;
    int32_t* cand_row;
    float* cand_val;
    int row_bytes;
    int ksteps;
    int cap;
    int ct0;
    int n_ctiles;
    int n_qtiles;
    int64_t row_end;
    int64_t row0;
    int emit_all;
};
constexpr int kEmitAll = 1, kEmitSlabMax = 2;
constexpr int kSlabRows = 64;

__device__ __forceinline__ void glds16(const void* gsrc, void* lds_wave_base) {
    __builtin_amdgcn_global_load_lds((const __attribute__((address_space(1))) void*)gsrc,
                                     (__attribute__((address_space(3))) void*)lds_wave_base, 16, 0, 0);
}

template <bool I8>
__device__ __forceinline__ f32x16 screen_mfma(bf16x8 fa, bf16x8 fb, f32x16 acc) {
    if constexpr (I8) {
        return __builtin_bit_cast(f32x16, __builtin_amdgcn_mfma_i32_32x32x32_i8(__builtin_bit_cast(i32x4, fa),
                                                                                __builtin_bit_cast(i32x4, fb),
                                                                                __builtin_bit_cast(i32x16, acc), 0, 0, 0));
    } else {
        return __builtin_amdgcn_mfma_f32_32x32x16_bf16(fa, fb, acc, 0, 0, 0);
    }
}

struct I8Blk {
    float m, ek;
};
__device__ __forceinline__ I8Blk i8_blk(const I8Group g, float sq, float kq) { return I8Blk{g.step * sq, g.err * kq}; }
__device__ __forceinline__ float i8_value(int acc, const I8Blk& b) { return __builtin_fmaf((float)acc, b.m, b.ek); }
__device__ __forceinline__ I8Group i8_group_of(const I8Group* grp, int64_t row0) {
    typedef const __attribute__((address_space(4))) float cfloat;
    cfloat* p = (cfloat*)(const float*)(grp + (row0 >> 5));
    return I8Group{p[0], p[1]};
}

__device__ __forceinline__ unsigned lds_addr(const void* p) {
    return (unsigned)(unsigned long)((const __attribute__((address_space(3))) char*)p);
}

}
```

### autorag_research_amd/csrc/screen_hits.h

```cpp
#pragma once
#include "screen_common.h"

namespace mi355 {


template <bool I8>
__device__ __forceinline__ void screen_emit_block(const ScreenArgs& a, f32x16 acc, int q, int64_t rbase, float th,
                                                  I8Blk blk) {
    bool any;
    if constexpr (I8) {
        const i32x16 v = __builtin_bit_cast(i32x16, acc);
        int m = v[0];
#pragma unroll
        for (int r = 1; r < 16; ++r) m = max(m, v[r]);
        any = i8_value(m, blk) >= th;
    } else {
        float m = acc[0];
#pragma unroll
        for (int r = 1; r < 16; ++r) m = fmaxf(m, acc[r]);
        any = m >= th;
    }
    if (!any) return;
    unsigned mask = 0;
#pragma unroll
    for (int r = 0; r < 16; ++r) {
        const int64_t row = rbase + (r & 3) + 8 * (r >> 2);
        bool hit;
        if constexpr (I8) hit = i8_value(__builtin_bit_cast(i32x16, acc)[r], blk) >= th;
        else hit = acc[r] >= th;
        if (hit && row < a.row_end) mask |= 1u << r;
    }
    if (mask == 0) return;
    int slot = atomicAdd(&a.cnt[q], __builtin_popcount(mask));
#pragma unroll
    for (int r = 0; r < 16; ++r) {
        if ((mask >> r) & 1u) {
            if (slot < a.cap) {
                float val;
                if constexpr (I8) val = i8_value(__builtin_bit_cast(i32x16, acc)[r], blk);
                else val = acc[r];
                a.cand_row[(int64_t)q * a.cap + slot] = (int32_t)(rbase + (r & 3) + 8 * (r >> 2));
                a.cand_val[(int64_t)q * a.cap + slot] = val;
            }
            ++slot;
        }
    }
}

template <bool I8>
__device__ __forceinline__ void screen_emit_all_block(const ScreenArgs& a, f32x16 acc, int q, int64_t rbase, I8Blk blk) {
#pragma unroll
    for (int r = 0; r < 16; ++r) {
        const int64_t row = rbase + (r & 3) + 8 * (r >> 2);
        if (row < a.row_end) {
            float val;
            if constexpr (I8) {
                val = a.flag8[row] ? __builtin_nanf("") : i8_value(__builtin_bit_cast(i32x16, acc)[r], blk);
            } else {
                val = acc[r];
            }
            a.cand_row[(int64_t)q * a.cap + (row - a.row0)] = (int32_t)row;
            a.cand_val[(int64_t)q * a.cap + (row - a.row0)] = val;
        }
    }
}

template <bool I8>
__device__ __forceinline__ void screen_emit_slab_max(const ScreenArgs& a, const f32x16 (&acc)[2], int q, int64_t slab_row0,
                                                     int lane, const I8Blk (&blk)[2]) {
    float best = -__builtin_inff();
    int64_t best_row = slab_row0;
#pragma unroll
    for (int i = 0; i < 2; ++i) {
        const int64_t rbase = slab_row0 + 32 * i + 4 * (lane >> 5);
        int br = 0;
        float bv;
        if constexpr (I8) {
            const i32x16 v = __builtin_bit_cast(i32x16, acc[i]);
            int m = v[0];
#pragma unroll
            for (int r = 1; r < 16; ++r)
                if (v[r] > m) {
                    m = v[r];
                    br = r;
                }
            bv = i8_value(m, blk[i]);
        } else {
            float m = acc[i][0];
            if (!(m == m)) m = -__builtin_inff();
#pragma unroll
            for (int r = 1; r < 16; ++r)
                if (acc[i][r] > m) {
                    m = acc[i][r];
                    br = r;
                }
            bv = m;
        }
        const int64_t row = rbase + (br & 3) + 8 * (br >> 2);
        if (row < a.row_end && bv > best) {
            best = bv;
            best_row = row;
        }
    }
    const float ov = __shfl_xor(best, 32, kWave);
    const int orow = __shfl_xor((int)best_row, 32, kWave);
    if (ov > best || (ov == best && orow < (int)best_row)) {
        best = ov;
        best_row = orow;
    }
    if (lane < 32) {
        const int64_t slot = (slab_row0 - a.row0) / kSlabRows;
        a.cand_row[(int64_t)q * a.cap + slot] = (int32_t)best_row;
        a.cand_val[(int64_t)q * a.cap + slot] = best;
    }
}

constexpr int kWaveQueueCap = 320;

__device__ __forceinline__ void wave_queue_flush(const ScreenArgs& a, const int32_t* que, int n) {
    const int lane = threadIdx.x & 63;
    for (int e = lane; e < n; e += kWave) {
        const int q = que[e];
        const int slot = atomicAdd(&a.cnt[q], 1);
        if (slot < a.cap) {
            a.cand_row[(int64_t)q * a.cap + slot] = que[kWaveQueueCap + e];
            a.cand_val[(int64_t)q * a.cap + slot] = __int_as_float(que[2 * kWaveQueueCap + e]);
        }
    }
}

template <bool I8>
__device__ __forceinline__ int screen_queue_hits_body(f32x16 acc, int any_i, int q, int rbase, int row_end, float th,
                                                     float m, float ek, unsigned a_q, int que_n, int* status) {
    const bool any = any_i != 0;
    bool gany[4];
    int thi = 0;
    if constexpr (I8) {
        const i32x16 v = __builtin_bit_cast(i32x16, acc);
        thi = i8_block_threshold(th, m, ek);
#pragma unroll
        for (int i = 0; i < 4; ++i)
            gany[i] = any && max(max(v[4 * i], v[4 * i + 1]), max(v[4 * i + 2], v[4 * i + 3])) >= thi;
    } else {
#pragma unroll
        for (int i = 0; i < 4; ++i)
            gany[i] = fmaxf(fmaxf(acc[4 * i], acc[4 * i + 1]), fmaxf(acc[4 * i + 2], acc[4 * i + 3])) >= th;
    }
    const unsigned a_r = a_q + 4u * kWaveQueueCap, a_v = a_q + 8u * kWaveQueueCap;
#pragma unroll
    for (int gi = 0; gi < 4; ++gi) {
        if (__builtin_amdgcn_ballot_w64(gany[gi]) == 0) continue;
#pragma unroll
        for (int ri = 0; ri < 4; ++ri) {
            const int r = 4 * gi + ri;
            bool hit;
            if constexpr (I8) hit = any && __builtin_bit_cast(i32x16, acc)[r] >= thi;
            else hit = acc[r] >= th;
            if (__builtin_amdgcn_ballot_w64(hit) == 0) continue;
            const int row = rbase + (r & 3) + 8 * (r >> 2);
            hit = hit && row < row_end;
            const unsigned long long bal = __builtin_amdgcn_ballot_w64(hit);
            if (hit) {
                const unsigned e = (unsigned)que_n +
                                   __builtin_amdgcn_mbcnt_hi((unsigned)(bal >> 32), __builtin_amdgcn_mbcnt_lo((unsigned)bal, 0));
                float val;
                if constexpr (I8) val = __builtin_fmaf((float)__builtin_bit_cast(i32x16, acc)[r], m, ek);
                else val = acc[r];
                if (e < (unsigned)kWaveQueueCap) {
                    asm volatile("ds_write_b32 %0, %1" ::"v"(a_q + 4u * e), "v"(q) : "memory");
                    asm volatile("ds_write_b32 %0, %1" ::"v"(a_r + 4u * e), "v"(row) : "memory");
                    asm volatile("ds_write_b32 %0, %1" ::"v"(a_v + 4u * e), "v"(val) : "memory");
                } else {
                    __hip_atomic_fetch_or(&status[q], kStOverflow, __ATOMIC_RELAXED, __HIP_MEMORY_SCOPE_AGENT);
                }
            }
            que_n += __builtin_popcountll(bal);
        }
    }
    return que_n;
}
template <bool I8>
__device__ __attribute__((noinline)) int screen_queue_hits(f32x16 acc, int any_i, int q, int rbase, int row_end, float th,
                                                            float m, float ek, unsigned a_q, int que_n, int* status) {
    return screen_queue_hits_body<I8>(acc, any_i, q, rbase, row_end, th, m, ek, a_q, que_n, status);
}
template <bool I8>
__device__ __forceinline__ void screen_test_block(int* status, f32x16 acc, int q, int rbase, int row_end, float th, I8Blk blk,
                                                  int32_t* que, int& que_n) {
    bool any;
    if constexpr (I8) {
        const i32x16 v = __builtin_bit_cast(i32x16, acc);
        int g[4];
#pragma unroll
        for (int i = 0; i < 4; ++i) g[i] = max(max(v[4 * i], v[4 * i + 1]), max(v[4 * i + 2], v[4 * i + 3]));
        any = i8_value(max(max(g[0], g[1]), max(g[2], g[3])), blk) >= th;
    } else {
        float g[4];
#pragma unroll
        for (int i = 0; i < 4; ++i) g[i] = fmaxf(fmaxf(acc[4 * i], acc[4 * i + 1]), fmaxf(acc[4 * i + 2], acc[4 * i + 3]));
        any = fmaxf(fmaxf(g[0], g[1]), fmaxf(g[2], g[3])) >= th;
    }
    if (__builtin_amdgcn_ballot_w64(any) == 0) return;
    que_n = screen_queue_hits<I8>(acc, any ? 1 : 0, q, rbase, row_end, th, blk.m, blk.ek, lds_addr(que), que_n, status);
}

constexpr int kLaneQueueCap = 64;
constexpr int kLaneQueueEntryBytes = 80;
constexpr int kLaneQueueBytes = kLaneQueueCap * kLaneQueueEntryBytes;
constexpr int kLaneQueueFlushAt = 24;

__device__ __forceinline__ void lds_store16(unsigned addr, i32x4 v) {
    asm volatile("ds_write_b128 %0, %1" ::"v"(addr), "v"(v) : "memory");
}

struct LaneQueueEntry {
    const __attribute__((address_space(3))) int* acc;
    int q, rbase;
    float m, ek, th;
    int thi;
};
template <bool I8>
__device__ __forceinline__ LaneQueueEntry lane_queue_entry(const ScreenArgs& a, unsigned lq_addr, int lane) {
    const __attribute__((address_space(3))) int* e =
        (const __attribute__((address_space(3))) int*)(unsigned long)(lq_addr + (unsigned)lane * 64u);
// ... 121 lines not shown
```

### include/mi355dr.h

```cpp
#ifndef MI355DR_H
#define MI355DR_H

#include <stddef.h>
#include <stdint.h>

#ifdef __cplusplus
extern "C" {
#endif

typedef struct mi355dr_index mi355dr_index;

enum {
    MI355DR_OK = 0,
    MI355DR_E_INVALID = -1,
    MI355DR_E_HIP = -2,
    MI355DR_E_NOMEM = -3,
    MI355DR_E_UNSUPPORTED = -4,
    MI355DR_E_INTERNAL = -5
};

enum { MI355DR_METRIC_COSINE = 0, MI355DR_METRIC_IP = 1 };

enum {
    MI355DR_PATH_AUTO = 0,
// ... 32 lines not shown
                                int64_t* out_rows_dev, void* stream, int64_t* ticket);
int mi355dr_search_wait(mi355dr_index* idx, int64_t ticket);

int mi355dr_search_subset(mi355dr_index* idx, const float* queries, int B, int k, const int64_t* row_ids, int64_t m,
                          double* out_dist, int64_t* out_rows);
int mi355dr_search_subset_device(mi355dr_index* idx, const float* queries_dev, int B, int k, const int64_t* row_ids, int64_t m,
                                 double* out_dist_dev, int64_t* out_rows_dev, void* stream);
int mi355dr_score_subset(mi355dr_index* idx, const float* queries, int B, const int64_t* row_ids, int m, double* out_dist);

int mi355dr_search_mmr(mi355dr_index* idx, const float* queries, int B, int k, int fetch_k, double lambda, double* out_dist,
                       int64_t* out_rows);
int mi355dr_search_mmr_device(mi355dr_index* idx, const float* queries_dev, int B, int k, int fetch_k, double lambda,
                              double* out_dist_dev, int64_t* out_rows_dev, void* stream);
int mi355dr_mmr_select(mi355dr_index* idx, const float* queries, int B, int k, const int64_t* cand_rows , int m,
                       double lambda, double* out_dist, int64_t* out_rows);

int mi355dr_merge_groups_device(mi355dr_index* idx, const double* vals_dev, const int64_t* rows_dev, int S, int width,
                                const int32_t* group_offsets , int G, int k_out, double* out_vals_dev,
                                int64_t* out_rows_dev, int32_t* out_count_dev , void* stream);
int mi355dr_search_groups(mi355dr_index* idx, const float* queries , const int32_t* group_offsets, int G, int k,
                          int fetch_k, double* out_dist , int64_t* out_rows ,
                          int32_t* out_count );
int mi355dr_search_groups_device(mi355dr_index* idx, const float* queries_dev, const int32_t* group_offsets , int G, int k,
                                 int fetch_k, double* out_dist_dev, int64_t* out_rows_dev, int32_t* out_count_dev, void* stream);

int mi355dr_search_range(mi355dr_index* idx, const float* queries, int B, const double* radius ,
                         int max_results, double* out_dist , int64_t* out_rows ,
                         int64_t* out_count );
int mi355dr_search_range_device(mi355dr_index* idx, const float* queries_dev, int B, const double* radius ,
                                int max_results, double* out_dist_dev, int64_t* out_rows_dev, int64_t* out_count_dev,
                                void* stream);

#define MI355DR_ROWS_INCLUDE_SELF 1
int mi355dr_search_rows(mi355dr_index* idx, const int64_t* row_ids , int B, int k, int flags,
                        double* out_dist , int64_t* out_rows );
int mi355dr_search_rows_device(mi355dr_index* idx, const int64_t* row_ids , int B, int k, int flags,
                               double* out_dist_dev, int64_t* out_rows_dev, void* stream);
int mi355dr_search_range_rows(mi355dr_index* idx, const int64_t* row_ids , int B, const double* radius ,
                              int max_results, int flags, double* out_dist ,
                              int64_t* out_rows , int64_t* out_count );
int mi355dr_search_range_rows_device(mi355dr_index* idx, const int64_t* row_ids , int B,
                                     const double* radius , int max_results, int flags, double* out_dist_dev,
                                     int64_t* out_rows_dev, int64_t* out_count_dev, void* stream);

int mi355dr_view_create(mi355dr_index* parent, const int64_t* row_ids, int64_t m_rows, const int64_t* doc_ids, int64_t m_docs,
                        mi355dr_index** out_view);

int mi355dr_add_multivec(mi355dr_index* idx, const float* vecs, const int64_t* offsets, int64_t n_docs);
int mi355dr_add_multivec_device(mi355dr_index* idx, const float* vecs_dev, const int64_t* offsets, int64_t n_docs);
int64_t mi355dr_size_multivec(const mi355dr_index* idx);

int mi355dr_set_multivec(mi355dr_index* idx, const int64_t* doc_ids, const float* vecs, const int64_t* offsets, int64_t n);
int mi355dr_set_multivec_device(mi355dr_index* idx, const int64_t* doc_ids, const float* vecs_dev, const int64_t* offsets, int64_t n);
int64_t mi355dr_live_multivec(const mi355dr_index* idx);

int mi355dr_search_maxsim(mi355dr_index* idx, const float* qtok, const int32_t* q_offsets, int B, int k,
                          float* out_dist, int64_t* out_rows);
int mi355dr_search_maxsim_device(mi355dr_index* idx, const float* qtok_dev, const int32_t* q_offsets, int B, int k,
                                 float* out_dist_dev, int64_t* out_rows_dev, void* stream);

int mi355dr_maxsim_subset(mi355dr_index* idx, const float* qtok, const int32_t* q_offsets, int B, const int64_t* doc_ids,
                          int m, float* out_dist);
#define MI355DR_MAXSIM_CLAMP0 1
int mi355dr_maxsim_subset_ex(mi355dr_index* idx, const float* qtok, const int32_t* q_offsets, int B, const int64_t* doc_ids,
                             int m, int flags, float* out_dist);

int mi355dr_search_maxsim_subset(mi355dr_index* idx, const float* qtok, const int32_t* q_offsets, int B, int k,
                                 const int64_t* doc_ids, int64_t m, float* out_dist, int64_t* out_rows);
int mi355dr_search_maxsim_subset_device(mi355dr_index* idx, const float* qtok_dev, const int32_t* q_offsets, int B, int k,
                                        const int64_t* doc_ids, int64_t m, float* out_dist_dev, int64_t* out_rows_dev,
                                        void* stream);

int mi355dr_add_sparse(mi355dr_index* idx, const int32_t* terms, const int64_t* offsets , int64_t n_docs);
int64_t mi355dr_size_sparse(const mi355dr_index* idx);
int mi355dr_sparse_df(mi355dr_index* idx, const int32_t* terms, int64_t n, int64_t* out_df);
int mi355dr_search_sparse(mi355dr_index* idx, const int32_t* q_terms, const double* q_weights, const int32_t* q_offsets ,
                          int B, int k, double k1, double b, double* out_dist , int64_t* out_rows );
int mi355dr_search_sparse_device(mi355dr_index* idx, const int32_t* q_terms, const double* q_weights, const int32_t* q_offsets,
                                 int B, int k, double k1, double b, double* out_dist_dev, int64_t* out_rows_dev, void* stream);
int mi355dr_search_bm25(mi355dr_index* idx, const int32_t* q_tokens, const int32_t* q_offsets , int B, int k, double k1,
                        double b, double* out_dist, int64_t* out_rows);
int mi355dr_search_bm25_device(mi355dr_index* idx, const int32_t* q_tokens, const int32_t* q_offsets, int B, int k, double k1,
                               double b, double* out_dist_dev, int64_t* out_rows_dev, void* stream);

int mi355dr_gqr_refine(mi355dr_index* idx, const double* queries, int B, const int64_t* cand_rows, int P,
                       const double* comp_dist, int n_steps, double learning_rate, double temperature,
                       double mixture_alpha, double* out_scores);
int mi355dr_gqr_refine_maxsim(mi355dr_index* idx, const double* qtok, const int32_t* q_offsets, int B,
                              const int64_t* doc_ids, int P, const double* comp_dist, int n_steps, double learning_rate,
                              double temperature, double mixture_alpha, double* out_scores);
int mi355dr_gqr_refine_scores(mi355dr_index* idx, const double* primary_scores, const int32_t* counts, int B, int P,
                              const double* comp_dist, int n_steps, double learning_rate, double temperature,
                              double mixture_alpha, double* out_scores);

int mi355dr_merge_topk_device(mi355dr_index* idx, const double* dist_all_dev, const int64_t* rows_all_dev, int world,
                              int B, int k, double* out_dist_dev, int64_t* out_rows_dev, void* stream);

int mi355dr_pack_topk_device(mi355dr_index* idx, const double* dist_dev, const int64_t* rows_dev, int B, int k,
                             int64_t* packed_dev, void* stream);
int mi355dr_merge_topk_packed_device(mi355dr_index* idx, const int64_t* packed_all_dev, int world, int B, int k,
                                     double* out_dist_dev, int64_t* out_rows_dev, void* stream);

int mi355dr_comm_unique_id(void* out_128_bytes, size_t len);
int mi355dr_comm_init(mi355dr_index* idx, int rank, int world, const void* nccl_unique_id, size_t id_len);
int mi355dr_comm_world(const mi355dr_index* idx);
int mi355dr_comm_count(mi355dr_index* idx, int* out);
typedef int (*mi355dr_allgather_fn)(const void* send_dev, void* recv_dev, size_t bytes_per_rank, void* stream, void* user);
int mi355dr_comm_init_custom(mi355dr_index* idx, int rank, int world, mi355dr_allgather_fn fn, void* user);
int mi355dr_search_sharded_device(mi355dr_index* idx, const float* queries_dev, int B, int k, double* out_dist_dev,
                                  int64_t* out_rows_dev, void* stream);

int mi355dr_search_range_sharded_device(mi355dr_index* idx, const float* queries_dev, int B, const double* radius ,
                                        int max_results, double* out_dist_dev, int64_t* out_rows_dev, int64_t* out_count_dev,
                                        void* stream);
int mi355dr_search_rows_sharded_device(mi355dr_index* idx, const int64_t* row_ids , int B, int k, int flags,
                                       double* out_dist_dev, int64_t* out_rows_dev, void* stream);
int mi355dr_search_range_rows_sharded_device(mi355dr_index* idx, const int64_t* row_ids , int B,
                                             const double* radius , int max_results, int flags,
                                             double* out_dist_dev, int64_t* out_rows_dev, int64_t* out_count_dev, void* stream);
int mi355dr_search_mmr_sharded_device(mi355dr_index* idx, const float* queries_dev, int B, int k, int fetch_k, double lambda,
                                      double* out_dist_dev, int64_t* out_rows_dev, void* stream);
int mi355dr_mmr_select_sharded(mi355dr_index* idx, const float* queries, int B, int k, const int64_t* cand_rows ,
                               int m, double lambda, double* out_dist, int64_t* out_rows);

int mi355dr_set_option(mi355dr_index* idx, const char* key, int64_t value);
int mi355dr_get_stat(mi355dr_index* idx, const char* key, int64_t* out);
int mi355dr_reset_stats(mi355dr_index* idx);
int mi355dr_timer_start(mi355dr_index* idx);
int mi355dr_timer_stop(mi355dr_index* idx, double* elapsed_ms);
int mi355dr_synchronize(mi355dr_index* idx);

int mi355dr_dev_alloc(mi355dr_index* idx, size_t bytes, void** out);
int mi355dr_dev_free(mi355dr_index* idx, void* p);
int mi355dr_dev_upload(mi355dr_index* idx, void* dst_dev, const void* src_host, size_t bytes);
int mi355dr_dev_download(mi355dr_index* idx, void* dst_host, const void* src_dev, size_t bytes);

int mi355dr_debug_screen_dense(mi355dr_index* idx, const float* queries, int B, int64_t row0, int64_t n, float* out_t);
int mi355dr_debug_screen_hits(mi355dr_index* idx, const float* queries, int B, int64_t row0, int64_t n, const float* thr,
                              int cap, int* out_count, int32_t* out_rows, float* out_vals, int* out_status, int* out_kernel);
#define MI355DR_MS_FORM_NONE 0
#define MI355DR_MS_FORM_GENERIC 1
#define MI355DR_MS_FORM_D128 2
#define MI355DR_MS_FORM_D128_PACKED 3
#define MI355DR_MS_FORM_WG 4
#define MI355DR_MS_FORM_WG_PACKED 5
#define MI355DR_MS_FORM_LIST_GENERIC 6
#define MI355DR_MS_FORM_LIST_D128 7
int mi355dr_debug_maxsim_pass(mi355dr_index* idx, const float* qtok, const int32_t* q_offsets, int B, int k, const int64_t* doc_ids,
                              int64_t m, int list_cap, int* out_live, float* out_screen, float* out_two_e, int32_t* out_lists,
                              int* out_ctl, float* out_wide_sd, int* out_form, int* out_info);
int mi355dr_debug_screen_bound(mi355dr_index* idx, const float* queries, int B, float* out_E);
int mi355dr_debug_i8_state(mi355dr_index* idx, const float* queries, int B, float* out_sq, float* out_kq, int64_t g0,
                           int64_t n_groups, float* out_step, float* out_err);
int mi355dr_debug_rescore(mi355dr_index* idx, const float* queries, int B, const int32_t* pair_q,
                          const int64_t* pair_row, int64_t n_pairs, float* out_dot, double* out_dist);

int mi355dr_diag_mfma_stream(int device, int format, double seconds, double* out_tops);

#ifdef __cplusplus
}
#endif
#endif
```

Measured before the change: 156,300.

## Speculate screen threshold from starter-sample score moments, skipping chunked passes

During the starter sample screen, per-slab sums and sums of squares of scores are recorded. The prune then fits a normal model and raises the screen threshold to the predicted k-th-best quantile (via spec_m expected survivors). The rest of the corpus is screened in a single pass. Finalize flags queries whose true k-th score falls below the speculative threshold as misses, which are then retried, and a backoff/probation scheme suspends speculation when misses are frequent. It aims to cut candidate volume and per-chunk prune overhead on large indexes, at the risk of retry cost when the score distribution is not normal.

After: 161,700 (median of 6 runs). 3.5% higher.

```diff
diff --git a/autorag_research_amd/_native.py b/autorag_research_amd/_native.py
--- a/autorag_research_amd/_native.py
+++ b/autorag_research_amd/_native.py
@@ -32,7 +32,7 @@
     "mi355dr_dev_alloc", "mi355dr_dev_free", "mi355dr_dev_upload", "mi355dr_dev_download",
     "mi355dr_diag_mfma_stream",
     "mi355dr_debug_screen_dense", "mi355dr_debug_screen_hits", "mi355dr_debug_screen_bound", "mi355dr_debug_i8_state", "mi355dr_debug_rescore",
-    "mi355dr_debug_maxsim_pass",
+    "mi355dr_debug_maxsim_pass", "mi355dr_debug_spec_m",
 ]
 
 
@@ -256,6 +256,8 @@
     L.mi355dr_debug_i8_state.argtypes = [vp, f32p, c_int, f32p, f32p, i64, i64, f32p, f32p]
     L.mi355dr_debug_rescore.restype = c_int
     L.mi355dr_debug_rescore.argtypes = [vp, f32p, c_int, i32p, i64p, i64, f32p, f64p]
+    L.mi355dr_debug_spec_m.restype = c_int
+    L.mi355dr_debug_spec_m.argtypes = [c_int]
     L.mi355dr_debug_maxsim_pass.restype = c_int
     L.mi355dr_debug_maxsim_pass.argtypes = [vp, f32p, i32p, c_int, c_int, i64p, i64, c_int, ctypes.POINTER(c_int), f32p, f32p, i32p,
                                             ctypes.POINTER(c_int), f32p, ctypes.POINTER(c_int), ctypes.POINTER(c_int)]
diff --git a/autorag_research_amd/csrc/dev_common.h b/autorag_research_amd/csrc/dev_common.h
--- a/autorag_research_amd/csrc/dev_common.h
+++ b/autorag_research_amd/csrc/dev_common.h
@@ -16,6 +16,7 @@
 
 constexpr int kStOverflow = 1;
 constexpr int kStIrregular = 2;
+constexpr int kStSpecMiss = 4;
 
 struct QueryState {
     float* qn;
@@ -34,6 +35,19 @@
     float* kq;
     int8_t* qhat8;
     int* carry;
+    float* thr_used;
+};
+
+constexpr int kSpecKMax = 32;
+constexpr int kSpecSlabsMax = 256;
+constexpr int kSpecInflation = 10;
+constexpr int kSpecM[kSpecKMax + 1] = {0,  0,  74, 58, 54, 53, 53, 54, 55, 57, 58, 60, 62, 64, 66, 68, 70,
+                                       71, 73, 75, 0,  0,  0,  0,  0,  0,  0,  0,  0,  0,  0,  0,  0};
+inline int spec_m_of(int k) { return k >= 1 && k <= kSpecKMax ? kSpecM[k] : 0; }
+struct SpecModel {
+    const float* moments;
+    int slabs, rows;
+    float zq;
 };
 
 __device__ __forceinline__ float bf16_bits_to_f32(uint16_t h) { return __uint_as_float((uint32_t)h << 16); }
diff --git a/autorag_research_amd/csrc/index.h b/autorag_research_amd/csrc/index.h
--- a/autorag_research_amd/csrc/index.h
+++ b/autorag_research_amd/csrc/index.h
@@ -80,6 +80,9 @@
     bool i8 = false;
     bool wide = false;
     int cap = 0;
+    bool speculative = false;
+    bool spec_eligible = false;
+    int spec_m = 0;
     const char* refused = nullptr;
 };
 struct Pending {
@@ -231,6 +234,11 @@
     int path = 0;
     int screen_dtype = 0;
     int i8_backoff = 0, i8_probation = 0;
+    int speculate = 1;
+    int64_t spec_min_rows = (int64_t)1 << 20;
+    int spec_shift_milli = 0;
+    int spec_backoff = 0, spec_probation = 0;
+    mi355::DevBuf<float> spec_moments;
     int i8_demoted_k = INT_MAX;
     double i8_min_budget = 0.25;
     mi355::RetryBufs retry[3];
@@ -289,6 +297,7 @@
     mi355::DevBuf<int> rq_progress;
     int rq_epoch = 0;
     int64_t s_rq_launches = 0;
+    int64_t s_spec_passes = 0, s_spec_miss_queries = 0, s_spec_overflow_queries = 0;
     int64_t s_retry_queries = 0;
     int64_t s_ms_screened = 0, s_ms_candidates = 0, s_ms_fallbacks = 0;
     int64_t s_ms_screen_ns = 0, s_ms_screen_launches = 0, s_ms_exact_ns = 0, s_ms_exact_launches = 0, s_ms_pack_ns = 0;
diff --git a/autorag_research_amd/csrc/k_prep.h b/autorag_research_amd/csrc/k_prep.h
--- a/autorag_research_amd/csrc/k_prep.h
+++ b/autorag_research_amd/csrc/k_prep.h
@@ -189,6 +189,7 @@
             st.thr[b] = __builtin_inff();
             st.cnt[b] = 0;
             st.carry[b] = 0;
+            st.thr_used[b] = -__builtin_inff();
             st.best_n[b] = 0;
             st.thr_key[b] = 0;
             st.thr_row[b] = -1;
@@ -259,6 +260,7 @@
         st.thr[b] = (regular || metric == 2) ? -__builtin_inff() : __builtin_inff();
         st.cnt[b] = cnt0;
         st.carry[b] = 0;
+        st.thr_used[b] = -__builtin_inff();
         st.best_n[b] = 0;
         st.thr_key[b] = kKeyNaN;
         st.thr_row[b] = 0x7FFFFFFF;
diff --git a/autorag_research_amd/csrc/k_select.h b/autorag_research_amd/csrc/k_select.h
--- a/autorag_research_amd/csrc/k_select.h
+++ b/autorag_research_amd/csrc/k_select.h
@@ -24,6 +24,7 @@
     int thr_only;
     int one_wave_only;
     int defer_b;
+    SpecModel spec;
 };
 
 __device__ __forceinline__ float unit_sim(int metric, double dist, float inv_qn) {
@@ -367,6 +368,23 @@
                     bkey[i] = K2[i];
                     brow[i] = R2[i];
                 }
+            float t_model = -__builtin_inff();
+            if (a.thr_only && a.spec.moments != nullptr) {
+                const float* mo = a.spec.moments + (int64_t)q * a.spec.slabs * 2;
+                double s1 = 0.0, s2 = 0.0;
+                for (int i = lane; i < a.spec.slabs; i += kWave) {
+                    s1 += (double)mo[2 * i];
+                    s2 += (double)mo[2 * i + 1];
+                }
+#pragma unroll
+                for (int o = 32; o > 0; o >>= 1) {
+                    s1 += __shfl_xor(s1, o, kWave);
+                    s2 += __shfl_xor(s2, o, kWave);
+                }
+                const double mean = s1 / (double)a.spec.rows;
+                const double var = s2 / (double)a.spec.rows - mean * mean;
+                t_model = (float)(mean + sqrt(var > 0.0 ? var : 0.0) * (double)a.spec.zq);
+            }
             if (lane == 0) {
                 if (!a.thr_only) a.st.best_n[q] = n_keep;
                 a.st.cnt[q] = carried;
@@ -377,8 +395,16 @@
                         a.st.thr_key[q] = wk;
                         a.st.thr_row[q] = R2[a.k - 1];
                     }
-                    if (wk != kKeyNaN && !(a.st.status[q] & kStIrregular))
-                        a.st.thr[q] = screen_threshold(a.metric, key_to_dist(wk), E, nq);
+                    if (wk != kKeyNaN && !(a.st.status[q] & kStIrregular)) {
+                        float thr = screen_threshold(a.metric, key_to_dist(wk), E, nq);
+                        if (a.thr_only && a.spec.moments != nullptr) {
+                            const double dist_t = a.metric == 0 ? 1.0 - (double)t_model : -(double)t_model * sqrt((double)nq);
+                            const float thr_model = screen_threshold(a.metric, dist_t, E, nq);
+                            if (thr_model > thr && thr_model < __builtin_inff()) thr = thr_model;
+                            a.st.thr_used[q] = thr;
+                        }
+                        a.st.thr[q] = thr;
+                    }
                 }
             }
             return;
@@ -515,9 +541,17 @@
 }
 
 __global__ __launch_bounds__(64) void k_finalize(QueryState st, int k, int64_t row_offset, const int64_t* __restrict__ row_map,
-                                                  double* out_dist, int64_t* out_rows, int* status_or) {
+                                                  double* out_dist, int64_t* out_rows, int* status_or, int spec_metric) {
     const int q = blockIdx.x;
     const int n = st.best_n[q];
+    if (threadIdx.x == 0 && spec_metric >= 0 && !(st.status[q] & kStIrregular)) {
+        float thr_final = -__builtin_inff();
+        if (n >= k) {
+            const uint64_t wk = st.best_key[(int64_t)q * kKMax + k - 1];
+            if (wk != kKeyNaN) thr_final = screen_threshold(spec_metric, key_to_dist(wk), st.E[q], st.qn[q]);
+        }
+        if (n < k || thr_final < st.thr_used[q]) st.status[q] |= kStSpecMiss;
+    }
     for (int s = threadIdx.x; s < k; s += blockDim.x) {
         if (s < n && st.best_row[(int64_t)q * kKMax + s] != kRowNone) {
             out_dist[(int64_t)q * k + s] = key_to_dist(st.best_key[(int64_t)q * kKMax + s]);
diff --git a/autorag_research_amd/csrc/mi355dr.hip b/autorag_research_amd/csrc/mi355dr.hip
--- a/autorag_research_amd/csrc/mi355dr.hip
+++ b/autorag_research_amd/csrc/mi355dr.hip
@@ -115,6 +115,8 @@
     HIPCHECK(idx, hipMemset(idx->rq_progress, 0, kRqProgressWords * sizeof(int)));
     HIPCHECK(idx, own(idx->st.qhat8, B * idx->dpad8));
     HIPCHECK(idx, own(idx->st.carry, B * sizeof(int)));
+    HIPCHECK(idx, own(idx->st.thr_used, B * sizeof(float)));
+    HIPCHECK(idx, idx->spec_moments.grow(B * kSpecSlabsMax * 2 * sizeof(float)));
     HIPCHECK(idx, idx->qdev.grow(B * idx->dim * sizeof(float)));
     HIPCHECK(idx, idx->cand_row.grow(B * kCandCapWide * sizeof(int32_t)));
     HIPCHECK(idx, idx->cand_val.grow(B * kCandCapWide * sizeof(float)));
@@ -224,6 +226,17 @@
 }
 
 inline bool i8_available(const mi355dr_index* idx) { return idx->irr8_n <= kIrrCap; }
+constexpr int kStarterKMax = 32;
+constexpr int64_t kStarterRows = 16384;
+static_assert(kStarterRows / kSlabRows <= kSpecSlabsMax, "the moment scratch holds one entry per slab of the starter's sample");
+int64_t starter_sample_rows(const mi355dr_index* idx, const Pass& ps) {
+    const int64_t n = idx->n;
+    const int64_t rows = std::min<int64_t>(ps.wide ? idx->starter_rows_wide : kStarterRows, n / 4) / kTileM * kTileM;
+    const int64_t slabs = (rows + kSlabRows - 1) / kSlabRows;
+    const bool take = idx->starter && (ps.k <= kStarterKMax || ps.wide) && ps.level == 0 && idx->chunk0_set == 0 && n >= 4 * 1024 &&
+                      slabs <= ps.cap && slabs >= ps.k;
+    return take ? rows : 0;
+}
 Pass decide_pass(const mi355dr_index* idx, int k, int level, bool force_scan, const char* no_screen = nullptr) {
     Pass ps;
     ps.k = k;
@@ -240,13 +253,19 @@
     if (idx->screen_dtype == MI355DR_SCREEN_I8 && !i8_available(idx) && path != MI355DR_PATH_SCAN)
         ps.refused = "int8 screen unavailable: too many rows outside the residual limit";
     else if (path == MI355DR_PATH_SCREEN && !screen_possible && idx->n > 0) ps.refused = no_screen;
+    ps.spec_m = spec_m_of(k);
+    ps.spec_eligible = level == 0 && ps.screening && !ps.wide && ps.spec_m > 0 && idx->speculate && idx->n >= idx->spec_min_rows &&
+                       kSpecInflation * ps.spec_m * 4 <= 3 * (std::min(kPruneSmallSort, ps.cap) - k) &&
+                       starter_sample_rows(idx, ps) > 0;
+    ps.speculative = ps.spec_eligible && idx->spec_probation <= 0;
     return ps;
 }
 inline bool idle_i8(const mi355dr_index* idx) { return decide_pass(idx, idx->last_pass_k, 0, false).i8; }
 
 int launch_prune(mi355dr_index* idx, hipStream_t s, const Pass& ps, int nblocks, const int* qlist, int exact,
-                 bool thr_only = false, bool one_wave_only = false, bool defer_b = false) {
+                 bool thr_only = false, bool one_wave_only = false, bool defer_b = false, const SpecModel* spec = nullptr) {
     PruneArgs pa{};
+    if (spec) pa.spec = *spec;
     pa.thr_only = thr_only ? 1 : 0;
     pa.one_wave_only = one_wave_only ? 1 : 0;
     pa.defer_b = defer_b && idx->defer_round_b ? 1 : 0;
@@ -313,7 +332,7 @@
 }
 
 int launch_screen(mi355dr_index* idx, hipStream_t s, bool i8, int B, int64_t r0, int64_t r_end, int cap, int emit_mode,
-                  int flush_mask) {
+                  int flush_mask, int moment_slabs = 0) {
     const bool emit_all = emit_mode != 0;
     const ScreenKernel kern = screen_kernel_for(idx, i8, B, r_end - r0, emit_all);
     const int tile = kern == kKern256c || kern == kKernRq ? kT2 : kTileM;
@@ -338,6 +357,10 @@
     sa.row_end = r_end;
     sa.row0 = r0;
     sa.emit_all = emit_mode;
+    if (moment_slabs > 0) {
+        sa.moments = idx->spec_moments;
+        sa.moment_slabs = moment_slabs;
+    }
     const int64_t grid = round_up(sa.n_ctiles, 8) * sa.n_qtiles;
     switch (kern) {
     case kKernRq: {
@@ -401,8 +424,6 @@
     return MI355DR_OK;
 }
 
-constexpr int kStarterKMax = 32;
-constexpr int64_t kStarterRows = 16384;
 struct PassPlan {
     int64_t sample = 0;
     std::vector<int64_t> ends;
@@ -411,16 +432,18 @@
 PassPlan plan_pass(const mi355dr_index* idx, const Pass& ps, int B, double growth) {
     PassPlan p;
     const int64_t n = idx->n;
-    const int k = ps.k, cap = ps.cap;
+    const int cap = ps.cap;
     const bool wide = ps.wide;
     const int tile = screen_tile(B);
     int64_t seen = 0;
-    const int64_t starter_rows = std::min<int64_t>(wide ? idx->starter_rows_wide : kStarterRows, n / 4) / kTileM * kTileM;
-    const int64_t starter_slabs = (starter_rows + kSlabRows - 1) / kSlabRows;
-    if (idx->starter && (k <= kStarterKMax || wide) && ps.level == 0 && idx->chunk0_set == 0 && n >= 4 * 1024 &&
-        starter_slabs <= cap && starter_slabs >= k) {
+    const int64_t starter_rows = starter_sample_rows(idx, ps);
+    if (starter_rows > 0) {
         p.sample = starter_rows;
         seen = p.sample;
+        if (ps.speculative) {
+            p.ends.push_back(n);
+            return p;
+        }
     } else {
         const int64_t c0 = std::min<int64_t>(n, round_up(std::max<int64_t>(tile, std::min<int64_t>(idx->chunk0_rows, cap)), tile));
         p.emit_all_first = c0 <= cap;
@@ -460,6 +483,16 @@
 }
 
 inline int starter_count(const PassPlan& p) { return (int)((p.sample + kSlabRows - 1) / kSlabRows); }
+
+inline double normal_quantile(double p) {
+    double lo = -40.0, hi = 40.0;
+    for (int i = 0; i < 200; ++i) {
+        const double mid = 0.5 * (lo + hi);
+        if (0.5 * std::erfc(-mid / std::sqrt(2.0)) < p) lo = mid;
+        else hi = mid;
+    }
+    return 0.5 * (lo + hi);
+}
 
 PassPlan make_plan(const mi355dr_index* idx, const Pass& ps, int B) {
     const double budget = growth_budget(idx, ps.k, ps.i8);
@@ -498,8 +531,19 @@
         return MI355DR_OK;
     };
     if (plan.sample > 0) {
-        CHECK(timed(false, plan.sample, [&] { return launch_screen(idx, s, i8, B, 0, plan.sample, ps.cap, kEmitSlabMax, -1); }));
-        CHECK(launch_prune(idx, s, ps, B, nullptr, 0, true, true));
+        SpecModel sm{};
+        if (ps.speculative) {
+            sm.moments = idx->spec_moments;
+            sm.slabs = starter_count(plan);
+            sm.rows = (int)plan.sample;
+            sm.zq = (float)(normal_quantile(1.0 - (double)ps.spec_m / (double)idx->n) + idx->spec_shift_milli / 1000.0);
+            idx->s_spec_passes++;
+        }
+        CHECK(timed(false, plan.sample, [&] {
+            return launch_screen(idx, s, i8, B, 0, plan.sample, ps.cap, kEmitSlabMax, -1, ps.speculative ? sm.slabs : 0);
+        }));
+        CHECK(launch_prune(idx, s, ps, B, nullptr, 0, true, true, false,
+                           ps.speculative ? &sm : nullptr));
         idx->s_starters++;
     }
     int64_t done = 0;
@@ -509,7 +553,8 @@
         if (emit_all) kept_all_below = end;
         const bool big = !emit_all && end - done > idx->small_chunk_rows && screen_tile(B) == kT2;
         const int64_t seen = ci == 0 ? (plan.sample > 0 ? plan.sample : end) : done;
-        const double lanes = 8.0 * ps.k * 4096.0 / (double)std::max<int64_t>(seen, 1);
+        const double lanes = ps.speculative ? (double)kSpecInflation * ps.spec_m * 4096.0 / (double)idx->n
+                                            : 8.0 * ps.k * 4096.0 / (double)std::max<int64_t>(seen, 1);
         int period = 1;
         while (period < 64 && period * 2 * lanes <= idx->screen_flush_lanes) period *= 2;
         const int flush_mask = idx->screen_flush_sync ? period - 1 : -1;
@@ -624,7 +669,7 @@
     for (int i = 0; i < B; ++i) all[i] = i;
     if (m > 0) CHECK(run_scan(idx, s, ps, all, m, idx->subset_ids));
     hipLaunchKernelGGL(k_finalize, dim3(B), dim3(64), 0, s, idx->st, k, idx->row_offset, idx->view_row_map.p, out_dist_dev,
-                       out_rows_dev, idx->status_or_dev);
+                       out_rows_dev, idx->status_or_dev, -1);
     HIPCHECK(idx, hipGetLastError());
     HIPCHECK(idx, hipMemcpyAsync(idx->status_host, idx->st.status, (size_t)kQBlockMax * sizeof(int), hipMemcpyDeviceToHost, s));
     HIPCHECK(idx, hipStreamSynchronize(s));
@@ -650,6 +695,7 @@
     const int Bpad = (int)round_up(B, screen_tile(B));
     const Pass ps = decide_pass(idx, k, level, force_scan, "screen path unavailable (metric or too many irregular rows)");
     if (ps.refused) return fail(idx, MI355DR_E_UNSUPPORTED, ps.refused);
+    if (idx->spec_probation > 0 && ps.spec_eligible) idx->spec_probation--;
     if (q_dev != idx->qdev)
         HIPCHECK(idx, hipMemcpyAsync(idx->qdev, q_dev, (size_t)B * idx->dim * sizeof(float), hipMemcpyDeviceToDevice, s));
     PassPlan plan;
@@ -665,7 +711,7 @@
         }
     }
     hipLaunchKernelGGL(k_finalize, dim3(B), dim3(64), 0, s, idx->st, k, idx->row_offset, idx->view_row_map.p, out_dist_dev,
-                       out_rows_dev, idx->status_or_dev);
+                       out_rows_dev, idx->status_or_dev, ps.speculative && idx->n > 0 ? idx->metric : -1);
     HIPCHECK(idx, hipGetLastError());
     HIPCHECK(idx, hipMemcpyAsync(p.status_host, idx->st.status, (size_t)(kQBlockMax + 1) * sizeof(int), hipMemcpyDeviceToHost, s));
     HIPCHECK(idx, hipEventRecord(p.done, s));
@@ -703,6 +749,10 @@
         for (int i = 0; i < B; ++i) {
             const int st = p.status_host[i];
             if (st == 0) continue;
+            if (p.pass.speculative && !(st & kStIrregular)) {
+                if (st & kStOverflow) idx->s_spec_overflow_queries++;
+                else if (st & kStSpecMiss) idx->s_spec_miss_queries++;
+            }
             if (level < kRetryLevels && !(st & kStIrregular)) retry.push_back(i);
             else sub.push_back(i);
         }
@@ -723,7 +773,12 @@
     if (n_todo > 0) CHECK(search_block(idx, s, rb.q, n_todo, k, rb.dist, rb.rows, level + 1, true));
     if (n_retry > 0) {
         idx->s_retry_queries += n_retry;
-        if (p.pass.i8 && idx->screen_dtype == MI355DR_SCREEN_AUTO && n_retry * 100 > B) {
+        if (p.pass.speculative) {
+            if (n_retry * 100 > B && idx->spec_probation <= 0) {
+                idx->spec_backoff = idx->spec_backoff == 0 ? 16 : std::min(idx->spec_backoff * 2, 4096);
+                idx->spec_probation = idx->spec_backoff;
+            }
+        } else if (p.pass.i8 && idx->screen_dtype == MI355DR_SCREEN_AUTO && n_retry * 100 > B) {
             idx->i8_demoted_k = std::min(idx->i8_demoted_k, k);
             idx->i8_backoff = idx->i8_backoff == 0 ? 16 : std::min(idx->i8_backoff * 2, 4096);
             idx->i8_probation = idx->i8_backoff;
@@ -1183,6 +1238,7 @@
     idx->n = n_new;
     idx->i8_demoted_k = INT_MAX;
     idx->i8_backoff = idx->i8_probation = 0;
+    idx->spec_backoff = idx->spec_probation = 0;
     idx->s_compactions += n_moved > 0;
     idx->s_compact_moved_rows += n_moved;
     if (new_of_old) {
@@ -2464,6 +2520,9 @@
     {"chunk0_rows", &Index::chunk0_rows, 1, INT64_MAX, [](Index* x) { x->chunk0_set = 1; }},
     {"starter", {&Index::starter, kSwitch}},
     {"prune_companion", {&Index::prune_companion, kSwitch}},
+    {"speculate", {&Index::speculate, kSwitch}, INT64_MIN, INT64_MAX, [](Index* x) { x->spec_backoff = x->spec_probation = 0; }},
+    {"spec_min_rows", &Index::spec_min_rows, 0},
+    {"spec_shift_milli", &Index::spec_shift_milli, -20000, 20000},
     {"scan_dma", {&Index::scan_dma, kSwitch}},
     {"defer_round_b", {&Index::defer_round_b, kSwitch}},
     {"chunk_growth", &Index::chunk_growth, 1, INT64_MAX, [](Index* x) { x->chunk_growth_set = 1; }},
@@ -2511,6 +2570,10 @@
     {"passes", &Index::s_passes, true},
     {"starters", &Index::s_starters, true},
     {"retry_queries", &Index::s_retry_queries, true},
+    {"spec_passes", &Index::s_spec_passes, true},
+    {"spec_miss_queries", &Index::s_spec_miss_queries, true},
+    {"spec_overflow_queries", &Index::s_spec_overflow_queries, true},
+    {"spec_suspended", nullptr, false, [](const Index* x) -> int64_t { return x->spec_probation > 0 ? 1 : 0; }},
     {"maxsim_screened", &Index::s_ms_screened, true},
     {"maxsim_candidates", &Index::s_ms_candidates, true},
     {"maxsim_fallbacks", &Index::s_ms_fallbacks, true},
@@ -2581,6 +2644,8 @@
 };
 }
 
+int mi355dr_debug_spec_m(int k) { return spec_m_of(k); }
+
 int mi355dr_set_option(mi355dr_index* idx, const char* key, int64_t value) {
     if (!idx || !key) return fail(idx, MI355DR_E_INVALID, "null argument");
     std::lock_guard<std::mutex> g(idx->mu);
diff --git a/autorag_research_amd/csrc/screen_common.h b/autorag_research_amd/csrc/screen_common.h
--- a/autorag_research_amd/csrc/screen_common.h
+++ b/autorag_research_amd/csrc/screen_common.h
@@ -33,6 +33,8 @@
     int64_t row_end;
     int64_t row0;
     int emit_all;
+    float* moments;
+    int moment_slabs;
 };
 constexpr int kEmitAll = 1, kEmitSlabMax = 2;
 constexpr int kSlabRows = 64;
diff --git a/autorag_research_amd/csrc/screen_hits.h b/autorag_research_amd/csrc/screen_hits.h
--- a/autorag_research_amd/csrc/screen_hits.h
+++ b/autorag_research_amd/csrc/screen_hits.h
@@ -70,6 +70,33 @@
                                                      int lane, const I8Blk (&blk)[2]) {
     float best = -__builtin_inff();
     int64_t best_row = slab_row0;
+    if (a.moments != nullptr) {
+        float s1 = 0.0f, s2 = 0.0f;
+#pragma unroll
+        for (int i = 0; i < 2; ++i) {
+            const int64_t rb = slab_row0 + 32 * i + 4 * (lane >> 5);
+#pragma unroll
+            for (int r = 0; r < 16; ++r) {
+                float v;
+                if constexpr (I8) v = (float)__builtin_bit_cast(i32x16, acc[i])[r] * blk[i].m;
+                else v = acc[i][r];
+                if (rb + (r & 3) + 8 * (r >> 2) < a.row_end && v == v) {
+                    s1 += v;
+                    s2 = __builtin_fmaf(v, v, s2);
+                }
+            }
+        }
+        s1 += __shfl_xor(s1, 32, kWave);
+        s2 += __shfl_xor(s2, 32, kWave);
+        if (lane < 32) {
+            const int64_t slot = (slab_row0 - a.row0) / kSlabRows;
+            if (slot < a.moment_slabs) {
+                float* mo = a.moments + ((int64_t)q * a.moment_slabs + slot) * 2;
+                mo[0] = s1;
+                mo[1] = s2;
+            }
+        }
+    }
 #pragma unroll
     for (int i = 0; i < 2; ++i) {
         const int64_t rbase = slab_row0 + 32 * i + 4 * (lane >> 5);
diff --git a/include/mi355dr.h b/include/mi355dr.h
--- a/include/mi355dr.h
+++ b/include/mi355dr.h
@@ -208,6 +208,7 @@
 int mi355dr_debug_screen_bound(mi355dr_index* idx, const float* queries, int B, float* out_E);
 int mi355dr_debug_i8_state(mi355dr_index* idx, const float* queries, int B, float* out_sq, float* out_kq, int64_t g0,
                            int64_t n_groups, float* out_step, float* out_err);
+int mi355dr_debug_spec_m(int k);
 int mi355dr_debug_rescore(mi355dr_index* idx, const float* queries, int B, const int32_t* pair_q,
                           const int64_t* pair_row, int64_t n_pairs, float* out_dot, double* out_dist);
 
```
